# glaretechnologies/substrata

Measured on AMD Instinct MI355X. Metric: physics steps/sec at fixed dt, 100k bodies, higher is better.
Workload: dtype f32; 1 GPU; BASELINE config 3: 100000 mixed box/sphere/capsule bodies, 100x100x10 lattice spacing 1.5 m, seed 3, ground quad 2000 m, dt 1/60, Jolt default settings (10 velocity / 2 position iterations), sleeping enabled; bodies_per_gpu=100000, tiles=1, active_bodies_end=99193, contact_constraints_start=296641, contact_constraints_end=299690, contact_points_end=362045, colours_end=21, contact_constraints_after_settle=293058, dropped_pairs_or_manifolds=0

## Files before the change

### substrata_amd/csrc/sgp_dev_solve.h

```cpp
#pragma once

SGP_DEV sym33 body_world_inv_inertia(const DV& d, uint32_t body)
{
	return world_inv_inertia(quat_to_m33(Q4(d.pose[POSE_F4 * (size_t)body + 1])), V3(d.pose[POSE_F4 * (size_t)body + 2]));
}
SGP_DEV sym33 body_world_inv_inertia_rec(const DV& d, uint32_t body)
{
	const float4 a = d.vel[VEL_F4 * (size_t)body + 2], b = d.vel[VEL_F4 * (size_t)body + 3];
	sym33 s; s.xx = a.x; s.xy = a.y; s.xz = a.z; s.yy = a.w; s.yz = b.x; s.zz = b.y;
	return s;
}

SGP_DEV float lane_swap1(float x)
{
	return __int_as_float(__builtin_amdgcn_mov_dpp(__float_as_int(x), 0xB1, 0xF, 0xF, true));
}

struct ConHalf {
	uint32_t body;
	float4 nf; int np_col;
	v3     c[4][3];
	v3     iv[4][3];
	float  eff[4][3];
	float  bias[4];
// ... 67 lines not shown
			h.lam[i] = V3(l4);
		}
	}
}

template <int ROWS = -1> SGP_DEV void half_load_known(const DV& d, uint32_t slot, int side, int np_col, uint32_t body, ConHalf& h)
{
	h.body = body;
	h.nf = CUR(d).n_fric[slot];
	h.np_col = np_col;
	half_load_rows<ROWS>(d, slot, side, h);
}
template <int ROWS = -1> SGP_DEV void half_load(const DV& d, uint32_t slot, int side, ConHalf& h)
{
	const uint4 hd = con_hdr(CUR(d), slot);
	half_load_known<ROWS>(d, slot, side, (int)hd.z, side ? hd.y : hd.x, h);
}

SGP_DEV void half_store(const DV& d, uint32_t slot, int side, const ConHalf& h)
{
	if (side) return;
	const int np = h.np_col & 0xFF;
#pragma unroll
	for (int i = 0; i < 4; ++i) { if (i < np) CUR(d).lam[i][slot] = F4(h.lam[i], 0.0f); }
}

SGP_DEV float half_jv(v3 lv, v3 av, v3 axis, v3 c, int side)
{
	const float mine = v3_dot(axis, lv) + v3_dot(c, av);
	const float other = lane_swap1(mine);
	return side ? other - mine : mine - other;
}
SGP_DEV void half_apply(v3& lv, v3& av, float im, v3 axis, v3 iv, float lambda, int side)
{
	if (!(im > 0.0f)) return;
	if (side) { lv = v3_add(lv, v3_scale(axis, lambda * im)); av = v3_add(av, v3_scale(iv, lambda)); }
	else      { lv = v3_sub(lv, v3_scale(axis, lambda * im)); av = v3_sub(av, v3_scale(iv, lambda)); }
}

SGP_DEV bool half_solve_core(ConHalf& h, int side, float4& v4, float4& w4, uint32_t dbg)
{
	const int np = h.np_col & 0xFF;
	const float im = v4.w, friction = h.nf.w;
	v3 lv = V3(v4), av = V3(w4);
	const v3 n = V3(h.nf);
	const v3 t1 = (dbg & 2u) ? v3_normalized_perpendicular(n) : h.t1;
	const v3 t2 = v3_cross(n, t1);
	if (friction > 0.0f) {
#pragma unroll
		for (int i = 0; i < 4; ++i) {
			if (i < np && !(h.eff[i][1] <= 0.0f && h.eff[i][2] <= 0.0f)) {
				float l1 = h.lam[i].y + h.eff[i][1] * half_jv(lv, av, t1, h.c[i][1], side);
				float l2 = h.lam[i].z + h.eff[i][2] * half_jv(lv, av, t2, h.c[i][2], side);
				const float max_f = friction * h.lam[i].x;
				const float tot_sq = l1 * l1 + l2 * l2;
				if (tot_sq > max_f * max_f) { const float sc = max_f / sqrtf(tot_sq); l1 = l1 * sc; l2 = l2 * sc; }
				half_apply(lv, av, im, t1, h.iv[i][1], l1 - h.lam[i].y, side); h.lam[i].y = l1;
				half_apply(lv, av, im, t2, h.iv[i][2], l2 - h.lam[i].z, side); h.lam[i].z = l2;
			}
		}
	}
#pragma unroll
	for (int i = 0; i < 4; ++i) {
		if (i < np && h.eff[i][0] > 0.0f) {
			const float jv = half_jv(lv, av, n, h.c[i][0], side);
			const float lambda = h.eff[i][0] * (jv - h.bias[i]);
			const float nl = max0f(h.lam[i].x + lambda);
			half_apply(lv, av, im, n, h.iv[i][0], nl - h.lam[i].x, side);
			h.lam[i].x = nl;
		}
	}
	v4 = F4(lv, im); w4 = F4(av, 0.0f);
	return im > 0.0f;
}
template <int VS> SGP_DEV void half_solve(ConHalf& h, int side, float4* vel, uint32_t dbg = 0)
{
	if ((h.np_col & 0xFF) == 0) return;
	float4 v4 = vel[VS * (size_t)h.body], w4 = vel[VS * (size_t)h.body + 1];
	if (half_solve_core(h, side, v4, w4, dbg)) { vel[VS * (size_t)h.body] = v4; vel[VS * (size_t)h.body + 1] = w4; }
}

template <int VS, int ROWS = -1> SGP_DEV void solve_velocity_pair_t(const DV& d, uint32_t slot, int side, float4* vel)
{
	ConHalf h;
	half_load<ROWS>(d, slot, side, h);
	half_solve<VS>(h, side, vel, d.dbg_flags);
	half_store(d, slot, side, h);
}

template <int VS> SGP_DEV void solve_velocity_pair_norows(const DV& d, uint32_t slot, int side, float4* vel)
{
	const uint4 hd = con_hdr(CUR(d), slot);
	const int np = (int)hd.z & 0xFF;
	const uint32_t body = side ? hd.y : hd.x;
	const float4 nf = CUR(d).n_fric[slot];
	float4 r4[4]; float2 et[4]; v3 lam[4];
#pragma unroll
	for (int i = 0; i < 4; ++i) {
		if (i == 0 || i < np) { r4[i] = side ? CUR(d).r2e[i][slot] : CUR(d).r1b[i][slot]; et[i] = CUR(d).efft[i][slot]; lam[i] = V3(CUR(d).lam[i][slot]); }
		else { r4[i] = make_float4(0.0f, 0.0f, 0.0f, 0.0f); et[i] = make_float2(0.0f, 0.0f); lam[i] = V3(0.0f, 0.0f, 0.0f); }
	}
	if (np == 0) return;
	const sym33 I = body_world_inv_inertia_rec(d, body);
	float4 v4 = vel[VS * (size_t)body], w4 = vel[VS * (size_t)body + 1];
	const float im = v4.w, friction = nf.w;
	v3 lv = V3(v4), av = V3(w4);
	const v3 n = V3(nf);
	const v3 t1 = v3_normalized_perpendicular(n);
	const v3 t2 = v3_cross(n, t1);
	float eff0[4], bias[4];
#pragma unroll
	for (int i = 0; i < 4; ++i) { const float ow = lane_swap1(r4[i].w); eff0[i] = side ? r4[i].w : ow; bias[i] = side ? ow : r4[i].w; }
	if (friction > 0.0f) {
#pragma unroll
		for (int i = 0; i < 4; ++i) {
			if (i < np && !(et[i].x <= 0.0f && et[i].y <= 0.0f)) {
				const v3 r = V3(r4[i]);
				const v3 c1 = v3_cross(r, t1), c2 = v3_cross(r, t2);
				float l1 = lam[i].y + et[i].x * half_jv(lv, av, t1, c1, side);
				float l2 = lam[i].z + et[i].y * half_jv(lv, av, t2, c2, side);
				const float max_f = friction * lam[i].x;
				const float tot_sq = l1 * l1 + l2 * l2;
				if (tot_sq > max_f * max_f) { const float sc = max_f / sqrtf(tot_sq); l1 = l1 * sc; l2 = l2 * sc; }
				half_apply(lv, av, im, t1, sym33_mul(I, c1), l1 - lam[i].y, side); lam[i].y = l1;
				half_apply(lv, av, im, t2, sym33_mul(I, c2), l2 - lam[i].z, side); lam[i].z = l2;
			}
		}
	}
#pragma unroll
	for (int i = 0; i < 4; ++i) {
		if (i < np && eff0[i] > 0.0f) {
			const v3 c0 = v3_cross(V3(r4[i]), n);
			const float jv = half_jv(lv, av, n, c0, side);
			const float lambda = eff0[i] * (jv - bias[i]);
			const float nl = max0f(lam[i].x + lambda);
			half_apply(lv, av, im, n, sym33_mul(I, c0), nl - lam[i].x, side);
			lam[i].x = nl;
		}
	}
	if (im > 0.0f) { vel[VS * (size_t)body] = F4(lv, im); vel[VS * (size_t)body + 1] = F4(av, 0.0f); }
	if (!side) {
#pragma unroll
		for (int i = 0; i < 4; ++i) { if (i < np) CUR(d).lam[i][slot] = F4(lam[i], 0.0f); }
	}
}

struct PosHalf { float4 nf; int np; v3 loc[4]; };
SGP_DEV void pos_half_load(const DV& d, uint32_t slot, int side, int np_col, PosHalf& ph)
{
	ph.nf = CUR(d).n_fric[slot];
	ph.np = np_col & 0xFF;
#pragma unroll
	for (int i = 0; i < 4; ++i) if (i == 0 || i < ph.np) ph.loc[i] = V3(side ? CUR(d).loc2[i][slot] : CUR(d).loc1[i][slot]);
}
SGP_DEV void pos_half_solve(const DV& d, const PosHalf& ph, int side, float4* rec, v3 ii)
{
	const v3 nrm = V3(ph.nf);
	const int np = ph.np;
	const float4 p4 = rec[0];
	const float im = p4.w;
	quat q = Q4(rec[1]);
	v3 pos = V3(p4);
	bool moved = false;
	m33 R = quat_to_m33(q);
#pragma unroll
	for (int i = 0; i < 4; ++i) {
		if (i >= np) continue;
		const v3 mine = v3_add(pos, m33_mul(R, ph.loc[i]));
		const v3 other = V3(lane_swap1(mine.x), lane_swap1(mine.y), lane_swap1(mine.z));
		const v3 p1 = side ? other : mine, p2 = side ? mine : other;
		float sep = v3_dot(v3_sub(p2, p1), nrm) + d.st.penetration_slop;
		if (sep < 0.0f) {
			sep = fmaxf(sep, -d.st.max_penetration_distance);
			const v3 mid = v3_scale(v3_add(p1, p2), 0.5f);
			const v3 r = v3_sub(mid, pos);
			v3 Ic = V3(0.0f, 0.0f, 0.0f);
			float share = 0.0f;
			if (im > 0.0f) { const v3 c = v3_cross(r, nrm); Ic = sym33_mul(world_inv_inertia(R, ii), c); share = im + v3_dot(Ic, c); }
			const float oshare = lane_swap1(share);
			const float s1 = side ? oshare : share, s2 = side ? share : oshare;
			const float inv = s1 + s2;
			const float eff = inv > 0.0f ? 1.0f / inv : 0.0f;
			if (eff <= 0.0f) continue;
			const float lambda = -eff * d.st.baumgarte * sep;
			if (im > 0.0f) {
				if (side) { pos = v3_add(pos, v3_scale(nrm, lambda * im)); q = quat_add_rotation_step(q, v3_scale(Ic, lambda)); }
				else      { pos = v3_sub(pos, v3_scale(nrm, lambda * im)); q = quat_add_rotation_step(q, v3_scale(Ic, -lambda)); }
				R = quat_to_m33(q);
			}
			moved = true;
		}
	}
	if (moved && im > 0.0f) { rec[0] = F4(pos, im); rec[1] = make_float4(q.x, q.y, q.z, q.w); }
}
SGP_DEV void solve_position_pair(const DV& d, uint32_t slot, int side)
{
	const uint4 hd = con_hdr(CUR(d), slot);
	const uint32_t body = side ? hd.y : hd.x;
	PosHalf ph;
	pos_half_load(d, slot, side, (int)hd.z, ph);
	pos_half_solve(d, ph, side, d.pose + POSE_F4 * (size_t)body, V3(d.pose[POSE_F4 * (size_t)body + 2]));
}
SGP_DEV void solve_position_pair_at(const DV& d, uint32_t slot, int side, float4* rec, v3 ii)
{
	PosHalf ph;
	pos_half_load(d, slot, side, con_npc(CUR(d), slot), ph);
	pos_half_solve(d, ph, side, rec, ii);
}
#define SOLVE_VEL_TPB 256
#define SOLVE_XCD_CHUNKS 0x100

SGP_DEV uint32_t uf_prio(uint32_t x);
SGP_DEV uint32_t uf_find(const uint32_t* parent, uint32_t x);
```

### substrata_amd/csrc/sgp_k_solve.hip

```cpp
#include "sgp_dev_all.h"


struct BodyVel { v3 lv, av; };

SGP_DEV void apply_impulse(BodyVel& A, BodyVel& B, float im1, const sym33& I1, float im2, const sym33& I2, v3 r1, v3 r2, v3 axis, float lambda)
{
	if (im1 > 0.0f) {
		A.lv = v3_sub(A.lv, v3_scale(axis, lambda * im1));
		A.av = v3_sub(A.av, v3_scale(sym33_mul(I1, v3_cross(r1, axis)), lambda));
	}
	if (im2 > 0.0f) {
		B.lv = v3_add(B.lv, v3_scale(axis, lambda * im2));
		B.av = v3_add(B.av, v3_scale(sym33_mul(I2, v3_cross(r2, axis)), lambda));
	}
}

SGP_DEV float axis_jv(const BodyVel& A, const BodyVel& B, v3 r1, v3 r2, v3 axis)
{
	return (v3_dot(axis, A.lv) + v3_dot(v3_cross(r1, axis), A.av)) - (v3_dot(axis, B.lv) + v3_dot(v3_cross(r2, axis), B.av));
}

struct PairCtx { uint2 ab; float im1, im2; sym33 I1, I2; BodyVel A, B; v3 n, t1, t2; float friction; int np; };
template <int VS> SGP_DEV void load_pair(const DV& d, uint32_t slot, PairCtx& c, const float4* vel)
{
// ... 209 lines not shown
	}
}

#define TAIL_VEL_TPB 768
template <int ROWS> __global__ void __launch_bounds__(TAIL_VEL_TPB) k_solve_tail_vel(DV d, int first_colour)
{
	__shared__ uint32_t cs[SGP_MAX_COLOURS + 1];
	if (threadIdx.x <= SGP_MAX_COLOURS) cs[threadIdx.x] = d.cstarts[threadIdx.x];
	__syncthreads();
	if (cs[first_colour] == cs[SGP_MAX_COLOURS]) return;
	const int side = (int)(threadIdx.x & 1u);
	const uint32_t pair = threadIdx.x >> 1;
	const uint32_t tail_n = cs[SGP_OVERFLOW_COLOUR] - cs[first_colour];
	if (tail_n <= TAIL_VEL_TPB / 2 && !(d.dbg_flags & 1u)) {
		const uint32_t slot = cs[first_colour] + pair;
		const bool mine = pair < tail_n;
		ConHalf h; int my_col = -1;
		if (mine) { half_load<ROWS>(d, slot, side, h); my_col = (h.np_col >> 8) & 0xFF; }
		for (int c = first_colour; c < SGP_OVERFLOW_COLOUR; ++c) {
			if (cs[c] == cs[c + 1]) continue;
			if (my_col == c) half_solve<VEL_F4>(h, side, d.vel, d.dbg_flags);
			__syncthreads();
		}
		if (mine) half_store(d, slot, side, h);
	} else
	for (int c = first_colour; c < SGP_OVERFLOW_COLOUR; ++c) {
		const uint32_t b = cs[c], e = cs[c + 1];
		if (b == e) continue;
		for (uint32_t k = b + pair; k < e; k += TAIL_VEL_TPB / 2) solve_velocity_pair_t<VEL_F4, ROWS>(d, k, side, d.vel);
		__syncthreads();
	}
	const uint32_t first = cs[SGP_OVERFLOW_COLOUR], count = cs[SGP_OVERFLOW_COLOUR + 1] - first;
	if (count == 0 || threadIdx.x >= 2) return;
	uint64_t last = 0; bool have_last = false;
	for (uint32_t it = 0; it < count; ++it) {
		const uint32_t bslot = overflow_next(d, first, count, last, have_last);
		solve_velocity_pair_t<VEL_F4, ROWS>(d, bslot, side, d.vel);
	}
}
#define HC_CLASSES 9
#define HC_WG_PAIRS 256
#define HC_TPB (2 * HC_WG_PAIRS)
#define HC_BIG 0xFFFFFFFFu
#define HC_NONE 0xFFFFFFFFu
#define NPCOL_CATCH_ALL (1 << 17)
#define HC_BIG_LIST (4 * HC_WG_PAIRS)

SGP_DEV bool hc_can_move(const DV& d, uint32_t body) { return d.vel[VEL_F4 * (size_t)body].w > 0.0f; }

__global__ void __launch_bounds__(TPB) k_hc_hook(DV d, int first_colour)
{
	const uint32_t b = d.cstarts[first_colour], e = d.cstarts[SGP_OVERFLOW_COLOUR];
	const uint32_t tid = blockIdx.x * TPB + threadIdx.x, stride = gridDim.x * TPB;
	const uint32_t lim = min(2u * (e - b) + HC_CLASSES * HC_WG_PAIRS, d.cap_hc_list);
	for (uint32_t i = tid; i < lim; i += stride) d.hc_list[i] = HC_NONE;
	for (uint32_t k = b + tid; k < e; k += stride) {
		const uint2 ab = con_ab(CUR(d), k);
		if (!hc_can_move(d, ab.x) || !hc_can_move(d, ab.y)) continue;
		uint32_t ra = uf_find(d.hc_root, ab.x), rb = uf_find(d.hc_root, ab.y);
		while (ra != rb) {
			const bool a_hi = uf_prio(ra) > uf_prio(rb);
			const uint32_t hi = a_hi ? ra : rb, lo = a_hi ? rb : ra;
			const uint32_t old = atomicCAS(&d.hc_root[hi], hi, lo);
			if (old == hi) break;
			ra = uf_find(d.hc_root, old); rb = uf_find(d.hc_root, lo);
		}
	}
}
SGP_DEV uint32_t hc_root_of(const DV& d, uint2 ab)
{
	const uint32_t x = hc_can_move(d, ab.x) ? ab.x : (hc_can_move(d, ab.y) ? ab.y : HC_NONE);
	return x == HC_NONE ? HC_NONE : uf_find(d.hc_root, x);
}
__global__ void __launch_bounds__(TPB) k_hc_count(DV d, int first_colour)
{
	const uint32_t b = d.cstarts[first_colour], e = d.cstarts[SGP_OVERFLOW_COLOUR];
	for (uint32_t k = b + blockIdx.x * TPB + threadIdx.x; k < e; k += gridDim.x * TPB) {
		const uint32_t r = hc_root_of(d, con_ab(CUR(d), k));
		d.hc_rank[k] = r == HC_NONE ? 0u : atomicAdd(&d.hc_count[r], 1u);
	}
}
__global__ void __launch_bounds__(TPB) k_hc_alloc(DV d, int first_colour)
{
	const uint32_t b = d.cstarts[first_colour], e = d.cstarts[SGP_OVERFLOW_COLOUR];
	const int lane = (int)(threadIdx.x & 63u);
	for (uint32_t k0 = b + blockIdx.x * TPB; k0 < e; k0 += gridDim.x * TPB) {
		const uint32_t k = k0 + threadIdx.x;
		uint32_t r = HC_NONE, size = 0;
		if (k < e && d.hc_rank[k] == 0u) { r = hc_root_of(d, con_ab(CUR(d), k)); if (r != HC_NONE) size = d.hc_count[r]; }
		const bool lead = r != HC_NONE;
		int cls = -1;
		if (lead) {
			if (size > (uint32_t)HC_WG_PAIRS) d.hc_base[r] = HC_BIG;
			else cls = size <= 1u ? 0 : 32 - __clz((int)(size - 1u));
		}
		unsigned long long mine_m = 0ull;
#pragma unroll
		for (int c = 0; c < HC_CLASSES; ++c) { const unsigned long long m = __ballot(cls == c); if (cls == c) mine_m = m; }
		const int leader = mine_m ? __ffsll((long long)mine_m) - 1 : lane;
		uint32_t base = 0;
		if (cls >= 0 && lane == leader) base = atomicAdd(&d.ctr->hc_class[cls], (uint32_t)__popcll(mine_m));
		base = __shfl(base, leader, 64);
		if (cls >= 0) d.hc_base[r] = ((uint32_t)cls << 28) | (base + (uint32_t)__popcll(mine_m & ((1ull << lane) - 1ull)));
	}
}
SGP_DEV uint32_t hc_class_first(const DV& d, int cls)
{
	uint32_t first = 0;
	for (int c = 0; c < cls; ++c) first += ((d.ctr->hc_class[c] << c) + (HC_WG_PAIRS - 1)) & ~(uint32_t)(HC_WG_PAIRS - 1);
	return first;
}
__global__ void __launch_bounds__(TPB) k_hc_scatter(DV d, int first_colour)
{
	const uint32_t b = d.cstarts[first_colour], e = d.cstarts[SGP_OVERFLOW_COLOUR];
	if (blockIdx.x == 0 && threadIdx.x == 0) { d.ctr->hc_entries = hc_class_first(d, HC_CLASSES); d.ctr->hc_n = e - b; }
	for (uint32_t k = b + blockIdx.x * TPB + threadIdx.x; k < e; k += gridDim.x * TPB) {
		const uint32_t r = hc_root_of(d, con_ab(CUR(d), k));
		const uint32_t place = r == HC_NONE ? HC_BIG : d.hc_base[r];
		uint32_t at = HC_NONE;
		if (place != HC_BIG) {
			const int cls = (int)(place >> 28);
			at = hc_class_first(d, cls) + ((place & 0x0FFFFFFFu) << cls) + d.hc_rank[k];
		}
		if (at < d.cap_hc_list) d.hc_list[at] = k;
		else {
			con_npc(CUR(d), k) |= NPCOL_CATCH_ALL;
			const uint32_t bi = wave_alloc(&d.ctr->hc_n_big);
			if (bi < HC_BIG_LIST) d.hc_big_list[bi] = k;
		}
	}
}

__global__ void __launch_bounds__(TPB) k_hc_init(DV d, int first_colour)
{
	const uint32_t b = d.cstarts[first_colour], e = d.cstarts[SGP_OVERFLOW_COLOUR];
	for (uint32_t k = b + blockIdx.x * TPB + threadIdx.x; k < e; k += gridDim.x * TPB) {
		const uint2 ab = con_ab(CUR(d), k);
		if (hc_can_move(d, ab.x)) { d.hc_root[ab.x] = ab.x; d.hc_count[ab.x] = 0u; }
		if (hc_can_move(d, ab.y)) { d.hc_root[ab.y] = ab.y; d.hc_count[ab.y] = 0u; }
	}
}
__global__ void __launch_bounds__(TPB) k_hc_probe(DV d, int first_colour)
{
	const uint32_t b = d.cstarts[first_colour], e = d.cstarts[SGP_OVERFLOW_COLOUR];
	for (uint32_t k = b + blockIdx.x * TPB + threadIdx.x; k < e; k += gridDim.x * TPB) {
		if (d.hc_rank[k] != 0u) continue;
		const uint32_t r = hc_root_of(d, con_ab(CUR(d), k));
		if (r == HC_NONE) continue;
		const uint32_t size = d.hc_count[r];
		if (size > (uint32_t)HC_WG_PAIRS) atomicAdd(&d.ctr->hc_probe_big, size);
	}
}

__global__ void __launch_bounds__(HC_WG_PAIRS) k_hc_sort(DV d)
{
	__shared__ uint32_t s_cnt[SGP_MAX_COLOURS], s_first[SGP_MAX_COLOURS];
	__shared__ uint4 s_slot[HC_WG_PAIRS];
	const uint32_t entries = d.ctr->hc_entries;
	for (uint32_t e0 = blockIdx.x * HC_WG_PAIRS; e0 < entries; e0 += gridDim.x * HC_WG_PAIRS) {
		if (threadIdx.x < SGP_MAX_COLOURS) s_cnt[threadIdx.x] = 0u;
		__syncthreads();
		const uint32_t slot = d.hc_list[e0 + threadIdx.x];
		const uint4 hd = slot != HC_NONE ? con_hdr(CUR(d), slot) : make_uint4(0u, 0u, 0u, 0u);
		const int npc = (int)hd.z;
		const uint2 ab = make_uint2(hd.x, hd.y);
		const int col = slot != HC_NONE ? ((npc >> 8) & 0xFF) : SGP_MAX_COLOURS - 1;
		const uint32_t rank = atomicAdd(&s_cnt[col], 1u);
		__syncthreads();
		if (threadIdx.x < 64) {
			const uint32_t v = s_cnt[threadIdx.x];
			uint32_t x = v;
			for (int off = 1; off < 64; off <<= 1) { const uint32_t y = __shfl_up(x, off, 64); if ((int)threadIdx.x >= off) x += y; }
			s_first[threadIdx.x] = x - v;
		}
		__syncthreads();
		s_slot[s_first[col] + rank] = make_uint4(slot, (uint32_t)npc, ab.x, ab.y);
		__syncthreads();
		d.hc_entry[e0 + threadIdx.x] = s_slot[threadIdx.x];
		__syncthreads();
	}
}

#define HC_TABLE 1024
template <int MODE, int ROWS = -1> __global__ void __launch_bounds__(HC_TPB) k_solve_hc(const StepCounters* ctr_pre, const uint4* hc_entry_pre, DV d, int first_colour)
{
	constexpr int RS = MODE == 1 ? 2 : 3;
	__shared__ float4 s_rec[HC_TABLE * RS];
	__shared__ uint32_t s_key[HC_TABLE];
	__shared__ unsigned long long s_present;
	__shared__ uint32_t s_ticket;
	const int side = (int)(threadIdx.x & 1u);
	const uint32_t pair = threadIdx.x >> 1;
	const uint32_t entries = ctr_pre->hc_entries;
	const int n_colours = (int)ctr_pre->n_colours;
	for (uint32_t e0 = blockIdx.x * HC_WG_PAIRS; e0 < entries; e0 += gridDim.x * HC_WG_PAIRS) {
		__syncthreads();
		for (uint32_t i = threadIdx.x; i < HC_TABLE; i += HC_TPB) s_key[i] = HC_NONE;
		if (threadIdx.x == 0) s_present = 0ull;
		__syncthreads();
		const uint4 entry = hc_entry_pre[e0 + pair];
		const uint32_t slot = entry.x;
		const bool mine = slot != HC_NONE;
		ConHalf h; PosHalf ph; int my_col = -1;
		uint32_t body = HC_NONE, at = 0; bool owner = false;
		if (mine) {
			my_col = ((int)entry.y >> 8) & 0xFF;
			body = side ? entry.w : entry.z;
			if (MODE == 1) half_load_known<ROWS>(d, slot, side, (int)entry.y, body, h); else pos_half_load(d, slot, side, (int)entry.y, ph);
			if (side == 0) atomicOr(&s_present, 1ull << my_col);
			at = uf_prio(body) & (HC_TABLE - 1);
			for (;;) {
				const uint32_t old = atomicCAS(&s_key[at], HC_NONE, body);
				if (old == HC_NONE) { owner = true; break; }
				if (old == body) break;
				at = (at + 1) & (HC_TABLE - 1);
			}
			if (owner) {
				const float4* g = (MODE == 1 ? d.vel + VEL_F4 * (size_t)body : d.pose + POSE_F4 * (size_t)body);
				s_rec[RS * at] = g[0]; s_rec[RS * at + 1] = g[1];
				if (MODE != 1) s_rec[RS * at + 2] = d.pose[POSE_F4 * (size_t)body + 2];
			}
			if (MODE == 1) h.body = at;
		}
		__syncthreads();
		const unsigned long long present = s_present;
		for (int c = first_colour; c < n_colours; ++c) {
			if (!((present >> c) & 1ull)) continue;
			if (my_col == c) { if (MODE == 1) half_solve<2>(h, side, s_rec, d.dbg_flags); else pos_half_solve(d, ph, side, s_rec + RS * at, V3(s_rec[RS * at + 2])); }
			__syncthreads();
		}
		if (MODE == 1 && mine) half_store(d, slot, side, h);
		if (owner && s_rec[RS * at].w > 0.0f) {
			float4* g = (MODE == 1 ? d.vel + VEL_F4 * (size_t)body : d.pose + POSE_F4 * (size_t)body);
			g[0] = s_rec[RS * at]; g[1] = s_rec[RS * at + 1];
		}
	}
	const uint32_t n_big = d.ctr->hc_n_big;
	const uint32_t ofirst = d.cstarts[SGP_OVERFLOW_COLOUR], ocount = d.cstarts[SGP_OVERFLOW_COLOUR + 1] - ofirst;
	if (n_big == 0u && ocount == 0u) return;
	__syncthreads();
	if (threadIdx.x == 0) { __threadfence(); s_ticket = atomicAdd(&d.ctr->hc_done, 1u); }
	__syncthreads();
	if (s_ticket != gridDim.x - 1u) return;
	if (threadIdx.x == 0) d.ctr->hc_done = 0u;
	__threadfence();
	if (n_big != 0u && n_big <= (uint32_t)HC_BIG_LIST) {
		uint32_t mine[4]; int mcol[4]; int cnt = 0;
		for (uint32_t e = pair; e < n_big; e += HC_WG_PAIRS) { const uint32_t k = d.hc_big_list[e]; mine[cnt] = k; mcol[cnt] = (int)((con_npc(CUR(d), k) >> 8) & 0xFF); ++cnt; }
		for (int c = first_colour; c < n_colours; ++c) {
#pragma unroll
			for (int j = 0; j < 4; ++j) if (j < cnt && mcol[j] == c) { if (MODE == 1) solve_velocity_pair_t<VEL_F4, ROWS>(d, mine[j], side, d.vel); else solve_position_pair(d, mine[j], side); }
			__syncthreads();
		}
	} else
	for (int c = first_colour; c < n_colours && n_big != 0u; ++c) {
		const uint32_t cb = d.cstarts[c], ce = d.cstarts[c + 1];
		for (uint32_t k = cb + pair; k < ce; k += HC_WG_PAIRS) {
			if (!(con_npc(CUR(d), k) & NPCOL_CATCH_ALL)) continue;
			if (MODE == 1) solve_velocity_pair_t<VEL_F4, ROWS>(d, k, side, d.vel); else solve_position_pair(d, k, side);
		}
		__syncthreads();
	}
	if (ocount == 0u || threadIdx.x >= 2u) return;
	uint64_t last = 0; bool have_last = false;
	for (uint32_t it = 0; it < ocount; ++it) {
		const uint32_t bslot = overflow_next(d, ofirst, ocount, last, have_last);
		if (MODE == 1) solve_velocity_pair_t<VEL_F4, ROWS>(d, bslot, side, d.vel); else solve_position_pair(d, bslot, side);
	}
}

#define SMALL_LDS_BODIES 2048
#define SMALL_TPB 768
__global__ void __launch_bounds__(SMALL_TPB) k_solve_small(DV d, int warm_start, int iterations)
{
	__shared__ float4 sv[2 * SMALL_LDS_BODIES];
	__shared__ uint32_t cs[SGP_MAX_COLOURS + 1];
	const uint32_t n = min(d.sp->n_slots, (uint32_t)SMALL_LDS_BODIES);
	if (threadIdx.x <= SGP_MAX_COLOURS) cs[threadIdx.x] = d.cstarts[threadIdx.x];
	for (uint32_t i = threadIdx.x; i < 2 * n; i += SMALL_TPB) sv[i] = d.vel[VEL_F4 * (size_t)(i >> 1) + (i & 1u)];
	__syncthreads();
	const int side = (int)(threadIdx.x & 1u);
	const uint32_t pair = threadIdx.x >> 1;
	const uint32_t all_n = cs[SGP_OVERFLOW_COLOUR];
	if (all_n != 0 && all_n <= SMALL_TPB / 2 && cs[SGP_OVERFLOW_COLOUR] == cs[SGP_MAX_COLOURS]) {
		const uint32_t slot = pair;
		const bool mine = slot < all_n;
		if (warm_start) {
			for (int c = 0; c < SGP_OVERFLOW_COLOUR; ++c) {
				const uint32_t b = cs[c], e = cs[c + 1];
				if (b == e) continue;
				if (side == 0 && slot >= b && slot < e) warm_start_one_t<2>(d, slot, sv);
				__syncthreads();
			}
		}
		ConHalf h; int my_col = -1;
		if (mine) { half_load<0>(d, slot, side, h); my_col = (h.np_col >> 8) & 0xFF; }
		for (int pass = 0; pass < iterations; ++pass) {
			for (int c = 0; c < SGP_OVERFLOW_COLOUR; ++c) {
				if (cs[c] == cs[c + 1]) continue;
				if (my_col == c) half_solve<2>(h, side, sv, d.dbg_flags);
				__syncthreads();
			}
		}
		if (mine) half_store(d, slot, side, h);
	} else
	if (cs[0] != cs[SGP_MAX_COLOURS]) {
		for (int pass = warm_start ? -1 : 0; pass < iterations; ++pass) {
			for (int c = 0; c < SGP_OVERFLOW_COLOUR; ++c) {
				const uint32_t b = cs[c], e = cs[c + 1];
				if (b == e) continue;
				if (pass < 0) { for (uint32_t k = b + threadIdx.x; k < e; k += SMALL_TPB) warm_start_one_t<2>(d, k, sv); }
				else { for (uint32_t k = b + pair; k < e; k += SMALL_TPB / 2) solve_velocity_pair_t<2, 0>(d, k, side, sv); }
				__syncthreads();
			}
			const uint32_t first = cs[SGP_OVERFLOW_COLOUR], count = cs[SGP_OVERFLOW_COLOUR + 1] - first;
			if (count != 0) {
				if (threadIdx.x < 2) {
					uint64_t last = 0; bool have_last = false;
					for (uint32_t it = 0; it < count; ++it) {
						const uint32_t bslot = overflow_next(d, first, count, last, have_last);
						if (pass < 0) { if (side == 0) warm_start_one_t<2>(d, bslot, sv); } else solve_velocity_pair_t<2, 0>(d, bslot, side, sv);
					}
				}
				__syncthreads();
			}
		}
	}
	for (uint32_t i = threadIdx.x; i < 2 * n; i += SMALL_TPB) d.vel[VEL_F4 * (size_t)(i >> 1) + (i & 1u)] = sv[i];
}

struct ConReg { uint2 ab; float4 nf; int np_col; AxisRows rn[4], rt1[4], rt2[4]; float4 lam[4]; };

SGP_DEV void con_load(const DV& d, uint32_t slot, ConReg& r)
{
	const uint4 hd = con_hdr(CUR(d), slot);
	r.ab = make_uint2(hd.x, hd.y);
	r.nf = CUR(d).n_fric[slot];
	r.np_col = (int)hd.z;
	const int np = r.np_col & 0xFF;
#pragma unroll
	for (int i = 0; i < 4; ++i) {
		if (i < np) {
			r.rn[i] = load_axis_rows(d, slot, i, 0); r.rt1[i] = load_axis_rows(d, slot, i, 1); r.rt2[i] = load_axis_rows(d, slot, i, 2);
			r.lam[i] = CUR(d).lam[i][slot];
		}
	}
}

SGP_DEV void con_store(const DV& d, uint32_t slot, const ConReg& r)
{
	const int np = r.np_col & 0xFF;
#pragma unroll
	for (int i = 0; i < 4; ++i) { if (i < np) CUR(d).lam[i][slot] = r.lam[i]; }
}

template <int VS> SGP_DEV void con_solve_velocity(ConReg& r, float4* vel, uint32_t dbg = 0)
{
	const uint2 ab = r.ab;
	const int np = r.np_col & 0xFF;
	if (np == 0) return;
	const float4 va = vel[VS * (size_t)ab.x], wa = vel[VS * (size_t)ab.x + 1];
	const float4 vb = vel[VS * (size_t)ab.y], wb = vel[VS * (size_t)ab.y + 1];
	const float im1 = va.w, im2 = vb.w, friction = r.nf.w;
	BodyVel A, B;
	A.lv = V3(va); A.av = V3(wa); B.lv = V3(vb); B.av = V3(wb);
	const v3 n = V3(r.nf);
	const v3 t1 = (dbg & 2u) ? v3_normalized_perpendicular(n) : V3(r.rn[0].i1.w, r.rn[0].i2.w, r.rt1[0].i1.w);
	const v3 t2 = v3_cross(n, t1);
	if (friction > 0.0f) {
#pragma unroll
		for (int i = 0; i < 4; ++i) {
			if (i < np && !(r.rt1[i].c2.w <= 0.0f && r.rt2[i].c2.w <= 0.0f)) {
				float l1 = r.lam[i].y + r.rt1[i].c2.w * rows_jv(A, B, t1, r.rt1[i]);
				float l2 = r.lam[i].z + r.rt2[i].c2.w * rows_jv(A, B, t2, r.rt2[i]);
				const float max_f = friction * r.lam[i].x;
				const float tot_sq = l1 * l1 + l2 * l2;
				if (tot_sq > max_f * max_f) { const float sc = max_f / sqrtf(tot_sq); l1 = l1 * sc; l2 = l2 * sc; }
				rows_apply(A, B, im1, im2, t1, r.rt1[i], l1 - r.lam[i].y); r.lam[i].y = l1;
				rows_apply(A, B, im1, im2, t2, r.rt2[i], l2 - r.lam[i].z); r.lam[i].z = l2;
			}
		}
	}
#pragma unroll
	for (int i = 0; i < 4; ++i) {
		if (i < np && r.rn[i].c2.w > 0.0f) {
			const float jv = rows_jv(A, B, n, r.rn[i]);
			const float lambda = r.rn[i].c2.w * (jv - r.rn[i].c1.w);
			const float nl = max0f(r.lam[i].x + lambda);
			rows_apply(A, B, im1, im2, n, r.rn[i], nl - r.lam[i].x);
			r.lam[i].x = nl;
		}
	}
	if (im1 > 0.0f) { vel[VS * (size_t)ab.x] = F4(A.lv, im1); vel[VS * (size_t)ab.x + 1] = F4(A.av, 0.0f); }
	if (im2 > 0.0f) { vel[VS * (size_t)ab.y] = F4(B.lv, im2); vel[VS * (size_t)ab.y + 1] = F4(B.av, 0.0f); }
}

template <int VS> SGP_DEV void solve_velocity_one_t(const DV& d, uint32_t slot, float4* vel)
{
	ConReg r;
	con_load(d, slot, r);
	con_solve_velocity<VS>(r, vel, d.dbg_flags);
	con_store(d, slot, r);
}
__global__ void __launch_bounds__(512) k_solve_small_single(DV d, int warm_start, int iterations)
{
	__shared__ float4 sv[2 * SMALL_LDS_BODIES];
	__shared__ uint32_t cs[SGP_MAX_COLOURS + 1];
	const uint32_t n = min(d.sp->n_slots, (uint32_t)SMALL_LDS_BODIES);
	if (threadIdx.x <= SGP_MAX_COLOURS) cs[threadIdx.x] = d.cstarts[threadIdx.x];
	for (uint32_t i = threadIdx.x; i < 2 * n; i += 512) sv[i] = d.vel[VEL_F4 * (size_t)(i >> 1) + (i & 1u)];
	__syncthreads();
	const uint32_t all_n = cs[SGP_OVERFLOW_COLOUR];
	if (all_n != 0 && all_n <= 512u && cs[SGP_OVERFLOW_COLOUR] == cs[SGP_MAX_COLOURS]) {
		const uint32_t slot = threadIdx.x;
		const bool mine = slot < all_n;
		if (warm_start) {
			for (int c = 0; c < SGP_OVERFLOW_COLOUR; ++c) {
				const uint32_t b = cs[c], e = cs[c + 1];
				if (b == e) continue;
				if (slot >= b && slot < e) warm_start_one_t<2>(d, slot, sv);
				__syncthreads();
			}
		}
		ConReg r; int my_col = -1;
		if (mine) { con_load(d, slot, r); my_col = (r.np_col >> 8) & 0xFF; }
		for (int pass = 0; pass < iterations; ++pass) {
			for (int c = 0; c < SGP_OVERFLOW_COLOUR; ++c) {
				if (cs[c] == cs[c + 1]) continue;
				if (my_col == c) con_solve_velocity<2>(r, sv, d.dbg_flags);
				__syncthreads();
			}
		}
		if (mine) con_store(d, slot, r);
	} else
	if (cs[0] != cs[SGP_MAX_COLOURS]) {
		for (int pass = warm_start ? -1 : 0; pass < iterations; ++pass) {
			for (int c = 0; c < SGP_OVERFLOW_COLOUR; ++c) {
				const uint32_t b = cs[c], e = cs[c + 1];
				if (b == e) continue;
				for (uint32_t k = b + threadIdx.x; k < e; k += 512) {
					if (pass < 0) warm_start_one_t<2>(d, k, sv); else solve_velocity_one_t<2>(d, k, sv);
				}
				__syncthreads();
			}
			const uint32_t first = cs[SGP_OVERFLOW_COLOUR], count = cs[SGP_OVERFLOW_COLOUR + 1] - first;
			if (count != 0) {
				if (threadIdx.x == 0) {
					uint64_t last = 0; bool have_last = false;
					for (uint32_t it = 0; it < count; ++it) {
						uint64_t best = ~0ull; uint32_t bslot = first;
						for (uint32_t k = 0; k < count; ++k) {
							const uint2 okab = con_ab(CUR(d), first + k); const uint64_t pr = sgp_mix64(((uint64_t)okab.x << 32) | okab.y);
							if ((!have_last || pr > last) && pr <= best) { best = pr; bslot = first + k; }
						}
						last = best; have_last = true;
						if (pass < 0) warm_start_one_t<2>(d, bslot, sv); else solve_velocity_one_t<2>(d, bslot, sv);
					}
				}
				__syncthreads();
			}
		}
	}
	for (uint32_t i = threadIdx.x; i < 2 * n; i += 512) d.vel[VEL_F4 * (size_t)(i >> 1) + (i & 1u)] = sv[i];
}
#ifndef SGP_EXPERIMENTS
void launch_solve_probe(const DV&, int, int, uint32_t, hipStream_t) {}
void launch_ts_label(const DV&, uint32_t, hipStream_t) {}
void launch_colour_count_ts(const DV&, uint32_t, hipStream_t) {}
void launch_setup_ts(const DV&, uint32_t, hipStream_t) {}
void launch_ts_solve(const DV&, int, int, hipStream_t) {}
#endif
#define SOLVE_MANY_MIN 131072u
#ifndef SOLVE_MANY_OCC
#define SOLVE_MANY_OCC 3
#endif
void launch_solve_colour(const DV& d, int colour, uint32_t est, int mode, hipStream_t s, int compact_rows)
{
	uint32_t blocks = (est + est / 8 + 64 + SOLVE_TPB - 1) / SOLVE_TPB;
	if (mode != 0) blocks = (est + est / 8 + 64 + SOLVE_VEL_TPB / 2 - 1) / (SOLVE_VEL_TPB / 2);
	if (blocks > 8192) blocks = 8192;
	if (mode != 0) blocks = (blocks + 7u) & ~7u;
	if (mode != 0 && est >= 8192u && est <= 65536u) colour |= SOLVE_XCD_CHUNKS;
	if (mode == 0) hipLaunchKernelGGL(k_solve_colour<0>, dim3(blocks), dim3(SOLVE_TPB), 0, s, (const uint32_t*)d.cstarts, d.sp, d, colour);
	else if (mode == 1) {
		const bool many = est > SOLVE_MANY_MIN;
		if (compact_rows == 2) hipLaunchKernelGGL((k_solve_colour<1, 2>), dim3(blocks), dim3(SOLVE_VEL_TPB), 0, s, (const uint32_t*)d.cstarts, d.sp, d, colour);
		else if (compact_rows) { if (many) hipLaunchKernelGGL((k_solve_colour<1, 1, SOLVE_MANY_OCC>), dim3(blocks), dim3(SOLVE_VEL_TPB), 0, s, (const uint32_t*)d.cstarts, d.sp, d, colour); else hipLaunchKernelGGL((k_solve_colour<1, 1>), dim3(blocks), dim3(SOLVE_VEL_TPB), 0, s, (const uint32_t*)d.cstarts, d.sp, d, colour); }
		else hipLaunchKernelGGL((k_solve_colour<1, 0>), dim3(blocks), dim3(SOLVE_VEL_TPB), 0, s, (const uint32_t*)d.cstarts, d.sp, d, colour);
	}
	else if (est > SOLVE_MANY_MIN) hipLaunchKernelGGL((k_solve_colour<2, -1, SOLVE_MANY_OCC>), dim3(blocks), dim3(SOLVE_VEL_TPB), 0, s, (const uint32_t*)d.cstarts, d.sp, d, colour);
	else hipLaunchKernelGGL(k_solve_colour<2>, dim3(blocks), dim3(SOLVE_VEL_TPB), 0, s, (const uint32_t*)d.cstarts, d.sp, d, colour);
}
void launch_warm_bodies(const DV& d, uint32_t nb, hipStream_t s) { hipLaunchKernelGGL(k_warm_bodies, dim3(blocks_for(nb)), dim3(TPB), 0, s, d); }
void launch_solve_tail(const DV& d, int first_colour, int mode, hipStream_t s, int compact_rows)
{
	if (mode == 1) {
		if (compact_rows == 2) hipLaunchKernelGGL(k_solve_tail_vel<2>, dim3(1), dim3(TAIL_VEL_TPB), 0, s, d, first_colour);
		else if (compact_rows) hipLaunchKernelGGL(k_solve_tail_vel<1>, dim3(1), dim3(TAIL_VEL_TPB), 0, s, d, first_colour);
		else hipLaunchKernelGGL(k_solve_tail_vel<0>, dim3(1), dim3(TAIL_VEL_TPB), 0, s, d, first_colour);
	}
	else hipLaunchKernelGGL(k_solve_tail, dim3(1), dim3(512), 0, s, d, first_colour, mode);
}
void launch_hc_build(const DV& d, int first_colour, uint32_t est, hipStream_t s)
{
	const uint32_t blocks = std::max(1u, std::min(1024u, (est + est / 8 + TPB - 1) / TPB));
	hipLaunchKernelGGL(k_hc_hook, dim3(blocks), dim3(TPB), 0, s, d, first_colour);
	hipLaunchKernelGGL(k_hc_count, dim3(blocks), dim3(TPB), 0, s, d, first_colour);
	hipLaunchKernelGGL(k_hc_alloc, dim3(blocks), dim3(TPB), 0, s, d, first_colour);
	hipLaunchKernelGGL(k_hc_scatter, dim3(blocks), dim3(TPB), 0, s, d, first_colour);
	hipLaunchKernelGGL(k_hc_sort, dim3(std::max(1u, std::min(2048u, (2u * est + HC_CLASSES * HC_WG_PAIRS) / HC_WG_PAIRS))), dim3(HC_WG_PAIRS), 0, s, d);
}
void launch_hc_probe(const DV& d, int probe_colour, uint32_t probe_est, hipStream_t s)
{
	const uint32_t pb = std::max(1u, std::min(1024u, (probe_est + probe_est / 8 + TPB - 1) / TPB));
	hipLaunchKernelGGL(k_hc_hook, dim3(pb), dim3(TPB), 0, s, d, probe_colour);
	hipLaunchKernelGGL(k_hc_count, dim3(pb), dim3(TPB), 0, s, d, probe_colour);
	hipLaunchKernelGGL(k_hc_probe, dim3(pb), dim3(TPB), 0, s, d, probe_colour);
	hipLaunchKernelGGL(k_hc_init, dim3(pb), dim3(TPB), 0, s, d, probe_colour);
}
void launch_solve_hc(const DV& d, int first_colour, uint32_t est, int mode, hipStream_t s, int compact_rows)
{
	const uint32_t blocks = std::max(1u, std::min(2048u, (2u * est + HC_CLASSES * HC_WG_PAIRS) / HC_WG_PAIRS));
	if (mode == 1) {
		if (compact_rows == 2) hipLaunchKernelGGL((k_solve_hc<1, 2>), dim3(blocks), dim3(HC_TPB), 0, s, (const StepCounters*)d.ctr, (const uint4*)d.hc_entry, d, first_colour);
		else if (compact_rows) hipLaunchKernelGGL((k_solve_hc<1, 1>), dim3(blocks), dim3(HC_TPB), 0, s, (const StepCounters*)d.ctr, (const uint4*)d.hc_entry, d, first_colour);
		else hipLaunchKernelGGL((k_solve_hc<1, 0>), dim3(blocks), dim3(HC_TPB), 0, s, (const StepCounters*)d.ctr, (const uint4*)d.hc_entry, d, first_colour);
	}
	else hipLaunchKernelGGL((k_solve_hc<2, -1>), dim3(blocks), dim3(HC_TPB), 0, s, (const StepCounters*)d.ctr, (const uint4*)d.hc_entry, d, first_colour);
}
void launch_solve_small(const DV& d, int warm_start, int iterations, int lane_pairs, hipStream_t s)
{
	if (lane_pairs) hipLaunchKernelGGL(k_solve_small, dim3(1), dim3(SMALL_TPB), 0, s, d, warm_start, iterations);
	else hipLaunchKernelGGL(k_solve_small_single, dim3(1), dim3(512), 0, s, d, warm_start, iterations);
}
```

### substrata_amd/csrc/sgp_kernels.h

```cpp
#pragma once
#include <hip/hip_runtime.h>
#include <stdint.h>
#include "../../include/sgp.h"

#define BF_MOTION_MASK   0x3u
#define BF_LAYER_SHIFT   2
#define BF_LAYER_MASK    (0x3u << BF_LAYER_SHIFT)
#define BF_ALIVE         (1u << 4)
#define BF_ACTIVE        (1u << 5)
#define BF_SENSOR        (1u << 6)
#define BF_ALLOW_SLEEP   (1u << 7)
#define BF_ZERO_LIN_DRAG (1u << 8)
#define BF_LARGE         (1u << 9)
#define BF_UNDERWATER    (1u << 10)
#define BF_GHOST         (1u << 11)
#define BF_HAS_FORCE     (1u << 13)
#define BF_CACHE_INVALID (1u << 12)
#define BF_SHAPE_SHIFT   18
#define BF_SHAPE_MASK    (0x7u << BF_SHAPE_SHIFT)
#define BF_CHASSIS       (1u << 22)
#define BF_ALIAS         (1u << 21)
#define BF_WAKE          (1u << 14)
#define BF_CAN_SLEEP     (1u << 15)
#define BF_MOVABLE_PREV  (1u << 16)
// ... 83 lines not shown
	uint32_t colour_fill[SGP_MAX_COLOURS];
	uint32_t cnp_count[SGP_MAX_COLOURS * 4];
	uint32_t cnp_start[SGP_MAX_COLOURS * 4];
	uint32_t cnp_fill[SGP_MAX_COLOURS * 4];
};

struct EventCounters {
	uint32_t n_activated;
	uint32_t n_deactivated;
	uint32_t n_water;
	uint32_t n_contact_added;
	uint32_t n_contact_persisted;
	uint32_t pad[3];
};
#define SGP_EVENT_WINDOW 256u
struct EventWindow {
	EventCounters c;
	uint32_t ids[3][SGP_EVENT_WINDOW];
};

#define CMD_SET_POS      (1u << 0)
#define CMD_SET_ROT      (1u << 1)
#define CMD_SET_VEL      (1u << 2)
#define CMD_SET_SHAPE    (1u << 3)
#define CMD_ADD_FORCE    (1u << 4)
#define CMD_ADD_TORQUE   (1u << 5)
#define CMD_ADD_FORCE_AT (1u << 6)
#define CMD_ACTIVATE     (1u << 7)
#define CMD_SET_LAYER    (1u << 8)
#define CMD_REMOVE       (1u << 9)
#define CMD_MOVE_KINEMATIC (1u << 10)
#define CMD_CREATE       (1u << 11)
#define CMD_SET_CHASSIS  (1u << 12)

struct GhostRefresh { uint32_t id; float pos[3]; float rot[4]; float linv[3]; float angv[3]; };

struct BodyCmd {
	uint32_t id;
	uint32_t ops;
	float pos[3];
	float rot[4];
	float linv[3];
	float angv[3];
	float shape[4];
	float dt;
	float inv_mass, mass;
	float inv_inertia[3];
	float friction, restitution, gravity_factor, lin_damp, ang_damp;
	uint32_t flags;
	uint32_t pad_;
	uint64_t userdata;
};

struct StepParams {
	float    dt;
	uint32_t n_slots;
	uint32_t n_large;
	float    cell_size;
	float    bp_rmax;
	int      water_enabled; float water_z;
	int      contact_events;
	uint32_t parity;
	uint32_t compact_rows;
	uint32_t pad[6];
};

#define PREC_F4 4
struct ConstraintArrays {
	uint4*    hdr;
	float4*   n_fric;
	float4*   r1b[4];
	float4*   r2e[4];
	float4*   lam[4];
	float2*   efft[4];
	float4*   loc1[4];
	float4*   loc2[4];
	float4*   prec;
};

#define POSE_F4 4u
#define VEL_F4 4u
struct DV {
	StepParams* sp;
	uint32_t cap_bodies, cap_pairs, cap_manifolds;
	float4* pose;
	float4* vel;
	float4* dyn;
	float4* force;
	float4* torque;
	uint32_t* flags;
	float4* aabb_min;
	float4* aabb_max;
	float4* sleep_s[3];
	float*  sleep_timer;
	uint32_t* sleep_label;
	uint32_t* slot_gen;
	uint32_t* label_wake;
	uint2*  wake_pairs; uint32_t cap_wake_pairs;
	float*  submerged;
	uint64_t* userdata;
	uint64_t* colour_mask;
	float4* warm;
	uint64_t* claim[2];
	uint32_t* island;
	uint32_t* island_awake;
	uint32_t* export_counts;
	uint32_t* awake_mark;
	uint32_t ts_nt, ts_gx, ts_gy;
	uint8_t*  body_tile;
	uint64_t* body_tiles4;
	uint8_t*  man_tile;
	uint32_t* ts_count;
	uint32_t* ts_start;
	uint32_t* ts_fill;
	uint32_t* ts_adj;
	uint64_t* ts_wait;
	uint32_t* ts_epoch;
	uint32_t* ts_flags;
	uint16_t* ts_at;
	uint8_t*  ts_side;
	uint32_t table_size;
	uint32_t* cell_hash;
	uint32_t* cell_count;
	uint32_t* cell_start;
	uint32_t* cell_fill;
	uint32_t* scan_block_sums;
	float4*   sorted_min;
	float4*   sorted_max;
	struct BpGrid* grid;
	int*      bounds_acc;
	uint32_t* grid_cells_used;
	uint32_t* tile_slot;
	uint32_t* tile_of_slot;
	uint32_t  tile_table_size;
	const uint32_t* large_ids;
	uint2*    pairs;
	uint2*    man_ab;
	float4*   man_n;
	float4*   man_p1[4];
	float4*   man_p2[4];
	int32_t*  man_colour;
	uint32_t* ulist[2];
	uint64_t* man_prio;
	uint32_t* man_slot;
	uint32_t* man_prev;
	uint32_t* hc_root;
	uint32_t* hc_count;
	uint32_t* hc_base;
	uint32_t* hc_rank;
	uint32_t* hc_list;
	uint4*    hc_entry;
	uint32_t  cap_hc_list;
	uint32_t* hc_big_list;
	uint32_t dbg_flags;
	float4* rows;
	ConstraintArrays ca[2];
	uint4* ht; uint32_t ht_size;
	uint32_t* cache_total;
	uint32_t* ht_cur;
	uint32_t* cstarts;
	StepCounters* ctr;
	EventCounters* evc;
	uint32_t* ev_activated; uint32_t* ev_deactivated; uint32_t* ev_water;
	uint32_t ev_window;
	sgp_contact_event* ev_contacts_added; sgp_contact_event* ev_contacts_persisted; uint32_t cap_contact_events;
	const struct sgd_hull_s* hulls; uint32_t n_hulls;
	uint2* hull_pairs; uint32_t cap_hull_pairs;
	struct HullWork* hull_work;
	const struct MeshHeader* meshes; uint32_t n_meshes;
	const float4* mesh_verts; const uint4* mesh_tris; const uint32_t* mesh_tri_mat; const struct MeshNode* mesh_nodes; const uint32_t* mesh_field;
	const LargeGrid* lgrid; const uint32_t* lg_start; const uint32_t* lg_items;
	uint2* mesh_pairs; uint32_t cap_mesh_pairs; uint32_t* mesh_big;
	struct sgd_vehicle* vehicles; uint32_t n_vehicles; const sgp_vehicle_input* vehicle_inputs;
	float4* veh_rows; float4* veh_head; uint32_t veh_cap;
	uint64_t* veh_claim; uint32_t* veh_epoch; uint32_t* veh_defer_bits;
	sgp_settings st;
	float gx, gy, gz;
};

void launch_step_begin(const DV& d, const StepParams& sp, uint32_t nb, bool reset_step_scratch, bool ev_reset, hipStream_t s);
void launch_set_params(const DV& d, const StepParams& sp, hipStream_t s);
void launch_step_end(const DV& d, StepCounters* host_mapped, EventWindow* host_events, hipStream_t s);
void launch_fill_u64(uint64_t* p, uint64_t v, size_t n, hipStream_t s);
void launch_pre_solve(const DV& d, uint32_t nb, hipStream_t s);
void launch_bp_bounds(const DV& d, uint32_t nb, hipStream_t s);
void launch_bp_cell(const DV& d, uint32_t nb, hipStream_t s);
void launch_bp_scan(const DV& d, hipStream_t s);
void launch_bp_scatter(const DV& d, uint32_t nb, hipStream_t s);
void launch_bp_pairs(const DV& d, int small_lds, hipStream_t s);
void launch_bp_large(const DV& d, uint32_t nb, hipStream_t s);
void launch_bp_scatter_large(const DV& d, uint32_t nb, hipStream_t s);
void launch_narrowphase(const DV& d, uint32_t n_pairs_upper, hipStream_t s);
void launch_wake_round(const DV& d, uint32_t nb, int has_hulls, bool has_meshes, hipStream_t s);
void launch_narrowphase_hull(const DV& d, bool big_hulls, hipStream_t s);
void launch_narrowphase_mesh(const DV& d, bool has_hulls, hipStream_t s);
void launch_narrowphase_mesh_blocks(const DV& d, bool has_hulls, uint32_t blocks, hipStream_t s);
void launch_colour_inherit(const DV& d, uint32_t n_man, hipStream_t s);
void launch_colour_claim(const DV& d, uint32_t n_man, uint32_t round, hipStream_t s);
void launch_colour_commit(const DV& d, uint32_t n_man, uint32_t round, hipStream_t s);
void launch_colour_count(const DV& d, uint32_t n_man, hipStream_t s);
void launch_colour_finish(const DV& d, uint32_t first_round, int build_list, hipStream_t s);
void launch_setup(const DV& d, uint32_t n_man, hipStream_t s);
void launch_ts_label(const DV& d, uint32_t nb, hipStream_t s);
void launch_colour_count_ts(const DV& d, uint32_t n_man, hipStream_t s);
void launch_setup_ts(const DV& d, uint32_t n_man, hipStream_t s);
void launch_ts_solve(const DV& d, int passes, int colour_end, hipStream_t s);
void launch_solve_colour(const DV& d, int colour, uint32_t est, int mode, hipStream_t s, int compact_rows);
void launch_solve_probe(const DV& d, int variant, int colour, uint32_t est, hipStream_t s);
void launch_warm_bodies(const DV& d, uint32_t nb, hipStream_t s);
void launch_solve_tail(const DV& d, int first_colour, int mode, hipStream_t s, int compact_rows = 0);
#define SGP_SMALL_WORLD_BODIES 2048
void launch_hc_build(const DV& d, int first_colour, uint32_t est, hipStream_t s);
void launch_hc_probe(const DV& d, int probe_colour, uint32_t probe_est, hipStream_t s);
void launch_solve_hc(const DV& d, int first_colour, uint32_t est, int mode, hipStream_t s, int compact_rows);
void launch_solve_small(const DV& d, int warm_start, int iterations, int lane_pairs, hipStream_t s);
void launch_integrate_pose(const DV& d, uint32_t nb, hipStream_t s);
void launch_finalize(const DV& d, uint32_t nb, hipStream_t s);
void launch_island_mark(const DV& d, uint32_t n_con, int clear_cache, hipStream_t s);
void launch_island_hook(const DV& d, uint32_t n_con, hipStream_t s);
void launch_island_flag(const DV& d, uint32_t n_con, hipStream_t s);
void launch_sleep_apply(const DV& d, uint32_t nb, hipStream_t s);
void launch_buoyancy(const DV& d, uint32_t nb, hipStream_t s);
void launch_cache_build(const DV& d, uint32_t n_con, StepCounters* host_mapped, EventWindow* host_events, hipStream_t s);
void launch_contact_events(const DV& d, uint32_t n_man, hipStream_t s);
void launch_ghost_refresh(const DV& d, const GhostRefresh* recs, uint32_t n, hipStream_t s);
void launch_apply_cmds(const DV& d, const BodyCmd* cmds, const uint32_t* run_start, uint32_t n_runs, hipStream_t s);
void launch_gather_aabbs(const DV& d, const uint32_t* ids, uint32_t n, float4* out, hipStream_t s);
void launch_gather_states(const DV& d, const uint32_t* ids, uint32_t first, uint32_t n, sgp_body_state* out, hipStream_t s);
void launch_gather_active(const DV& d, uint32_t nb, sgp_body_state* out, uint32_t cap, hipStream_t s);
void launch_gather_active_poses(const DV& d, uint32_t nb, void* out, uint32_t cap, hipStream_t s);
void launch_dump_constraints(const DV& d, uint32_t which, uint32_t n_con, void* out, uint32_t cap, hipStream_t s);
void launch_vehicle_pre(const DV& d, bool cylinder_testers, hipStream_t s);
void launch_vehicle_solve(const DV& d, int mode, hipStream_t s);
void launch_solve_colour_veh(const DV& d, int colour, uint32_t est, int mode, hipStream_t s, int compact_rows);
struct RayMailbox {
	uint32_t req_seq, stop_gen; sgp_ray ray; uint32_t pad0[16 - 2 - sizeof(sgp_ray) / 4];
	uint32_t done_seq, exited_gen; sgp_hit hit; uint32_t pad1[16 - 2 - sizeof(sgp_hit) / 4 - 1]; uint32_t done_seq2;
};
static_assert(sizeof(RayMailbox) == 128 && sizeof(sgp_ray) == 36 && sizeof(sgp_hit) == 48, "RayMailbox: two 64-byte lines");
void launch_ray_server(const DV& d, RayMailbox* mb, uint32_t first_seq, uint32_t generation, uint64_t idle_ticks, uint64_t max_ticks, hipStream_t s);
void launch_raycast(const DV& d, const sgp_ray* rays, uint32_t n, sgp_hit* hits, hipStream_t s);
void launch_collide_capsules(const DV& d, const sgp_capsule_query* q, uint32_t n, sgp_query_contact* out, uint32_t cap, uint32_t* count, hipStream_t s);
void launch_spherecast(const DV& d, const sgp_ray* rays, const float* radii, uint32_t n, sgp_hit* hits, hipStream_t s);
enum { SQ_N_OUT = 0, SQ_N_PRIM = 1, SQ_N_HULL = 2, SQ_N_MESH = 3 };
struct SqBufs {
	const sgp_shape_query* qs; uint32_t n;
	sgp_query_contact* out; uint32_t cap;
	uint32_t* ctr;
	uint2* prim; uint2* hull; uint2* mesh; uint32_t pcap;
};
void launch_shape_queries_wave(const DV& d, const SqBufs& b, hipStream_t s);
void launch_shape_queries_pairs(const DV& d, const SqBufs& b, hipStream_t s);
enum { SC_N_OUT = 0, SC_N_PRIM = 1, SC_N_HULL = 2, SC_N_MESH = 3, SC_N_CAPPED = 4, SC_N_DROPPED = 5, SC_N_CTR = 8 };
struct ScBufs {
	const sgp_shape_cast* cs; uint32_t n;
	sgp_cast_hit* out;
	uint32_t* ctr;
	uint2* prim; uint2* hull; uint2* mesh; uint32_t pcap;
};
void launch_shape_casts(const DV& d, const ScBufs& b, hipStream_t s);
#define SGP_CHAR_MAX_PUSHES 32
#define SGP_CHAR_MAX_ADDED 32
#define SGP_CHAR_MAX_SEEN 128
#define SGP_CHAR_MESH_LIST 32
struct CharRec {
	uint32_t alive, reset_serial, pose_serial, pad_;
	float pose[3];
	float radius, half_height, offset[3], up[3], sv_n[3], sv_c, cos_max_slope, mass, max_strength, predictive, padding, recovery, tolerance;
	uint32_t max_coll_it, max_cons_it; float min_time;
	float stick[3], stairs_up[3], min_step_fwd, step_fwd_test, cos_fwd, down_extra[3];
};
struct CharIn { float vel[3]; uint32_t ignore, flags, serial; };
struct CharContact { uint32_t body, idx; float p[3], n[3], v[3], dist; uint32_t bits; float inv_mass; };
struct CharState {
	float pos[3], vel[3]; uint32_t ground_state; float gn[3], gv[3], gp[3]; uint32_t ground_body, overflow;
	uint32_t n_active, n_seen, reset_serial, pose_serial, in_serial, pad_[3];
};
struct CharPush { uint32_t body; float f[3], p[3]; uint32_t pad_; };
struct CharAdded { uint32_t body, pad_; float p[3], n[3]; };
struct CharBufs {
	const CharRec* rec; const CharIn* in; CharState* st;
	CharContact* active;
	uint32_t* seen;
	CharPush* push; uint32_t* n_push;
	uint32_t* push_any;
	CharAdded* added; uint32_t* n_added;
	uint32_t n;
};
void launch_characters_update(const DV* d_dev, const CharBufs& b, float dt, hipStream_t s);
void launch_characters_push(const DV& d, const CharBufs& b, hipStream_t s);
void launch_characters_sync(const CharBufs& b, hipStream_t s);
void launch_export_boundary(const DV& d, uint32_t nb, float3 lo, float3 hi, float margin, sgp_ghost_record* out, uint32_t cap, uint32_t* count, hipStream_t s);

#define SGP_MAX_TILES 64
struct TileRoute { float boxes[6 * SGP_MAX_TILES]; uint32_t n_tiles, my_rank; float margin, pad; };
struct RouteHeader { uint32_t seg_count[SGP_MAX_TILES]; uint32_t seg_start[SGP_MAX_TILES]; uint32_t n_emigrants; uint32_t total; uint32_t pad[2]; };
#define SGP_TILE_HIST_BINS 1024
struct TilePlanes { uint32_t gx, gy, gz, by_contacts; float glo[3], ghi[3]; float xp[4]; float yp[16]; };
void launch_tiles_hist(const DV& d, uint32_t nb, const TilePlanes& tp, int level, uint32_t* out, hipStream_t s);
#define ROUTE_OK 0u
#define ROUTE_REDO 1u
#define ROUTE_FAILED 2u
void launch_route_export(const DV& d, uint32_t nb, const TileRoute& t, uint32_t* block_counts, uint32_t* block_offsets, RouteHeader* header,
                         sgp_ghost_record* out, uint32_t cap, uint32_t* emigrant_ids, uint32_t emigrant_cap, uint32_t* gather_row, uint32_t cap_recv, uint32_t host_status, hipStream_t s);
void launch_pack_ghost_keys(const sgp_ghost_record* recs, uint32_t n, void* out_uint4, void* aux_uint4, const float* region_lo, const float* region_hi, hipStream_t s);
void launch_create_from_records(const DV& d, const sgp_ghost_record* recs, const void* list_uint4, uint32_t n, float gravity_factor, float lin_damp, float ang_damp, hipStream_t s);
#define GKEY_VALID      (1u << 0)
#define GKEY_SHAPE_SHIFT 1
#define GKEY_FLAGS_SHIFT 4
#define GKEY_IN_REGION  (1u << 10)
void launch_ghost_refresh_records(const DV& d, const sgp_ghost_record* recs, const uint32_t* ids, uint32_t n, hipStream_t s);

#define SGP_CKPT_MAX_SEGS 160
struct CkptTable { uint32_t n; uint32_t start[SGP_CKPT_MAX_SEGS + 1]; const void* src[SGP_CKPT_MAX_SEGS]; void* dst[SGP_CKPT_MAX_SEGS]; };
void launch_ckpt_copy(const CkptTable& t, uint32_t n_cus, hipStream_t s);
void launch_ckpt_grid_reset(const DV& d, hipStream_t s);
```

### substrata_amd/csrc/sgp_world.hip

```cpp
#include "sgp_world_internal.h"

thread_local std::string g_last_error;
int g_device_count = -1;

static std::mutex g_worlds_mutex;
static std::set<uint64_t> g_worlds;
static uint64_t g_next_serial = 0;
uint64_t world_register() { std::lock_guard<std::mutex> l(g_worlds_mutex); const uint64_t s = ++g_next_serial; g_worlds.insert(s); return s; }
void world_unregister(uint64_t serial) { std::lock_guard<std::mutex> l(g_worlds_mutex); g_worlds.erase(serial); }
bool world_alive(uint64_t serial) { std::lock_guard<std::mutex> l(g_worlds_mutex); return g_worlds.count(serial) != 0; }


SGP_API void sgp_default_settings(sgp_settings* s)
{
	s->num_velocity_steps = 10;
	s->num_position_steps = 2;
	s->baumgarte = 0.2f;
	s->penetration_slop = 0.02f;
	s->speculative_contact_distance = 0.02f;
	s->min_velocity_for_restitution = 1.0f;
	s->max_penetration_distance = 0.2f;
	s->time_before_sleep = 0.5f;
	s->point_velocity_sleep_threshold = 0.03f;
	s->contact_point_preserve_lambda_max_dist_sq = 0.01f * 0.01f;
// ... 8 lines not shown

SGP_API void sgp_default_world_desc(sgp_world_desc* d)
{
	memset(d, 0, sizeof(*d));
	d->max_bodies = 65536;
	d->gravity[0] = 0.0f; d->gravity[1] = 0.0f; d->gravity[2] = -9.81f;
	d->large_body_radius = 4.0f;
	sgp_default_settings(&d->settings);
}

SGP_API void sgp_default_body_desc(sgp_body_desc* d)
{
	memset(d, 0, sizeof(*d));
	d->rot[3] = 1.0f;
	d->shape_type = SGP_SHAPE_BOX;
	d->shape[0] = d->shape[1] = d->shape[2] = 0.5f;
	d->motion_type = SGP_MOTION_STATIC;
	d->layer = SGP_LAYER_NON_MOVING;
	d->mass = 100.0f; d->friction = 0.5f; d->restitution = 0.3f;
	d->gravity_factor = 1.0f;
	d->linear_damping = 0.05f; d->angular_damping = 0.05f;
	d->allow_sleeping = 1;
}

SGP_API int sgp_abi_version(void) { return SGP_ABI_VERSION; }
SGP_API const char* sgp_last_error(void) { return g_last_error.c_str(); }
SGP_API const char* sgp_kernel_class_name(int k) { return (k >= 0 && k < KC_COUNT) ? k_class_names[k] : nullptr; }
SGP_API int sgp_abi_sizeof(int which)
{
	switch (which) {
	case 0: return (int)sizeof(sgp_settings); case 1: return (int)sizeof(sgp_world_desc); case 2: return (int)sizeof(sgp_body_desc);
	case 3: return (int)sizeof(sgp_body_state); case 4: return (int)sizeof(sgp_body_event); case 5: return (int)sizeof(sgp_contact_event);
	case 6: return (int)sizeof(sgp_ray); case 7: return (int)sizeof(sgp_hit); case 8: return (int)sizeof(sgp_step_stats);
	case 9: return (int)sizeof(sgp_step_profile); case 10: return (int)sizeof(sgp_ghost_record);
	case 11: return (int)sizeof(sgp_vehicle_desc); case 12: return (int)sizeof(sgp_vehicle_input); case 13: return (int)sizeof(sgp_vehicle_state);
	case 14: return (int)sizeof(sgp_hull_info); case 15: return (int)sizeof(sgp_capsule_query); case 16: return (int)sizeof(sgp_query_contact); case 17: return (int)sizeof(sgp_mesh_info);
	case 18: return (int)sizeof(sgp_heightfield_desc); case 19: return (int)sizeof(sgp_checkpoint_info); case 20: return (int)sizeof(sgp_shape_query);
	case 22: return (int)sizeof(sgp_shape_cast); case 23: return (int)sizeof(sgp_cast_hit);
	case 25: return (int)sizeof(sgp_character_desc); case 26: return (int)sizeof(sgp_character_input); case 27: return (int)sizeof(sgp_character_state);
	case 28: return (int)sizeof(sgp_character_contact);
	default: return -1;
	}
}

SGP_API int sgp_init(void)
{
	int n = 0;
	const hipError_t e = hipGetDeviceCount(&n);
	if (e != hipSuccess || n <= 0) { g_device_count = 0; return fail(SGP_ERR_NO_DEVICE, "no HIP device available (there is no CPU fallback)", e); }
	g_device_count = n;
	return n;
}


static int alloc_constraints(sgp_world* w, ConstraintArrays& c, uint32_t cap)
{
	DEV_ALLOC(c.hdr, cap); DEV_ALLOC(c.n_fric, cap);
	DEV_ALLOC(c.prec, (size_t)cap * PREC_F4);
	for (int k = 0; k < 4; ++k) {
		DEV_ALLOC(c.r1b[k], cap); DEV_ALLOC(c.r2e[k], cap); DEV_ALLOC(c.lam[k], cap); DEV_ALLOC(c.efft[k], cap);
		DEV_ALLOC(c.loc1[k], cap); DEV_ALLOC(c.loc2[k], cap);
	}
	return SGP_OK;
}

SGP_API int sgp_world_destroy(sgp_world* w);
SGP_API int sgp_vehicle_destroy(sgp_world* w, uint32_t id);

SGP_API int sgp_world_create(const sgp_world_desc* desc, sgp_world** out)
{
	if (!desc || !out || desc->max_bodies == 0) return fail(SGP_ERR_INVALID, "sgp_world_create: bad arguments");
	if (g_device_count < 0) sgp_init();
	if (g_device_count <= 0) return fail(SGP_ERR_NO_DEVICE, "sgp_world_create: no HIP device available (there is no CPU fallback)");
	if (desc->device < 0 || desc->device >= g_device_count) return fail(SGP_ERR_INVALID, "sgp_world_create: bad device ordinal");
	if (desc->max_bodies >= (1u << 25)) return fail(SGP_ERR_CAPACITY, "sgp_world_create: max_bodies must be below 2^25 (the cell arrays hold 64 cells per body slot in 32-bit indices)");
	sgp_world* w = new sgp_world();
	w->desc = *desc;
	w->device = desc->device;
	if (w->desc.large_body_radius <= 0.0f) w->desc.large_body_radius = 4.0f;
	if (w->desc.max_body_pairs == 0) w->desc.max_body_pairs = 16u * desc->max_bodies + 1024u;
	if (w->desc.max_manifolds == 0) w->desc.max_manifolds = std::min(8u * desc->max_bodies + 1024u, MAN_PREV_NONE - 1u);
	if (w->desc.max_manifolds >= MAN_PREV_NONE) { delete w; return fail(SGP_ERR_CAPACITY, "sgp_world_create: max_manifolds must be below 2^28 (a manifold's reference to its previous constraint keeps 28 bits for the slot)"); }
	memset(&w->dv, 0, sizeof(w->dv));
	memset(&w->stats, 0, sizeof(w->stats));
	hipError_t e = hipSetDevice(w->device);
	if (e != hipSuccess) { delete w; return fail(SGP_ERR_HIP, "hipSetDevice", e); }
	e = hipStreamCreateWithFlags(&w->stream, hipStreamNonBlocking);
	if (e != hipSuccess) { delete w; return fail(SGP_ERR_HIP, "hipStreamCreate", e); }
	e = hipStreamCreateWithFlags(&w->capture_stream, hipStreamNonBlocking);
	if (e != hipSuccess) { delete w; return fail(SGP_ERR_HIP, "hipStreamCreate", e); }
	*out = w;
	DV& d = w->dv;
	const uint32_t N = desc->max_bodies, P = w->desc.max_body_pairs, M = w->desc.max_manifolds;
	d.cap_bodies = N; d.cap_pairs = P; d.cap_manifolds = M;
	DEV_ALLOC(d.pose, POSE_F4 * (size_t)N); DEV_ALLOC(d.vel, VEL_F4 * (size_t)N); DEV_ALLOC(d.dyn, N);
	DEV_ALLOC(d.force, N); DEV_ALLOC(d.torque, N);
	DEV_ALLOC(d.flags, N); DEV_ALLOC(d.aabb_min, N); DEV_ALLOC(d.aabb_max, N);
	for (int k = 0; k < 3; ++k) DEV_ALLOC(d.sleep_s[k], N);
	DEV_ALLOC(d.sleep_timer, N); DEV_ALLOC(d.submerged, N); DEV_ALLOC(d.userdata, N);
	DEV_ALLOC(d.colour_mask, N); DEV_ALLOC(d.warm, (size_t)N * SGP_MAX_COLOURS * 2); DEV_ALLOC(d.claim[0], N); DEV_ALLOC(d.claim[1], N);
	DEV_ALLOC(d.veh_claim, N); DEV_ALLOC(d.veh_epoch, 1);
	DEV_ALLOC(d.island, N); DEV_ALLOC(d.island_awake, N); DEV_ALLOC(d.awake_mark, N); DEV_ALLOC(d.export_counts, N / 256 + 2);
	d.table_size = std::max(4096u, next_pow2(64u * N));
	DEV_ALLOC(d.cell_hash, N);
	DEV_ALLOC(d.cell_count, d.table_size + 4); DEV_ALLOC(d.cell_start, d.table_size + 4); DEV_ALLOC(d.cell_fill, d.table_size + 4);
	{
		uint32_t dflt = 1u << 16; while (dflt < (1u << 23) && (uint64_t)dflt < 1024ull * (uint64_t)N) dflt <<= 1;
		const char* e = getenv("SGP_GRID_TILE_TABLE"); d.tile_table_size = e && atoi(e) > 0 ? (uint32_t)atoi(e) : dflt;
	}
	DEV_ALLOC(d.tile_slot, d.tile_table_size); DEV_ALLOC(d.tile_of_slot, d.table_size / 64u + 4u);
	if (hipMemsetAsync(d.tile_slot, 0xFF, sizeof(uint32_t) * (size_t)d.tile_table_size, w->stream) != hipSuccess) return fail(SGP_ERR_HIP, "tile table init");
	DEV_ALLOC(w->d_large, N); w->cap_large = N; d.large_ids = w->d_large;
	DEV_ALLOC(w->d_lgrid, 1); DEV_ALLOC(w->d_lg_start, SGP_LG_MAX_CELLS + 1); w->cap_lg_items = 4096; DEV_ALLOC(w->d_lg_items, w->cap_lg_items);
	HIP_TRY(hipMemset(w->d_lgrid, 0, sizeof(LargeGrid)));
	d.lgrid = w->d_lgrid; d.lg_start = w->d_lg_start; d.lg_items = w->d_lg_items;
	{ void* q = nullptr; w->cap_mesh_table = 256; HIP_TRY(hipMalloc(&q, sizeof(MeshHeader) * w->cap_mesh_table)); HIP_TRY(hipMemsetAsync(q, 0, sizeof(MeshHeader) * w->cap_mesh_table, w->stream)); w->d_meshes = (MeshHeader*)q; w->device_bytes += sizeof(MeshHeader) * w->cap_mesh_table; }
	d.meshes = w->d_meshes; d.n_meshes = 1; w->meshes.push_back(MeshHeader{}); w->mesh_refs.push_back(0);
	d.cap_mesh_pairs = P / 4 + 1024; DEV_ALLOC(d.mesh_pairs, 4 * (size_t)d.cap_mesh_pairs); DEV_ALLOC(d.mesh_big, d.cap_mesh_pairs);
	{ void* q = nullptr; w->cap_hull_table = 64; HIP_TRY(hipMalloc(&q, sizeof(sgd_hull) * w->cap_hull_table)); HIP_TRY(hipMemsetAsync(q, 0, sizeof(sgd_hull) * w->cap_hull_table, w->stream)); w->d_hulls = (sgd_hull*)q; w->device_bytes += sizeof(sgd_hull) * w->cap_hull_table; }
	d.hulls = w->d_hulls;
	d.cap_hull_pairs = P / 4 + 1024; DEV_ALLOC(d.hull_pairs, d.cap_hull_pairs);
	{ void* hw = nullptr; const size_t bytes = (size_t)d.cap_hull_pairs * 64; HIP_TRY(hipMalloc(&hw, bytes)); w->allocs.push_back(hw); w->alloc_bytes[hw] = bytes; w->device_bytes += bytes; d.hull_work = (HullWork*)hw; }
	{
		sgd_hull cube; sgd_hull_cube_template(&cube);
		w->hulls.push_back(cube); w->hull_refs.push_back(1);
		HIP_TRY(hipMemcpyAsync(&w->d_hulls[0], &w->hulls[0], sizeof(sgd_hull), hipMemcpyHostToDevice, w->stream));
		d.n_hulls = 1;
	}
	DEV_ALLOC(d.sorted_min, N); DEV_ALLOC(d.sorted_max, N); DEV_ALLOC(d.grid, 1); DEV_ALLOC(d.grid_cells_used, 1);
	DEV_ALLOC(d.bounds_acc, 8); { const int init[8] = { 0x7FFFFFFF, 0x7FFFFFFF, 0x7FFFFFFF, (int)0x80000000, (int)0x80000000, (int)0x80000000, 0, 0 }; if (hipMemcpyAsync(d.bounds_acc, init, sizeof(init), hipMemcpyHostToDevice, w->stream) != hipSuccess || hipStreamSynchronize(w->stream) != hipSuccess) return fail(SGP_ERR_HIP, "bounds_acc init"); } DEV_ALLOC(d.scan_block_sums, (d.table_size + 1) / 1024 + 2);
	DEV_ALLOC(d.pairs, P);
	d.cap_wake_pairs = P / 4 + 1024; DEV_ALLOC(d.wake_pairs, d.cap_wake_pairs);
	DEV_ALLOC(d.sleep_label, N); DEV_ALLOC(d.label_wake, N); DEV_ALLOC(d.slot_gen, N);
	HIP_TRY(hipMemsetAsync(d.label_wake, 0, sizeof(uint32_t) * N, w->stream));
	HIP_TRY(hipMemsetAsync(d.slot_gen, 0, sizeof(uint32_t) * N, w->stream));
	DEV_ALLOC(d.man_ab, M); DEV_ALLOC(d.man_n, M); DEV_ALLOC(d.man_colour, M); DEV_ALLOC(d.man_prio, M); DEV_ALLOC(d.man_prev, M); DEV_ALLOC(d.man_slot, M);
	DEV_ALLOC(d.hc_root, N); DEV_ALLOC(d.hc_count, N); DEV_ALLOC(d.hc_base, N); DEV_ALLOC(d.hc_rank, M);
	{
		int dev = 0, cus = 0;
		if (hipGetDevice(&dev) == hipSuccess) hipDeviceGetAttribute(&cus, hipDeviceAttributeMultiprocessorCount, dev);
		d.ts_nt = 0; d.ts_gx = d.ts_gy = 0;
#ifdef SGP_EXPERIMENTS
		if (cus >= 256) { d.ts_nt = 256; d.ts_gx = 16; d.ts_gy = 16; } else if (cus >= 128) { d.ts_nt = 128; d.ts_gx = 16; d.ts_gy = 8; } else if (cus >= 64) { d.ts_nt = 64; d.ts_gx = 8; d.ts_gy = 8; }
#endif
		if (d.ts_nt) {
			const size_t E = (size_t)SGP_MAX_COLOURS * d.ts_nt;
			DEV_ALLOC(d.body_tile, N); DEV_ALLOC(d.body_tiles4, N); DEV_ALLOC(d.man_tile, M);
			DEV_ALLOC(d.ts_count, E + 1); DEV_ALLOC(d.ts_start, E + 1); DEV_ALLOC(d.ts_fill, E + 1);
			DEV_ALLOC(d.ts_adj, (size_t)d.ts_nt * 8); DEV_ALLOC(d.ts_wait, d.ts_nt); DEV_ALLOC(d.ts_epoch, (size_t)d.ts_nt * 32); DEV_ALLOC(d.ts_flags, 4);
			DEV_ALLOC(d.ts_at, 2 * (size_t)M); DEV_ALLOC(d.ts_side, 2 * (size_t)M);
		}
	}
	d.cap_hc_list = 2u * M + 4096u; DEV_ALLOC(d.hc_list, d.cap_hc_list); DEV_ALLOC(d.hc_entry, d.cap_hc_list); DEV_ALLOC(d.hc_big_list, 1024);
	DEV_ALLOC(d.ulist[0], M); DEV_ALLOC(d.ulist[1], M);
	for (int k = 0; k < 4; ++k) { DEV_ALLOC(d.man_p1[k], M); DEV_ALLOC(d.man_p2[k], M); }
	DEV_ALLOC(d.rows, (size_t)48 * M);
	{ int r = alloc_constraints(w, d.ca[0], M); if (r != SGP_OK) return r; }
	{ int r = alloc_constraints(w, d.ca[1], M); if (r != SGP_OK) return r; }
	w->ht_alloc = next_pow2(2u * M);
	DEV_ALLOC(d.ht, w->ht_alloc);
	HIP_TRY(hipMemsetAsync(d.ht, 0xFF, sizeof(uint4) * w->ht_alloc, w->stream));
	d.ht_size = w->ht_alloc;
	DEV_ALLOC(d.ht_cur, 1);
	DEV_ALLOC(d.cache_total, 2); HIP_TRY(hipMemsetAsync(d.cache_total, 0, sizeof(uint32_t) * 2, w->stream));
	{ static const uint32_t first = 1024u; HIP_TRY(hipMemcpyAsync(d.ht_cur, &first, sizeof(first), hipMemcpyHostToDevice, w->stream)); }
	DEV_ALLOC(d.cstarts, SGP_MAX_COLOURS + 2);
	DEV_ALLOC(d.ctr, 1); DEV_ALLOC(d.evc, 1);
	DEV_ALLOC(d.ev_activated, N); DEV_ALLOC(d.ev_deactivated, N); DEV_ALLOC(d.ev_water, N);
	HIP_TRY(hipHostMalloc((void**)&w->h_ctr, sizeof(StepCounters), hipHostMallocMapped));
	HIP_TRY(hipHostGetDevicePointer((void**)&w->h_ctr_dev, w->h_ctr, 0));
	HIP_TRY(hipHostMalloc((void**)&w->h_evw, sizeof(EventWindow), hipHostMallocMapped));
	HIP_TRY(hipHostGetDevicePointer((void**)&w->h_evw_dev, w->h_evw, 0));
	memset(w->h_evw, 0, sizeof(EventWindow)); w->h_evc = &w->h_evw->c;
	d.ev_window = SGP_EVENT_WINDOW;
	{ const char* e = getenv("SGP_EVENT_WINDOW"); if (e && atoi(e) >= 0) d.ev_window = std::min((uint32_t)atoi(e), SGP_EVENT_WINDOW); }
	HIP_TRY(hipHostMalloc((void**)&w->h_sp, sizeof(StepParams), hipHostMallocDefault));
	memset(w->h_sp, 0, sizeof(StepParams));
	DEV_ALLOC(w->d_sp, 1);
	d.sp = w->d_sp;
	{ StepParams init = *w->h_sp; init.parity = w->h_sp->parity ^ 1u; HIP_TRY(hipMemcpyAsync(w->d_sp, &init, sizeof(init), hipMemcpyHostToDevice, w->stream)); HIP_TRY(hipStreamSynchronize(w->stream)); }
	{ const char* e = getenv("SGP_NO_GRAPH"); if (e && e[0] == '1') w->use_graphs = false; }
	{ const char* e = getenv("SGP_NO_SMALL_WORLD"); if (e && e[0] == '1') w->use_small_world = false; }
	{ const char* e = getenv("SGP_NO_RAY_SERVER"); if (e && e[0] == '1') w->ray_server_enabled = false; }
	{ const char* e = getenv("SGP_QUERY_PATH"); if (e && !strcmp(e, "wave")) w->query_path = 1; else if (e && !strcmp(e, "pairs")) w->query_path = 2; }
	{ const char* e = getenv("SGP_NO_WAKE_ROUND"); if (e && e[0] == '1') w->use_wake_round = false; }
	{ const char* e = getenv("SGP_CHECKPOINT_FULL"); if (e && e[0] == '1') w->checkpoint_full = true; }
	w->serial = world_register();
	{ const char* e = getenv("SGP_DEBUG_FLAGS"); w->dv.dbg_flags = e ? (uint32_t)atoi(e) : 0u; }
#ifdef SGP_EXPERIMENTS
	{ const char* e = getenv("SGP_TILE_SOLVER"); if (e) w->use_tile_solver = atoi(e); }
#endif
	{ const char* e = getenv("SGP_VEHICLE_FUSED"); if (e) w->fuse_vehicle_solve = atoi(e) != 0; }
	{ const char* e = getenv("SGP_COMPACT_ROWS_MIN"); if (e && atoll(e) >= 0) w->compact_rows_min = (uint32_t)atoll(e); }
	{ const char* e = getenv("SGP_ROWS_MODE"); if (e && (atoi(e) == 1 || atoi(e) == 2)) w->rows_mode_large = (uint32_t)atoi(e); }
	{ const char* e = getenv("SGP_ROWS_IN_SMALL_WORLDS"); if (e && e[0] == '1' && !w->use_small_world) w->rows_in_small_worlds = true; }
	{ const char* e = getenv("SGP_ROWS_MODE2_MIN"); if (e && atoll(e) >= 0) w->rows_mode2_min = (uint32_t)atoll(e); }
	{ const char* e = getenv("SGP_ROWS_MODE_DEFAULT"); if (e && atoi(e) >= 0 && atoi(e) <= 2) w->rows_mode_default = (uint32_t)atoi(e); }
	{ const char* e = getenv("SGP_TS_MIN_CONSTRAINTS"); if (e && atoi(e) >= 0) w->ts_min_constraints = (uint32_t)atoi(e); }
	{ const char* e = getenv("SGP_HC_BUDGET"); if (e) { const int v = atoi(e); if (v <= 0) w->use_components = false; else w->hc_budget = (uint32_t)v; } }
	{ int dev = 0, cus = 0; if (hipGetDevice(&dev) == hipSuccess && hipDeviceGetAttribute(&cus, hipDeviceAttributeMultiprocessorCount, dev) == hipSuccess && cus > 0) w->n_cus = (uint32_t)cus; }
	{ const char* e = getenv("SGP_HC_MIN_COLOURS"); if (e && atoi(e) >= 0) w->hc_min_colours = (uint32_t)atoi(e); }
	{ const char* e = getenv("SGP_TAIL_THRESHOLD"); if (e && atoi(e) > 0) w->tail_threshold = (uint32_t)atoi(e); }
	d.st = desc->settings;
	d.gx = desc->gravity[0]; d.gy = desc->gravity[1]; d.gz = desc->gravity[2];
	w->hb.resize(N);
	HIP_TRY(hipStreamSynchronize(w->stream));
	return SGP_OK;
}

SGP_API int sgp_world_destroy(sgp_world* w)
{
	if (!w) return fail(SGP_ERR_INVALID, "sgp_world_destroy: NULL");
	if (w->serial) world_unregister(w->serial);
	hipSetDevice(w->device);
	ray_server_stop(w);
	if (w->stream) hipStreamSynchronize(w->stream);
	if (w->ray_mb) hipHostFree(w->ray_mb);
	for (void* p : w->allocs) hipFree(p);
	if (w->stage_dev) hipFree(w->stage_dev);
	if (w->d_meshes) hipFree(w->d_meshes);
	if (w->d_hulls) hipFree(w->d_hulls);
	if (w->d_mesh_verts) hipFree(w->d_mesh_verts);
	if (w->d_mesh_tris) hipFree(w->d_mesh_tris);
	if (w->d_mesh_tri_mat) hipFree(w->d_mesh_tri_mat);
	if (w->d_mesh_nodes) hipFree(w->d_mesh_nodes);
	if (w->d_mesh_field) hipFree(w->d_mesh_field);
	if (w->d_vehicles) hipFree(w->d_vehicles);
	if (w->d_veh_inputs) hipFree(w->d_veh_inputs);
	hipFree(w->d_veh_rows); hipFree(w->d_veh_head);
	if (w->stage_host) hipHostFree(w->stage_host);
	if (w->view_host) hipHostFree(w->view_host);
	if (w->h_ctr) hipHostFree(w->h_ctr);
	if (w->h_evw) hipHostFree(w->h_evw);
	if (w->h_sp) hipHostFree(w->h_sp);
	for (auto& kv : w->graphs) hipGraphExecDestroy(kv.second);
	for (hipEvent_t ev : w->event_pool) hipEventDestroy(ev);
	if (w->stage_ev_ok) for (int i = 0; i <= SGP_NUM_STAGES; ++i) hipEventDestroy(w->stage_ev[i]);
	if (w->capture_stream) hipStreamDestroy(w->capture_stream);
	if (w->stream) hipStreamDestroy(w->stream);
	delete w;
	return SGP_OK;
}


static int upload_sp(sgp_world* w)
{
	StepParams& sp = *w->h_sp;
	sp.n_slots = w->high;
	sp.n_large = (uint32_t)w->large_linear.size();
	sp.bp_rmax = std::max(0.25f, w->max_small_radius);
	sp.cell_size = sp.bp_rmax + w->dv.st.speculative_contact_distance;
	if (w->sp_uploaded_valid) {
		StepParams cmp = sp; cmp.dt = w->sp_uploaded.dt; cmp.parity = w->sp_uploaded.parity;
		if (memcmp(&w->sp_uploaded, &cmp, sizeof(cmp)) == 0) return SGP_OK;
	}
	{ StepParams up = sp; up.parity = sp.parity ^ 1u; launch_set_params(w->dv, up, w->stream); }
	w->sp_uploaded = sp; w->sp_uploaded_valid = true;
	return SGP_OK;
}

static int rebuild_large_grid(sgp_world* w)
{
	if (!w->large_dirty) {
		if (!w->large_list_dirty) return SGP_OK;
		w->large_list_dirty = false;
		if (w->large_linear.size() > w->cap_large) return fail(SGP_ERR_CAPACITY, "large-body list full");
		if (!w->large_linear.empty()) HIP_TRY(hipMemcpyAsync(w->d_large, w->large_linear.data(), sizeof(uint32_t) * w->large_linear.size(), hipMemcpyHostToDevice, w->stream));
		HIP_TRY(hipStreamSynchronize(w->stream));
		w->grid_valid = false;
		return upload_sp(w);
	}
	w->large_dirty = false; w->large_list_dirty = false;
	DV& d = w->dv;
	std::vector<uint32_t> stat;
	w->large_linear.clear();
	{
		std::vector<uint32_t> keep; keep.reserve(w->large_ids.size());
		for (uint32_t id : w->large_ids) { HostBody& b = w->hb[id]; if (b.in_large_ids == 1 && (b.flags & BF_ALIVE) && (b.flags & BF_LARGE)) { keep.push_back(id); b.in_large_ids = 2; } }
		for (uint32_t id : keep) w->hb[id].in_large_ids = 1;
		w->large_ids.swap(keep);
	}
	if (w->lg_tombs) for (HostBody& b : w->hb) b.lg_tomb = 0;
	w->lg_tombs = 0; w->lg_pending = 0;
	for (uint32_t id : w->large_ids) { w->hb[id].lg_state = 0; if ((w->hb[id].flags & BF_MOTION_MASK) == SGP_MOTION_STATIC) stat.push_back(id); else w->large_linear.push_back(id); }
	LargeGrid g; memset(&g, 0, sizeof(g)); g.cell = 1.0f; g.inv_cell = 1.0f; g.nx = g.ny = g.nz = 1;
	std::vector<uint32_t> start, items;
	if (stat.size() < 32) { w->large_linear.insert(w->large_linear.end(), stat.begin(), stat.end()); stat.clear(); }
	if (!stat.empty()) {
		const uint32_t n = (uint32_t)stat.size();
		const size_t id_bytes = (sizeof(uint32_t) * n + 15) & ~size_t(15);
		{ int r = ensure_stage(w, id_bytes + sizeof(float4) * 2 * (size_t)n); if (r != SGP_OK) return r; }
		memcpy(w->stage_host, stat.data(), sizeof(uint32_t) * n);
		HIP_TRY(hipMemcpyAsync(w->stage_dev, w->stage_host, sizeof(uint32_t) * n, hipMemcpyHostToDevice, w->stream));
		launch_gather_aabbs(d, (const uint32_t*)w->stage_dev, n, (float4*)((char*)w->stage_dev + id_bytes), w->stream);
		HIP_TRY(hipMemcpyAsync((char*)w->stage_host + id_bytes, (char*)w->stage_dev + id_bytes, sizeof(float4) * 2 * (size_t)n, hipMemcpyDeviceToHost, w->stream));
		HIP_TRY(hipStreamSynchronize(w->stream));
		const float4* bb = (const float4*)((char*)w->stage_host + id_bytes);
		std::vector<float> ext(n);
		for (uint32_t k = 0; k < n; ++k) ext[k] = std::max(std::max(bb[2 * k + 1].x - bb[2 * k].x, bb[2 * k + 1].y - bb[2 * k].y), bb[2 * k + 1].z - bb[2 * k].z);
		std::vector<float> sorted_ext(ext);
		std::nth_element(sorted_ext.begin(), sorted_ext.begin() + n / 2, sorted_ext.end());
		float cell = std::max(2.0f * sorted_ext[n / 2], 0.5f);
		if (!(cell < 1.0e30f)) cell = 1.0e30f;
		auto cell_of = [](float x, float o, float inv, int nn) { return std::min(std::max((int)floorf((x - o) * inv), 0), nn - 1); };
		bool placed = false;
		for (int attempt = 0; attempt < 64 && !placed; ++attempt) {
// ... 65 lines not shown
	hipSetDevice(w->device);
	DV& d = w->dv;
	{ int r = upload_sp(w); if (r != SGP_OK) return r; }
	if (!w->ghost_refresh.empty() || !w->cmds.empty()) { int r = flush_event_reset(w); if (r != SGP_OK) return r; }
	if (!w->ghost_refresh.empty()) {
		const size_t bytes = w->ghost_refresh.size() * sizeof(GhostRefresh);
		{ int r = ensure_stage(w, bytes); if (r != SGP_OK) return r; }
		memcpy(w->stage_host, w->ghost_refresh.data(), bytes);
		HIP_TRY(hipMemcpyAsync(w->stage_dev, w->stage_host, bytes, hipMemcpyHostToDevice, w->stream));
		launch_ghost_refresh(d, (const GhostRefresh*)w->stage_dev, (uint32_t)w->ghost_refresh.size(), w->stream);
		HIP_TRY(hipStreamSynchronize(w->stream));
		w->ghost_refresh.clear();
		w->grid_valid = false;
		w->dirty_since_step = true;
	}
	if (w->cmds.empty()) return rebuild_large_grid(w);
	w->grid_valid = false;
	w->dirty_since_step = true;
	w->events_on_device = true;
	const size_t n = w->cmds.size();
	std::vector<uint32_t> order(n);
	for (size_t i = 0; i < n; ++i) order[i] = (uint32_t)i;
	bool ordered = true;
	for (size_t i = 1; i < n && ordered; ++i) ordered = w->cmds[i - 1].id <= w->cmds[i].id;
	if (!ordered) {
		std::vector<uint64_t> keys(n);
		for (size_t i = 0; i < n; ++i) keys[i] = ((uint64_t)w->cmds[i].id << 32) | (uint64_t)i;
		std::sort(keys.begin(), keys.end());
		for (size_t i = 0; i < n; ++i) order[i] = (uint32_t)(keys[i] & 0xFFFFFFFFull);
	}
	const size_t cmd_bytes = n * sizeof(BodyCmd);
	const size_t run_off = (cmd_bytes + 15) & ~size_t(15);
	const size_t total = run_off + (n + 1) * sizeof(uint32_t);
	{ int r = ensure_stage(w, total); if (r != SGP_OK) return r; }
	BodyCmd* hc = (BodyCmd*)w->stage_host;
	uint32_t* hr = (uint32_t*)((char*)w->stage_host + run_off);
	uint32_t n_runs = 0;
	for (size_t i = 0; i < n; ++i) {
		hc[i] = w->cmds[order[i]];
		if (i == 0 || hc[i].id != hc[i - 1].id) hr[n_runs++] = (uint32_t)i;
		if ((hc[i].ops & (CMD_SET_POS | CMD_SET_ROT | CMD_SET_SHAPE)) && hc[i].id < w->hb.size() && (w->hb[hc[i].id].flags & BF_LARGE) && (w->hb[hc[i].id].flags & BF_MOTION_MASK) == SGP_MOTION_STATIC) w->large_dirty = true;
	}
	hr[n_runs] = (uint32_t)n;
	HIP_TRY(hipMemcpyAsync(w->stage_dev, w->stage_host, total, hipMemcpyHostToDevice, w->stream));
	launch_apply_cmds(d, (const BodyCmd*)w->stage_dev, (const uint32_t*)((char*)w->stage_dev + run_off), n_runs, w->stream);
	HIP_TRY(hipStreamSynchronize(w->stream));
	w->cmds.clear();
	return rebuild_large_grid(w);
}

int flush_event_reset(sgp_world* w)
{
	if (!w->ev_reset_pending) return SGP_OK;
	HIP_TRY(hipMemsetAsync(w->dv.evc, 0, sizeof(EventCounters), w->stream));
	w->ev_reset_pending = false;
	return SGP_OK;
}

int collect_events(sgp_world* w, bool counters_fresh)
{
	DV& d = w->dv;
	if (!counters_fresh) {
		if (!w->events_on_device) return SGP_OK;
		if (w->ev_reset_pending) { w->events_on_device = false; return SGP_OK; }
		HIP_TRY(hipMemcpyAsync(w->h_evc, d.evc, sizeof(EventCounters), hipMemcpyDeviceToHost, w->stream));
		HIP_TRY(hipStreamSynchronize(w->stream));
	}
	w->events_on_device = false;
	const EventCounters ec = *w->h_evc;
	if (!(ec.n_activated | ec.n_deactivated | ec.n_water | ec.n_contact_added | ec.n_contact_persisted)) return SGP_OK;
	struct L { uint32_t n_raised, n; uint32_t* dev; const uint32_t* win; std::vector<sgp_body_event>* out; };
	L lists[3] = { { ec.n_activated, std::min(ec.n_activated, d.cap_bodies), d.ev_activated, w->h_evw->ids[0], &w->ev_act },
	               { ec.n_deactivated, std::min(ec.n_deactivated, d.cap_bodies), d.ev_deactivated, w->h_evw->ids[1], &w->ev_deact },
	               { ec.n_water, std::min(ec.n_water, d.cap_bodies), d.ev_water, w->h_evw->ids[2], &w->ev_water } };
	const uint32_t win = std::min(std::min(d.ev_window, SGP_EVENT_WINDOW), d.cap_bodies);
	for (L& l : lists) {
		if (!l.n) continue;
		const uint32_t* ids = l.win;
		if (!counters_fresh || l.n_raised > win) {
			{ int r = ensure_stage(w, sizeof(uint32_t) * l.n); if (r != SGP_OK) return r; }
			HIP_TRY(hipMemcpyAsync(w->stage_host, l.dev, sizeof(uint32_t) * l.n, hipMemcpyDeviceToHost, w->stream));
			HIP_TRY(hipStreamSynchronize(w->stream));
			ids = (const uint32_t*)w->stage_host;
		}
		for (uint32_t k = 0; k < l.n; ++k) { sgp_body_event e; e.id = ids[k]; e._pad = 0; e.userdata = w->hb[ids[k]].userdata; l.out->push_back(e); }
	}
	struct CL { uint32_t n; sgp_contact_event* dev; std::vector<sgp_contact_event>* out; };
	CL cl[2] = { { std::min(ec.n_contact_added, d.cap_contact_events), d.ev_contacts_added, &w->ev_added },
	             { std::min(ec.n_contact_persisted, d.cap_contact_events), d.ev_contacts_persisted, &w->ev_pers } };
	for (CL& l : cl) {
		if (!l.n) continue;
		{ int r = ensure_stage(w, sizeof(sgp_contact_event) * l.n); if (r != SGP_OK) return r; }
		HIP_TRY(hipMemcpyAsync(w->stage_host, l.dev, sizeof(sgp_contact_event) * l.n, hipMemcpyDeviceToHost, w->stream));
		HIP_TRY(hipStreamSynchronize(w->stream));
		const sgp_contact_event* src = (const sgp_contact_event*)w->stage_host;
		for (uint32_t k = 0; k < l.n; ++k) { sgp_contact_event e = src[k];
			while (e.id1 > 0 && (w->hb[e.id1].flags & BF_ALIAS)) --e.id1;
			while (e.id2 > 0 && (w->hb[e.id2].flags & BF_ALIAS)) --e.id2;
			e.id1 = compound_id_of(w, e.id1, nullptr); e.id2 = compound_id_of(w, e.id2, nullptr);
			e.userdata1 = w->hb[e.id1].userdata; e.userdata2 = w->hb[e.id2].userdata; l.out->push_back(e); }
	}
	w->ev_reset_pending = true;
	return SGP_OK;
}


static hipEvent_t pool_event(sgp_world* w)
{
	if (w->event_next == w->event_pool.size()) { hipEvent_t e; hipEventCreate(&e); w->event_pool.push_back(e); }
	return w->event_pool[w->event_next++];
}
struct KScope {
	sgp_world* w; int kc; hipEvent_t a, b; bool on;
	KScope(sgp_world* w_, int kc_) : w(w_), kc(kc_), on(w_->profiling) { if (on) { a = pool_event(w); b = pool_event(w); hipEventRecord(a, w->stream); } }
	~KScope() { if (on) { hipEventRecord(b, w->stream); w->prof.push_back({ kc, a, b }); } }
};
#define STAGE_MARK(i) do { if (w->profiling) hipEventRecord(w->stage_ev[i], w->stream); } while (0)

int read_counters(sgp_world* w)
{
	HIP_TRY(hipMemcpyAsync(w->h_ctr, w->dv.ctr, sizeof(StepCounters), hipMemcpyDeviceToHost, w->stream));
	HIP_TRY(hipStreamSynchronize(w->stream));
	return SGP_OK;
}


static uint32_t bucket_up(uint32_t x)
{
	if (x <= 1024) return 1024;
	uint32_t p = 1; while ((p << 1) <= x) p <<= 1;
	const uint32_t q = p / 4;
	return ((x + q - 1) / q) * q;
}

struct StepPlan {
	uint32_t nb;
	uint32_t rounds;
	uint32_t est_pairs, est_man;
	int      tail_first;
	uint32_t colour_est[SGP_MAX_COLOURS];
	int      water, contact_events, warm_start, vel_iters, pos_iters;
	uint32_t n_vehicles;
	int      veh_cylinder;
	int      has_meshes;
	int      has_hulls;
	int      wake_round;
	int      small_colouring;
	int      small_world;
	int      bp_small;
	int      hc_first;
	uint32_t hc_est;
	int      hc_probe;
	uint32_t hc_probe_est;
	int      tile_solver;
	int      small_pairs;
	int      ev_reset;
	StepParams sp;
};

static void make_plan(const sgp_world* w, StepPlan& p)
{
	memset(&p, 0, sizeof(p));
	p.nb = bucket_up(w->high);
	{
		uint32_t r = 1;
		while (r < 16u && r < w->plan_rounds && w->plan_round_n[r] > SGP_COLOUR_WIDE_MIN) ++r;
		static const uint32_t steps[] = { 1, 2, 3, 4, 6, 8, 12, 16 };
		p.rounds = 16; for (uint32_t k : steps) if (k >= r) { p.rounds = k; break; }
	}
	p.est_pairs = bucket_up(std::max(w->last_pairs + w->last_pairs / 8, 4u * w->high));
	p.est_man = bucket_up(std::max(w->last_manifolds + w->last_manifolds / 8, 2u * w->high));
	int tf = 0;
	while (tf < SGP_OVERFLOW_COLOUR && w->plan_colour_count[tf] > w->tail_threshold) { p.colour_est[tf] = bucket_up(w->plan_colour_count[tf] + w->plan_colour_count[tf] / 8); ++tf; }
	if (tf == 0 && !w->plan_seen && w->high > SGP_SMALL_WORLD_BODIES) {
		for (; tf < 12; ++tf) p.colour_est[tf] = bucket_up(w->high / 2u);
	}
	p.tail_first = tf;
	p.water = w->h_sp->water_enabled; p.contact_events = w->h_sp->contact_events;
	p.warm_start = w->dv.st.warm_start; p.vel_iters = w->dv.st.num_velocity_steps; p.pos_iters = w->dv.st.num_position_steps;
	p.n_vehicles = w->n_vehicles;
	p.veh_cylinder = w->veh_cylinder_seen ? 1 : 0;
	p.has_hulls = w->hulls.size() > 1 ? (w->n_big_hulls ? 2 : 1) : 0;
	p.has_meshes = w->meshes.size() > 1 ? 1 : 0;
	p.wake_round = w->use_wake_round ? 1 : 0;
	p.small_colouring = (w->last_manifolds <= SGP_SMALL_COLOURING_MANIFOLDS && w->high <= SGP_SMALL_WORLD_BODIES) ? 1 : 0;
	p.small_world = (tf == 0 && w->high <= SGP_SMALL_WORLD_BODIES && w->n_vehicles == 0 && w->use_small_world) ? 1 : 0;
	p.small_pairs = (w->n_con <= 384u || w->n_con > 512u) ? 1 : 0;
	p.bp_small = w->bp_dense_last ? 0 : 1;
	p.hc_first = -1;
	if (!p.small_world && w->use_components && w->n_con != 0) {
		uint64_t total = 0, sum = 0;
		for (int c = 0; c < SGP_OVERFLOW_COLOUR; ++c) total += w->plan_colour_count[c];
		for (int c = tf; c < SGP_OVERFLOW_COLOUR; ++c) sum += w->plan_colour_count[c];
		int k = tf;
		const uint64_t budget = w->hc_k < 0 ? w->hc_budget : 1000u;
		const uint64_t fits = (uint64_t)w->n_cus * 256u * 18u / 25u;
		while (k > 0 && (sum + w->plan_colour_count[k - 1]) * 1000u <= total * budget && sum + w->plan_colour_count[k - 1] <= fits) sum += w->plan_colour_count[--k];
		if (w->hc_k >= 0) k = std::min(tf, std::max(k, w->hc_k));
		sum = 0; for (int c = k; c < SGP_OVERFLOW_COLOUR; ++c) sum += w->plan_colour_count[c];
		p.hc_first = k;
		p.hc_est = bucket_up((uint32_t)sum + (uint32_t)(sum / 8));
		p.hc_probe = -1;
		if (w->hc_k >= 0 && w->hc_probe_in == 0 && k > 0 && (sum + w->plan_colour_count[k - 1]) * 1000u <= total * budget && sum + w->plan_colour_count[k - 1] <= fits) {
			p.hc_probe = k - 1;
			const uint64_t ps = sum + w->plan_colour_count[k - 1];
			p.hc_probe_est = bucket_up((uint32_t)ps + (uint32_t)(ps / 8));
		}
		p.tail_first = k;
		int used = 0;
		for (int c = k; c < SGP_OVERFLOW_COLOUR; ++c) used += w->plan_colour_count[c] != 0u;
		if (used < (int)w->hc_min_colours) { p.hc_first = -1; p.hc_probe = -1; p.hc_est = 0; p.hc_probe_est = 0; p.tail_first = tf; }
	}
	p.tile_solver = (w->use_tile_solver && w->dv.ts_nt && !p.small_world && w->n_vehicles == 0 && p.vel_iters > 0 && w->n_con >= w->ts_min_constraints &&
	                 w->high >= SGP_MAX_COLOURS * w->dv.ts_nt && w->last_active <= w->dv.ts_nt * 1536u && !w->h_sp->compact_rows) ? w->use_tile_solver : 0;
	p.ev_reset = w->ev_reset_pending ? 1 : 0;
	p.sp = *w->h_sp;
	p.sp.parity = 0u;
}

static int enqueue_step(sgp_world* w, const StepPlan& p)
{
	const DV& d = w->dv;
	hipStream_t s = w->stream;
	const uint32_t nb = p.nb;
	STAGE_MARK(0);
	{ KScope k(w, KC_MISC); launch_step_begin(d, p.sp, nb, true, p.ev_reset != 0, s); }
	STAGE_MARK(1);
	{ KScope k(w, KC_BP_CELL); launch_bp_bounds(d, nb, s); launch_bp_cell(d, nb, s); }
	{ KScope k(w, KC_BP_SCAN); launch_bp_scan(d, s); }
	{ KScope k(w, KC_BP_SCATTER); launch_bp_scatter_large(d, nb, s); }
	if (p.n_vehicles) { KScope k(w, KC_VEHICLE); launch_vehicle_pre(d, p.veh_cylinder != 0, s); }
	{ KScope k(w, KC_BP_PAIRS); launch_bp_pairs(d, p.bp_small, s); }
	STAGE_MARK(2);
	{ KScope k(w, KC_NARROWPHASE); launch_narrowphase(d, p.est_pairs, s); if (p.has_hulls) launch_narrowphase_hull(d, p.has_hulls == 2, s); if (p.has_meshes) launch_narrowphase_mesh(d, p.has_hulls != 0, s); }
	if (p.wake_round) { KScope k(w, KC_NARROWPHASE); launch_wake_round(d, nb, p.has_hulls, p.has_meshes, s); }
	{ KScope k(w, KC_APPLY_FORCES); launch_pre_solve(d, nb, s); }
	STAGE_MARK(3);
	{ KScope k(w, KC_COLOUR_CLAIM); launch_colour_inherit(d, p.est_man, s); }
	if (p.contact_events) { KScope k(w, KC_MISC); launch_contact_events(d, p.est_man, s); }
	if (p.small_colouring) {
		KScope k(w, KC_COLOUR_COMMIT); launch_colour_finish(d, 0, 1, s);
	} else {
		uint32_t est_unc = p.est_man;
		for (uint32_t round = 0; round < p.rounds; ++round) {
			{ KScope k(w, KC_COLOUR_CLAIM); launch_colour_claim(d, est_unc, round, s); }
			{ KScope k(w, KC_COLOUR_COMMIT); launch_colour_commit(d, est_unc, round, s); }
			if (round >= 1) est_unc = std::max(est_unc - est_unc / 4, 8192u);
		}
		{ KScope k(w, KC_COLOUR_COMMIT); launch_colour_finish(d, p.rounds, 0, s); }
	}
	if (p.tile_solver) {
		{ KScope k(w, KC_COLOUR_COUNT); launch_ts_label(d, nb, s); launch_colour_count_ts(d, p.est_man, s); }
		{ KScope k(w, KC_SETUP); launch_setup_ts(d, p.est_man, s); }
	} else {
		{ KScope k(w, KC_COLOUR_COUNT); launch_colour_count(d, p.est_man, s); }
		{ KScope k(w, KC_SETUP); launch_setup(d, p.est_man, s); }
	}
	if (p.hc_first >= 0 && p.hc_probe >= 0) { KScope k(w, KC_SETUP); launch_hc_probe(d, p.hc_probe, p.hc_probe_est, s); }
	if (p.hc_first >= 0) { KScope k(w, KC_SETUP); launch_hc_build(d, p.hc_first, p.hc_est, s); }
	STAGE_MARK(4);
	auto solve_pass = [&](int mode, int kc) {
		const bool veh_fused = p.n_vehicles && p.tail_first > 0 && mode != 0 && w->fuse_vehicle_solve;
		if (p.n_vehicles && !veh_fused) { KScope k(w, KC_VEHICLE); launch_vehicle_solve(d, mode, s); }
		for (int c = 0; c < p.tail_first; ++c) { KScope k(w, kc); if (c == 0 && veh_fused) launch_solve_colour_veh(d, c, p.colour_est[c], mode, s, (int)p.sp.compact_rows); else launch_solve_colour(d, c, p.colour_est[c], mode, s, (int)p.sp.compact_rows); }
		if (p.hc_first >= 0) { KScope k(w, kc); launch_solve_hc(d, p.hc_first, p.hc_est, mode, s, (int)p.sp.compact_rows); }
		else { KScope k(w, kc); launch_solve_tail(d, p.tail_first, mode, s, (int)p.sp.compact_rows); }
	};
	if (p.small_world) { KScope k(w, KC_SOLVE_VELOCITY); launch_solve_small(d, p.warm_start, p.vel_iters, p.small_pairs, s); }
	else {
		if (p.warm_start) {
			if (p.n_vehicles) { KScope k(w, KC_VEHICLE); launch_vehicle_solve(d, 0, s); }
			{ KScope k(w, KC_WARM_START); launch_warm_bodies(d, nb, s); }
		}
		if (p.tile_solver == 1) { KScope k(w, KC_SOLVE_VELOCITY); launch_ts_solve(d, p.vel_iters, SGP_MAX_COLOURS, s); }
		else if (p.tile_solver == 3 && p.hc_first >= 0) {
			for (int it = 0; it < p.vel_iters; ++it) {
				{ KScope k(w, KC_SOLVE_VELOCITY); launch_ts_solve(d, 1, p.tail_first, s); }
				{ KScope k(w, KC_SOLVE_VELOCITY); launch_solve_hc(d, p.hc_first, p.hc_est, 1, s, (int)p.sp.compact_rows); }
			}
		}
		else for (int it = 0; it < p.vel_iters; ++it) solve_pass(1, KC_SOLVE_VELOCITY);
	}
	STAGE_MARK(5);
	{ KScope k(w, KC_INTEGRATE_POSE); launch_integrate_pose(d, nb, s); }
	STAGE_MARK(6);
	for (int it = 0; it < p.pos_iters; ++it) solve_pass(2, KC_SOLVE_POSITION);
	STAGE_MARK(7);
	{ KScope k(w, KC_FINALIZE); launch_finalize(d, nb, s); }
	for (int r = 0; r < SGP_ISLAND_MARK_ROUNDS; ++r) { KScope k(w, KC_ISLAND_HOOK); launch_island_mark(d, p.est_man, r == 0 ? 1 : 0, s); }
	{ KScope k(w, KC_ISLAND_HOOK); launch_island_hook(d, p.est_man, s); }
	{ KScope k(w, KC_ISLAND_FLAG); launch_island_flag(d, p.est_man, s); }
	{ KScope k(w, KC_SLEEP_APPLY); launch_sleep_apply(d, nb, s); }
	if (p.water) { KScope k(w, KC_BUOYANCY); launch_buoyancy(d, nb, s); }
	{
		KScope k(w, KC_CACHE_BUILD);
		launch_cache_build(d, p.est_man, w->h_ctr_dev, w->h_evw_dev, s);
	}
	STAGE_MARK(8);
	return SGP_OK;
}

static int step_impl(sgp_world* w, float dt, bool final_readback)
{
	if (!(dt > 0.0f)) return fail(SGP_ERR_INVALID, "sgp_world_step: dt must be > 0");
	static const bool timing = getenv("SGP_TIMING") != nullptr;
	static double t_acc[8] = { 0, 0, 0, 0, 0, 0, 0, 0 }; static int t_n = 0; static double t_exit = 0.0;
	auto now = []() { return std::chrono::duration<double, std::micro>(std::chrono::steady_clock::now().time_since_epoch()).count(); };
	const double ts0 = timing ? now() : 0.0;
	{ int r = flush_cmds(w); if (r != SGP_OK) return r; }
	DV& d = w->dv;
	if (w->high == 0) { memset(&w->stats, 0, sizeof(w->stats)); return SGP_OK; }
	if (w->last_active == 0 && !w->dirty_since_step && !w->profiling) {
		sgp_step_stats& st = w->stats;
		const uint32_t nb_ = st.num_bodies;
		uint32_t lc[SGP_NUM_LAYERS]; memcpy(lc, st.layer_counts, sizeof(lc));
		memset(&st, 0, sizeof(st));
		st.num_bodies = nb_; memcpy(st.layer_counts, lc, sizeof(lc)); st.device_bytes = w->device_bytes;
		w->idle_steps++; w->last_step_idle = true; w->steps_taken++;
		return SGP_OK;
	}
	w->last_step_idle = false;
	w->steps_taken++;
	if (w->veh_inputs_dirty && w->n_vehicles) {
		HIP_TRY(hipMemcpyAsync(w->d_veh_inputs, w->veh_inputs.data(), sizeof(sgp_vehicle_input) * w->n_vehicles, hipMemcpyHostToDevice, w->stream));
		w->veh_inputs_dirty = false;
	}
	const double tt0 = timing ? now() : 0.0;
	w->h_sp->dt = dt;
	w->h_sp->compact_rows = ((w->high <= SGP_SMALL_WORLD_BODIES && !w->rows_in_small_worlds) || w->n_con == 0u) ? 0u : (w->n_con >= w->compact_rows_min ? w->rows_mode_large : (w->rows_mode_default == 2u && w->n_con < w->rows_mode2_min ? 1u : w->rows_mode_default));
	StepPlan plan;
	make_plan(w, plan);
	const std::string key((const char*)&plan, sizeof(plan));
	bool launched = false;
	const double ts2 = timing ? now() : 0.0;
	if (w->use_graphs && !w->profiling) {
		auto it = w->graphs.find(key);
		if (it == w->graphs.end()) {
			const uint32_t par = 0u;
			w->plan_repeats[par] = (key == w->last_plan_key[par]) ? w->plan_repeats[par] + 1 : 0;
			if (w->plan_repeats[par] >= (plan.nb <= 2048u ? 1u : 3u)) {
				{ const int r0 = enqueue_step(w, plan); if (r0 != SGP_OK) return r0; w->eager_steps++; launched = true; }
				if (w->graphs.size() >= 16) { for (auto& kv : w->graphs) hipGraphExecDestroy(kv.second); w->graphs.clear(); }
				hipGraph_t g = nullptr; hipGraphExec_t ge = nullptr;
				HIP_TRY(hipStreamBeginCapture(w->capture_stream, hipStreamCaptureModeThreadLocal));
				hipStream_t run_stream = w->stream; w->stream = w->capture_stream;
				const int r = enqueue_step(w, plan);
				w->stream = run_stream;
				const hipError_t e = hipStreamEndCapture(w->capture_stream, &g);
				if (r != SGP_OK) { if (g) hipGraphDestroy(g); return r; }
				if (e != hipSuccess) return fail(SGP_ERR_HIP, "hipStreamEndCapture", e);
				const hipError_t e2 = hipGraphInstantiate(&ge, g, nullptr, nullptr, 0);
				hipGraphDestroy(g);
				if (e2 != hipSuccess) return fail(SGP_ERR_HIP, "hipGraphInstantiate", e2);
				w->graphs.emplace(key, ge);
			}
		}
		else { HIP_TRY(hipGraphLaunch(it->second, w->stream)); launched = true; w->graph_launches++; }
	}
	w->last_plan_key[0] = key;
	if (!launched) { const int r = enqueue_step(w, plan); if (r != SGP_OK) return r; w->eager_steps++; }
	w->sp_uploaded = plan.sp; w->sp_uploaded_valid = true;
	w->events_on_device = true;
	w->ev_reset_pending = false;
	const double tt1 = timing ? now() : 0.0;
	HIP_TRY(hipStreamSynchronize(w->stream));
	const double tt2 = timing ? now() : 0.0;
	if (w->h_ctr->any_awake) w->h_sp->parity ^= 1u;
	w->grid_valid = false;
	w->dirty_since_step = false;
	w->last_active = w->h_ctr->n_active;
	const StepCounters c1 = *w->h_ctr;
	const uint32_t n_con = c1.n_constraints;
	if (plan.tile_solver && c1.ts_error) return fail(SGP_ERR_HIP, "sgp_world_step: the tile solver timed out waiting for a neighbouring tile (a workgroup of the resident launch was not running); set SGP_TILE_SOLVER=0");
	w->n_con = n_con;
	w->last_pairs = c1.n_pairs; w->last_manifolds = c1.n_manifolds;
	w->plan_rounds = c1.rounds_used;
	memcpy(w->plan_round_n, c1.round_n, sizeof(w->plan_round_n));
	for (int c = 0; c < SGP_MAX_COLOURS; ++c) w->plan_colour_count[c] = c1.colour_count[c];
	w->plan_seen = true;
	w->bp_dense_last = c1.bp_dense != 0u;
	if (plan.hc_first >= 0) {
		int k = plan.hc_first;
		if (c1.hc_n_big > 0u) {
			w->hc_bump = (w->hc_since_bump < 32u) ? std::min(2u * w->hc_bump, 8u) : 1u;
			w->hc_since_bump = 0;
			if (c1.hc_n_big > 4096u) w->hc_bump = 8u;
			k = std::min(k + (int)w->hc_bump, (int)SGP_OVERFLOW_COLOUR - 1); w->hc_probe_gap = 64; w->hc_probe_in = 64;
		}
		else if (plan.hc_probe >= 0) {
			if (c1.hc_probe_big == 0u) { k = plan.hc_probe; w->hc_probe_gap = 16; w->hc_probe_in = 16; }
			else { w->hc_probe_gap = std::min(2u * w->hc_probe_gap, 1024u); w->hc_probe_in = w->hc_probe_gap; }
		} else if (w->hc_probe_in) w->hc_probe_in--;
		w->hc_k = k;
		if (w->hc_since_bump < 0xFFFFu) w->hc_since_bump++;
	}
	sgp_step_stats& st = w->stats;
	memset(&st, 0, sizeof(st));
	st.num_bodies = w->n_alive;
	st.num_wake_pairs = std::min(c1.n_wake_pairs, d.cap_wake_pairs);
	st.num_pairs = std::min(c1.n_pairs, d.cap_pairs) + st.num_wake_pairs;
	st.num_manifolds = n_con;
	st.num_contact_points = c1.n_points;
	st.num_colours = c1.n_colours;
	st.num_colour_rounds = c1.rounds_used;
	st.num_overflow_constraints = c1.colour_count[SGP_OVERFLOW_COLOUR];
	st.num_cached_manifolds = c1.n_cached;
	st.num_component_constraints = c1.hc_n; st.num_catch_all_constraints = c1.hc_n_big;
	st.num_deferred_vehicles = c1.veh_deferred;
	st.tile_solver = plan.tile_solver ? (c1.ts_all_adjacent ? 2u : 1u) : 0u;
	st.pairs_dropped = c1.pairs_dropped; st.manifolds_dropped = c1.manifolds_dropped;
	st.device_bytes = w->device_bytes;
	st.num_active = c1.n_active;
	const double ts5 = timing ? now() : 0.0;
	double ts6 = ts5;
	if (final_readback) {
		const size_t a0 = w->ev_act.size(), d0 = w->ev_deact.size();
		{ int r = collect_events(w, true); if (r != SGP_OK) return r; }
		st.num_activated = (uint32_t)(w->ev_act.size() - a0);
		st.num_deactivated = (uint32_t)(w->ev_deact.size() - d0);
		if (timing) ts6 = now();
		memcpy(st.layer_counts, w->layer_counts, sizeof(st.layer_counts));
	}
	if (timing) {
		const double tt3 = now();
		t_acc[0] += tt1 - tt0; t_acc[1] += tt2 - tt1; t_acc[2] += tt3 - tt2; t_n++;
		t_acc[3] += tt0 - ts0; t_acc[4] += ts2 - tt0; t_acc[5] += ts5 - tt2; t_acc[6] += ts6 - ts5; if (t_exit != 0.0) t_acc[7] += ts0 - t_exit;
		if (t_n == 500 || t_n == 100) {
			fprintf(stderr, "[sgp timing] enqueue %.1f us  sync wait %.1f us  post %.1f us; colouring: %u rounds used, %u planned wide, uncoloured at round start:", t_acc[0] / t_n, t_acc[1] / t_n, t_acc[2] / t_n, c1.rounds_used, plan.rounds);
			for (uint32_t r = 1; r < std::min(c1.rounds_used + 1u, 32u); ++r) fprintf(stderr, " %u", c1.round_n[r]);
			fprintf(stderr, "\n");
			fprintf(stderr, "[sgp timing] host parts (us): flush %.1f  plan %.1f  launch %.1f  wait %.1f  stats %.1f  events %.1f  layer counts %.1f  caller %.1f\n",
			        t_acc[3] / t_n, t_acc[4] / t_n, (t_acc[0] - t_acc[4]) / t_n, t_acc[1] / t_n, t_acc[5] / t_n, t_acc[6] / t_n, (t_acc[2] - t_acc[5] - t_acc[6]) / t_n, t_acc[7] / t_n);
			if (t_n == 500) { for (double& a : t_acc) a = 0; t_n = 0; }
		}
		t_exit = now();
	}
	return SGP_OK;
}

// ... 118 lines not shown
```

### substrata_amd/csrc/sgp_world_checkpoint.hip

```cpp
#include "sgp_world_internal.h"

#define CKPT_MAGIC "SGPCKPT"
#define CKPT_FORMAT_VERSION 1u
#define CKPT_MAX_VEHICLES (1u << 20)

struct CkptScalars {
	uint32_t high, n_alive, lg_pending, lg_tombs, lg_static, last_active, last_pairs, last_manifolds, n_con, plan_rounds, n_vehicles, steps_taken;
	uint32_t plan_round_n[32], plan_colour_count[SGP_MAX_COLOURS];
	uint32_t hc_bump, hc_since_bump, hc_probe_in, hc_probe_gap; int32_t hc_k;
	uint32_t large_dirty, large_list_dirty, dirty_since_step, sp_uploaded_valid, plan_seen, bp_dense_last, last_step_idle, veh_cylinder_seen;
	float max_small_radius; uint32_t pad_;
	StepParams h_sp, sp_uploaded; StepCounters h_ctr; EventCounters h_evc; sgp_step_stats stats;
};
struct CkptCompound { uint32_t id; std::vector<uint32_t> ids; std::vector<sgp_compound_child> children; float pos[3]; float rot[4]; };
struct CkptHost {
	CkptScalars s;
	std::vector<HostBody> hb;
	std::vector<uint32_t> free_list, large_ids, large_linear, free_triples, mesh_refs, hull_refs, veh_body;
	std::vector<uint8_t> veh_alive; std::vector<sgp_vehicle_input> veh_inputs;
	std::vector<CkptCompound> compounds;
	std::vector<sgp_body_event> ev_act, ev_deact, ev_water; std::vector<sgp_contact_event> ev_added, ev_pers;
	size_t bytes() const
	{
		size_t b = sizeof(s) + hb.size() * sizeof(HostBody) + 4 * (free_list.size() + large_ids.size() + large_linear.size() + free_triples.size() + mesh_refs.size() + hull_refs.size() + veh_body.size());
		b += veh_alive.size() + veh_inputs.size() * sizeof(sgp_vehicle_input) + (ev_act.size() + ev_deact.size() + ev_water.size()) * sizeof(sgp_body_event) + (ev_added.size() + ev_pers.size()) * sizeof(sgp_contact_event);
		for (const CkptCompound& c : compounds) b += sizeof(CkptCompound) + c.ids.size() * 4 + c.children.size() * sizeof(sgp_compound_child);
		return b;
	}
};
struct CkptShapes {
	uint64_t epoch = 0; uint32_t n_big_hulls = 0;
	std::vector<MeshHeader> meshes; std::vector<float4> mesh_verts; std::vector<uint4> mesh_tris; std::vector<uint32_t> mesh_tri_mat; std::vector<MeshNode> mesh_nodes; std::vector<uint32_t> mesh_field;
	std::vector<sgd_hull> hulls; std::vector<uint32_t> free_mesh_ids, free_hull_ids;
	std::vector<std::pair<uint32_t, uint32_t>> free_vert_ranges, free_tri_ranges, free_node_ranges, free_field_ranges;
	size_t bytes() const
	{
		return meshes.size() * sizeof(MeshHeader) + mesh_verts.size() * 16 + mesh_tris.size() * 16 + mesh_tri_mat.size() * 4 + mesh_nodes.size() * sizeof(MeshNode) + mesh_field.size() * 4 + hulls.size() * sizeof(sgd_hull) +
		       4 * (free_mesh_ids.size() + free_hull_ids.size()) + 8 * (free_vert_ranges.size() + free_tri_ranges.size() + free_node_ranges.size() + free_field_ranges.size());
	}
};

struct CkptCounts { uint32_t high, cache_n, ht_n, n_vehicles, cache_buf; };
struct CkptArray { uint32_t id; void* ptr; size_t alloc, lean; };
struct CkptSeg { uint32_t id; uint32_t pad_; uint64_t bytes, lean, offset; };

struct sgp_checkpoint {
	sgp_world* owner = nullptr; uint64_t owner_serial = 0; int device = 0; hipStream_t stream = nullptr;
	sgp_world_desc desc{};
	bool full = false;
	void* dev = nullptr; size_t dev_cap = 0, dev_used = 0;
	std::vector<CkptSeg> segs; std::vector<void*> seg_ptr;
	CkptHost host;
	std::shared_ptr<const CkptShapes> shapes;
	CkptCounts counts{};
	mutable uint64_t shape_bytes_copied = 0;
	uint64_t world_device_bytes = 0;
};

static inline size_t up16(size_t b) { return (b + 15) & ~size_t(15); }
static inline size_t up256(size_t b) { return (b + 255) & ~size_t(255); }

#define CKPT_UNNAMED_BASE 0x40000000u
struct CkptIds { uint32_t lg_items = 0, vehicles = 0; };
static void for_each_array(sgp_world* w, const CkptCounts& c, std::vector<CkptArray>& out, CkptIds* ids = nullptr)
{
	out.clear();
	const DV& d = w->dv;
	uint32_t id = 0;
	std::unordered_map<void*, int> seen;
	auto add = [&](const void* cp, char kind, size_t stride, size_t alloc_override = 0) {
		++id;
		void* p = const_cast<void*>(cp);
		if (!p) return;
		size_t alloc = alloc_override;
		if (!alloc) { auto it = w->alloc_bytes.find(p); if (it == w->alloc_bytes.end()) return; alloc = it->second; }
		seen[p] = 1;
		size_t lean = 0;
		switch (kind) {
		case 'B': lean = (size_t)c.high * stride; break;
		case 'C': lean = (size_t)c.cache_n * stride; break;
		case 'T': lean = (size_t)c.ht_n * stride; break;
		case 'V': lean = (size_t)c.n_vehicles * stride; break;
		case 'W': lean = alloc; break;
		default: lean = 0; break;
		}
		lean = std::min(up16(lean), alloc & ~size_t(15));
		if (kind == 'W' && (alloc & 15)) lean = alloc;
		out.push_back(CkptArray{ id, p, alloc, lean });
	};
	add(d.pose, 'B', 16 * POSE_F4); add(d.vel, 'B', 16 * VEL_F4); add(d.dyn, 'B', 16); add(d.force, 'B', 16); add(d.torque, 'B', 16);
	add(d.flags, 'B', 4); add(d.aabb_min, 'B', 16); add(d.aabb_max, 'B', 16);
	for (int k = 0; k < 3; ++k) add(d.sleep_s[k], 'B', 16);
	add(d.sleep_timer, 'B', 4); add(d.submerged, 'B', 4); add(d.userdata, 'B', 8);
	add(d.colour_mask, 'B', 8);
	add(d.warm, 'S', 0);
	add(d.claim[0], 'B', 8); add(d.claim[1], 'B', 8);
	add(d.veh_claim, 'B', 8); add(d.veh_epoch, 'W', 0);
	add(d.island, 'B', 4); add(d.island_awake, 'B', 4); add(d.awake_mark, 'B', 4); add(d.export_counts, 'W', 0);
	add(d.cell_hash, 'B', 4);
	add(d.cell_count, 'S', 0); add(d.cell_start, 'S', 0); add(d.cell_fill, 'S', 0); add(d.tile_slot, 'S', 0); add(d.tile_of_slot, 'S', 0);
	add(w->d_large, 'B', 4); add(w->d_lgrid, 'W', 0); add(w->d_lg_start, 'W', 0); add(w->d_lg_items, 'W', 0); if (ids) ids->lg_items = id;
	add(d.mesh_pairs, 'S', 0); add(d.mesh_big, 'S', 0); add(d.hull_pairs, 'S', 0); add(d.hull_work, 'S', 0);
	add(d.sorted_min, 'S', 0); add(d.sorted_max, 'S', 0);
	add(d.grid, 'W', 0); add(d.grid_cells_used, 'S', 0); add(d.bounds_acc, 'S', 0); add(d.scan_block_sums, 'S', 0);
	add(d.pairs, 'S', 0); add(d.wake_pairs, 'S', 0);
	add(d.sleep_label, 'B', 4); add(d.label_wake, 'B', 4); add(d.slot_gen, 'B', 4);
	add(d.man_ab, 'S', 0); add(d.man_n, 'S', 0); add(d.man_colour, 'S', 0); add(d.man_prio, 'S', 0); add(d.man_prev, 'S', 0); add(d.man_slot, 'S', 0);
	add(d.hc_root, 'B', 4); add(d.hc_count, 'B', 4); add(d.hc_base, 'B', 4); add(d.hc_rank, 'S', 0);
	add(d.hc_list, 'S', 0); add(d.hc_entry, 'S', 0); add(d.hc_big_list, 'W', 0);
	add(d.ulist[0], 'S', 0); add(d.ulist[1], 'S', 0);
	for (int k = 0; k < 4; ++k) { add(d.man_p1[k], 'S', 0); add(d.man_p2[k], 'S', 0); }
	add(d.rows, 'S', 0);
	for (uint32_t b = 0; b < 2; ++b) {
		const ConstraintArrays& a = d.ca[b];
		const char k = b == c.cache_buf ? 'C' : 'S';
		add(a.hdr, k, 16); add(a.n_fric, k, 16); add(a.prec, k, 16 * PREC_F4);
		for (int j = 0; j < 4; ++j) { add(a.r1b[j], k, 16); add(a.r2e[j], k, 16); add(a.lam[j], k, 16); add(a.efft[j], k, 8); add(a.loc1[j], k, 16); add(a.loc2[j], k, 16); }
	}
	add(d.ht, 'T', 16); add(d.ht_cur, 'W', 0); add(d.cache_total, 'W', 0); add(d.cstarts, 'W', 0);
	add(d.ctr, 'W', 0); add(d.evc, 'W', 0);
	add(d.ev_activated, 'S', 0); add(d.ev_deactivated, 'S', 0); add(d.ev_water, 'S', 0);
	add(d.ev_contacts_added, 'S', 0); add(d.ev_contacts_persisted, 'S', 0);
	add(w->d_sp, 'W', 0);
	add(w->d_vehicles, 'V', sizeof(sgd_vehicle), w->cap_vehicles ? sizeof(sgd_vehicle) * (size_t)w->cap_vehicles : 0); if (ids) ids->vehicles = id;
	if (w->cap_vehicles) {
		const size_t nc = w->cap_vehicles;
		add(w->d_veh_inputs, 'S', 0, sizeof(sgp_vehicle_input) * nc);
		add(w->d_veh_rows, 'S', 0, sizeof(float4) * 16u * 4u * nc);
		add(w->d_veh_head, 'S', 0, sizeof(float4) * 5u * nc + sizeof(uint32_t) * (nc / 32u + 4u));
	} else id += 3;
	add(w->d_meshes, 'S', 0, sizeof(MeshHeader) * w->cap_mesh_table); add(w->d_hulls, 'S', 0, sizeof(sgd_hull) * w->cap_hull_table);
	add(w->d_mesh_verts, 'S', 0, sizeof(float4) * w->cap_mesh_verts); add(w->d_mesh_tris, 'S', 0, sizeof(uint4) * w->cap_mesh_tris);
	add(w->d_mesh_tri_mat, 'S', 0, sizeof(uint32_t) * w->cap_mesh_tri_mat); add(w->d_mesh_nodes, 'S', 0, sizeof(MeshNode) * w->cap_mesh_nodes);
	add(w->d_mesh_field, 'S', 0, sizeof(uint32_t) * w->cap_mesh_field);
	uint32_t k = 0;
	for (void* p : w->allocs) { if (!seen.count(p)) { auto it = w->alloc_bytes.find(p); if (it != w->alloc_bytes.end()) out.push_back(CkptArray{ CKPT_UNNAMED_BASE + k, p, it->second, it->second }); } ++k; }
}

static void copy_pieces_kernel(sgp_world* w, const std::vector<CkptSeg>& segs, const std::vector<void*>& world_ptr, const std::vector<uint64_t>& bytes, char* buf, bool to_checkpoint)
{
	CkptTable t; t.n = 0; t.start[0] = 0;
	auto flush = [&]() { if (t.n) launch_ckpt_copy(t, w->n_cus, w->stream); t.n = 0; t.start[0] = 0; };
	for (size_t i = 0; i < segs.size(); ++i) {
		if (!world_ptr[i] || !bytes[i]) continue;
		uint64_t done = 0;
		while (done < bytes[i]) {
			const uint64_t room = (uint64_t)0xFFFFFF00u - t.start[t.n];
			const uint64_t units = std::min((bytes[i] - done) / 16, room);
			if (t.n == SGP_CKPT_MAX_SEGS || units == 0) { flush(); continue; }
			char* a = (char*)world_ptr[i] + done; char* b = buf + segs[i].offset + done;
			t.src[t.n] = to_checkpoint ? a : b; t.dst[t.n] = to_checkpoint ? b : a;
			t.start[t.n + 1] = t.start[t.n] + (uint32_t)units; t.n++;
			done += units * 16;
		}
	}
	flush();
}

static int read_device_counts(sgp_world* w, CkptCounts& c)
{
	const DV& d = w->dv;
	{ int r = ensure_stage(w, 64); if (r != SGP_OK) return r; }
	uint32_t* h = (uint32_t*)w->stage_host;
	HIP_TRY(hipMemcpyAsync(h, d.cache_total, 8, hipMemcpyDeviceToHost, w->stream));
	HIP_TRY(hipMemcpyAsync(h + 2, d.ht_cur, 4, hipMemcpyDeviceToHost, w->stream));
	HIP_TRY(hipStreamSynchronize(w->stream));
	c.high = w->high;
	c.cache_buf = (w->h_sp->parity & 1u) ^ 1u;
	c.cache_n = std::min(h[c.cache_buf], d.cap_manifolds);
	c.ht_n = std::min(h[2], d.ht_size);
	c.n_vehicles = w->n_vehicles;
	return SGP_OK;
}

static void grab_host(const sgp_world* w, CkptHost& h)
{
	CkptScalars& s = h.s; memset(&s, 0, sizeof(s));
	s.high = w->high; s.n_alive = w->n_alive; s.lg_pending = w->lg_pending; s.lg_tombs = w->lg_tombs; s.lg_static = w->lg_static; s.last_active = w->last_active;
	s.last_pairs = w->last_pairs; s.last_manifolds = w->last_manifolds; s.n_con = w->n_con; s.plan_rounds = w->plan_rounds; s.n_vehicles = w->n_vehicles; s.steps_taken = w->steps_taken;
	memcpy(s.plan_round_n, w->plan_round_n, sizeof(s.plan_round_n)); memcpy(s.plan_colour_count, w->plan_colour_count, sizeof(s.plan_colour_count));
	s.hc_bump = w->hc_bump; s.hc_since_bump = w->hc_since_bump; s.hc_probe_in = w->hc_probe_in; s.hc_probe_gap = w->hc_probe_gap; s.hc_k = w->hc_k;
	s.large_dirty = w->large_dirty; s.large_list_dirty = w->large_list_dirty; s.dirty_since_step = w->dirty_since_step; s.sp_uploaded_valid = w->sp_uploaded_valid;
	s.plan_seen = w->plan_seen; s.bp_dense_last = w->bp_dense_last; s.last_step_idle = w->last_step_idle; s.veh_cylinder_seen = w->veh_cylinder_seen;
	s.max_small_radius = w->max_small_radius;
	s.h_sp = *w->h_sp; s.sp_uploaded = w->sp_uploaded; s.h_ctr = *w->h_ctr; s.h_evc = *w->h_evc; s.stats = w->stats;
	h.hb.assign(w->hb.begin(), w->hb.begin() + w->high);
	h.free_list = w->free_list; h.large_ids = w->large_ids; h.large_linear = w->large_linear; h.free_triples = w->free_triples; h.mesh_refs = w->mesh_refs; h.hull_refs = w->hull_refs;
	h.veh_body = w->veh_body; h.veh_alive = w->veh_alive; h.veh_inputs = w->veh_inputs;
	h.compounds.clear();
	for (const auto& kv : w->compounds) { CkptCompound c; c.id = kv.first; c.ids = kv.second.ids; c.children = kv.second.children; memcpy(c.pos, kv.second.pos, sizeof(c.pos)); memcpy(c.rot, kv.second.rot, sizeof(c.rot)); h.compounds.push_back(std::move(c)); }
	std::sort(h.compounds.begin(), h.compounds.end(), [](const CkptCompound& a, const CkptCompound& b) { return a.id < b.id; });
	h.ev_act = w->ev_act; h.ev_deact = w->ev_deact; h.ev_water = w->ev_water; h.ev_added = w->ev_added; h.ev_pers = w->ev_pers;
}

static void apply_host(sgp_world* w, const CkptHost& h)
{
	const CkptScalars& s = h.s;
	for (uint32_t i = s.high; i < w->high; ++i) w->hb[i] = HostBody{};
	std::copy(h.hb.begin(), h.hb.end(), w->hb.begin());
	w->high = s.high; w->n_alive = s.n_alive; w->lg_pending = s.lg_pending; w->lg_tombs = s.lg_tombs; w->lg_static = s.lg_static; w->last_active = s.last_active;
	w->last_pairs = s.last_pairs; w->last_manifolds = s.last_manifolds; w->n_con = s.n_con; w->plan_rounds = s.plan_rounds; w->n_vehicles = s.n_vehicles; w->steps_taken = s.steps_taken;
	memcpy(w->plan_round_n, s.plan_round_n, sizeof(s.plan_round_n)); memcpy(w->plan_colour_count, s.plan_colour_count, sizeof(s.plan_colour_count));
	w->hc_bump = s.hc_bump; w->hc_since_bump = s.hc_since_bump; w->hc_probe_in = s.hc_probe_in; w->hc_probe_gap = s.hc_probe_gap; w->hc_k = s.hc_k;
	w->large_dirty = s.large_dirty != 0; w->large_list_dirty = s.large_list_dirty != 0; w->dirty_since_step = s.dirty_since_step != 0; w->sp_uploaded_valid = s.sp_uploaded_valid != 0;
	w->plan_seen = s.plan_seen != 0; w->bp_dense_last = s.bp_dense_last != 0; w->last_step_idle = s.last_step_idle != 0; w->veh_cylinder_seen = s.veh_cylinder_seen != 0;
	w->max_small_radius = s.max_small_radius;
	*w->h_sp = s.h_sp; w->sp_uploaded = s.sp_uploaded; *w->h_ctr = s.h_ctr; *w->h_evc = s.h_evc; w->stats = s.stats;
	w->free_list = h.free_list; w->large_ids = h.large_ids; w->large_linear = h.large_linear; w->free_triples = h.free_triples; w->mesh_refs = h.mesh_refs; w->hull_refs = h.hull_refs;
	w->veh_body = h.veh_body; w->veh_alive = h.veh_alive; w->veh_inputs = h.veh_inputs; w->veh_inputs_dirty = true;
	w->compounds.clear();
	for (const CkptCompound& c : h.compounds) { CompoundRec r; r.ids = c.ids; r.children = c.children; memcpy(r.pos, c.pos, sizeof(r.pos)); memcpy(r.rot, c.rot, sizeof(r.rot)); w->compounds.emplace(c.id, std::move(r)); }
	w->ev_act = h.ev_act; w->ev_deact = h.ev_deact; w->ev_water = h.ev_water; w->ev_added = h.ev_added; w->ev_pers = h.ev_pers;
	w->cmds.clear(); w->ghost_refresh.clear();
	w->events_on_device = false; w->ev_reset_pending = false;
	recount_layers(w);
	w->grid_valid = false;
}

static std::shared_ptr<const CkptShapes> grab_shapes(const sgp_world* w)
{
	auto p = std::make_shared<CkptShapes>();
	p->epoch = w->shape_epoch; p->n_big_hulls = w->n_big_hulls;
	p->meshes = w->meshes; p->mesh_verts = w->mesh_verts; p->mesh_tris = w->mesh_tris; p->mesh_tri_mat = w->mesh_tri_mat; p->mesh_nodes = w->mesh_nodes; p->mesh_field = w->mesh_field;
	p->hulls = w->hulls; p->free_mesh_ids = w->free_mesh_ids; p->free_hull_ids = w->free_hull_ids;
	p->free_vert_ranges = w->free_vert_ranges; p->free_tri_ranges = w->free_tri_ranges; p->free_node_ranges = w->free_node_ranges; p->free_field_ranges = w->free_field_ranges;
	return p;
}
static int apply_shapes(sgp_world* w, const CkptShapes& p)
{
	w->n_big_hulls = p.n_big_hulls;
	w->meshes = p.meshes; w->mesh_verts = p.mesh_verts; w->mesh_tris = p.mesh_tris; w->mesh_tri_mat = p.mesh_tri_mat; w->mesh_nodes = p.mesh_nodes; w->mesh_field = p.mesh_field;
	w->hulls = p.hulls; w->free_mesh_ids = p.free_mesh_ids; w->free_hull_ids = p.free_hull_ids;
	w->free_vert_ranges = p.free_vert_ranges; w->free_tri_ranges = p.free_tri_ranges; w->free_node_ranges = p.free_node_ranges; w->free_field_ranges = p.free_field_ranges;
	return shapes_upload_all(w);
}

static bool holds_ghosts(const sgp_world* w)
{
	if (!w->ghost_map.empty() || !w->ghost_seq.empty() || !w->ghost_refresh.empty() || !w->rec_creates.empty()) return true;
	for (uint32_t i = 0; i < w->high; ++i) if (w->hb[i].ghost) return true;
	return false;
}

static void fill_info(const sgp_checkpoint* cp, sgp_checkpoint_info* o);
static uint64_t blob_size(const sgp_checkpoint* cp);

SGP_API int sgp_world_checkpoint(sgp_world* w, sgp_checkpoint** io)
{
	if (!w || !io) return fail(SGP_ERR_INVALID, "sgp_world_checkpoint: NULL");
	if (*io && ((*io)->owner != w || (*io)->owner_serial != w->serial)) return fail(SGP_ERR_INVALID, "sgp_world_checkpoint: the checkpoint belongs to another world");
	if (holds_ghosts(w)) return fail(SGP_ERR_INVALID, "sgp_world_checkpoint: the world holds ghost bodies (a tiled world keeps state in sgp_tiles and on other ranks: not supported)");
	hipSetDevice(w->device);
	{ int r = flush_cmds(w); if (r != SGP_OK) return r; }
	{ int r = collect_events(w); if (r != SGP_OK) return r; }
	{ int r = flush_event_reset(w); if (r != SGP_OK) return r; }
	CkptCounts c;
	{ int r = read_device_counts(w, c); if (r != SGP_OK) return r; }
	std::vector<CkptArray> arrays;
	for_each_array(w, c, arrays);
	const bool full = w->checkpoint_full;
	std::vector<CkptSeg> segs; std::vector<void*> ptrs; std::vector<uint64_t> bytes;
	size_t total = 0;
	for (const CkptArray& a : arrays) {
		const size_t b = full ? a.alloc : a.lean;
		if (!b) continue;
		segs.push_back(CkptSeg{ a.id, 0u, (uint64_t)b, (uint64_t)a.lean, (uint64_t)total }); ptrs.push_back(a.ptr); bytes.push_back(b);
		total += up256(b);
	}
	sgp_checkpoint* cp = *io;
	const bool created = cp == nullptr;
	if (!cp) { cp = new sgp_checkpoint(); cp->owner = w; cp->owner_serial = w->serial; cp->device = w->device; cp->stream = w->stream; cp->desc = w->desc; }
	if (total > cp->dev_cap) {
		if (cp->dev) { hipFree(cp->dev); cp->dev = nullptr; cp->dev_cap = 0; }
		const size_t nc = up256(total + total / 4 + 4096);
		void* q = nullptr;
		const hipError_t e = hipMalloc(&q, nc);
		if (e != hipSuccess) { if (created) delete cp; else cp->segs.clear(); return fail(SGP_ERR_HIP, "sgp_world_checkpoint: hipMalloc", e); }
		cp->dev = q; cp->dev_cap = nc;
	}
	*io = cp;
	cp->full = full; cp->dev_used = total; cp->segs = segs; cp->seg_ptr = ptrs; cp->counts = c; cp->world_device_bytes = w->device_bytes;
	if (full) {
		for (size_t i = 0; i < segs.size(); ++i) HIP_TRY(hipMemcpyAsync((char*)cp->dev + segs[i].offset, ptrs[i], bytes[i], hipMemcpyDeviceToDevice, w->stream));
	} else {
		std::vector<void*> kp(ptrs);
		for (size_t i = 0; i < segs.size(); ++i) if (bytes[i] & 15) { HIP_TRY(hipMemcpyAsync((char*)cp->dev + segs[i].offset, ptrs[i], bytes[i], hipMemcpyDeviceToDevice, w->stream)); kp[i] = nullptr; }
		copy_pieces_kernel(w, segs, kp, bytes, (char*)cp->dev, true);
// ... 347 lines not shown
```

### substrata_amd/csrc/sgp_world_internal.h

```cpp
#pragma once
#include <hip/hip_runtime.h>
#include <algorithm>
#include <cmath>
#include <cstdio>
#include <cstdlib>
#include <cstring>
#include <string>
#include <vector>
#include <unordered_map>
#include <map>
#include <chrono>
#include <memory>
#include <mutex>
#include <set>
#include "sgp_kernels.h"
#include "sgp_device_vehicle.h"
#include "sgp_hull_build.h"

#define SGP_API extern "C" __attribute__((visibility("default")))

extern thread_local std::string g_last_error;
extern int g_device_count;

inline int fail(int code, const char* what, hipError_t e = hipSuccess)
{
	char buf[512];
	if (e != hipSuccess) snprintf(buf, sizeof(buf), "%s: %s", what, hipGetErrorString(e));
	else snprintf(buf, sizeof(buf), "%s", what);
	g_last_error = buf;
	return code;
}
#define HIP_TRY(expr) do { hipError_t e_ = (expr); if (e_ != hipSuccess) return fail(SGP_ERR_HIP, #expr, e_); } while (0)

inline const char* const k_class_names[KC_COUNT] = {
	"apply_forces", "bp_cell", "bp_scan", "bp_scatter", "bp_pairs", "bp_large", "narrowphase", "wake",
	"colour_claim", "colour_commit", "colour_count", "setup", "warm_start", "solve_velocity",
	"integrate_pose", "solve_position", "finalize", "island_hook", "island_flag", "sleep_apply", "buoyancy",
	"cache_build", "misc", "edit", "gather", "prep_bodies", "vehicle" };


struct HostBody {
	uint32_t flags = 0;
	uint64_t userdata = 0;
	float bound_radius = 0.0f;
	float volume = 0.0f;
	bool ghost = false;
	uint32_t shape_ref = 0;
	uint32_t comp_root = SGP_INVALID_ID;
	uint32_t comp_child = 0;
	uint8_t in_large_ids = 0;
	uint8_t lg_state = 0;
	uint8_t lg_tomb = 0;
};

struct CompoundRec { std::vector<uint32_t> ids; std::vector<sgp_compound_child> children; float pos[3]; float rot[4]; };

struct ProfEvent { int kc; hipEvent_t a, b; };

struct sgp_world {
	sgp_world_desc desc;
	int device = 0;
	hipStream_t stream = nullptr;
	hipStream_t capture_stream = nullptr;
	DV dv;
	std::vector<void*> allocs;
	std::unordered_map<void*, size_t> alloc_bytes;
	bool checkpoint_full = false;
	uint64_t serial = 0;
	uint64_t shape_epoch = 0, shape_epoch_counter = 0;
	std::shared_ptr<const struct CkptShapes> shape_snapshot;
	uint32_t steps_taken = 0;
	uint64_t device_bytes = 0;
	std::vector<HostBody> hb;
	std::vector<uint32_t> free_list;
	uint32_t high = 0, n_alive = 0;
	std::vector<uint32_t> large_ids; bool large_dirty = false;
	uint32_t lg_pending = 0, lg_tombs = 0; bool large_list_dirty = false;
	std::vector<uint32_t> large_linear;
	LargeGrid* d_lgrid = nullptr; uint32_t* d_lg_start = nullptr; uint32_t* d_lg_items = nullptr; uint32_t cap_lg_items = 0; uint32_t lg_static = 0;
	uint32_t* d_large = nullptr; uint32_t cap_large = 0;
	float max_small_radius = 0.0f;
	uint32_t last_export = 0;
	std::unordered_map<uint64_t, uint64_t> ghost_map;
	std::vector<uint4> rec_creates;
	uint32_t ghost_gen = 0; bool ghost_map_stale = false; uint64_t ghost_seq_version = 1;
	std::vector<GhostRefresh> ghost_refresh;
	std::vector<std::pair<uint64_t, uint32_t>> ghost_seq;
	std::unordered_map<uint32_t, CompoundRec> compounds;
	std::vector<BodyCmd> cmds;
	void* stage_dev = nullptr; size_t stage_dev_bytes = 0;
	void* stage_host = nullptr; size_t stage_host_bytes = 0;
	void* view_host = nullptr; size_t view_host_bytes = 0;
	StepCounters* h_ctr = nullptr; StepCounters* h_ctr_dev = nullptr;
	EventWindow* h_evw = nullptr; EventWindow* h_evw_dev = nullptr; EventCounters* h_evc = nullptr;
	bool ev_reset_pending = false;
	uint32_t layer_counts[SGP_NUM_LAYERS] = { 0 };
	bool dirty_since_step = true;
	bool events_on_device = true;
	StepParams sp_uploaded; bool sp_uploaded_valid = false;
	uint32_t last_active = 0xFFFFFFFFu;
	StepParams* h_sp = nullptr; StepParams* d_sp = nullptr;
	std::map<std::string, hipGraphExec_t> graphs;
	std::string last_plan_key[2]; uint32_t plan_repeats[2] = { 0, 0 };
	bool use_graphs = true; bool use_small_world = true; bool use_wake_round = true; uint32_t tail_threshold = 256;
	uint32_t rows_mode_default = 2;
	bool rows_in_small_worlds = false;
	uint32_t rows_mode2_min = 65536;
	uint32_t rows_mode_large = 2;
	uint32_t compact_rows_min = 1000000;
	int use_tile_solver = 0;
	uint32_t ts_min_constraints = 16384;
	bool use_components = true; uint32_t hc_budget = 160; uint32_t n_cus = 256; uint32_t hc_min_colours = 4; int hc_k = -1; uint32_t hc_bump = 1, hc_since_bump = 0xFFFFu; uint32_t hc_probe_in = 8, hc_probe_gap = 16;
	bool bp_dense_last = false;
	bool plan_seen = false;
	uint32_t graph_launches = 0, eager_steps = 0, idle_steps = 0;
	RayMailbox* ray_mb = nullptr; bool ray_server_on = false; bool ray_server_enabled = true; uint32_t ray_seq = 0, ray_gen = 0;
	uint32_t ray_server_launches = 0, ray_server_rays = 0;
	int query_path = 0; uint32_t sq_wave_max_n = 32; float sq_pairs_per_query = 2.0f, sq_out_per_query = 4.0f; uint32_t sq_reruns = 0, sq_last_n = 0, sq_last_out = 0, sq_last_pairs = 0;
	float sc_pairs_per_cast = 2.0f; uint32_t sc_reruns = 0, sc_capped = 0;
	bool last_step_idle = false;
	bool grid_valid = false;
	std::vector<MeshHeader> meshes; std::vector<float4> mesh_verts; std::vector<uint4> mesh_tris; std::vector<uint32_t> mesh_tri_mat; std::vector<MeshNode> mesh_nodes;
	MeshHeader* d_meshes = nullptr; float4* d_mesh_verts = nullptr; uint4* d_mesh_tris = nullptr; uint32_t* d_mesh_tri_mat = nullptr; MeshNode* d_mesh_nodes = nullptr;
	size_t cap_mesh_verts = 0, cap_mesh_tris = 0, cap_mesh_tri_mat = 0, cap_mesh_nodes = 0;
	std::vector<uint32_t> mesh_field; uint32_t* d_mesh_field = nullptr; size_t cap_mesh_field = 0;
	std::vector<uint32_t> mesh_refs, hull_refs, free_mesh_ids, free_hull_ids;
	uint32_t n_big_hulls = 0;
	std::vector<std::pair<uint32_t, uint32_t>> free_vert_ranges, free_tri_ranges, free_node_ranges, free_field_ranges;
	size_t cap_mesh_table = 0, cap_hull_table = 0;
	std::vector<uint32_t> free_triples;
	std::vector<sgd_hull> hulls; sgd_hull* d_hulls = nullptr;
	sgd_vehicle* d_vehicles = nullptr; sgp_vehicle_input* d_veh_inputs = nullptr; uint32_t cap_vehicles = 0, n_vehicles = 0;
	float4* d_veh_rows = nullptr; float4* d_veh_head = nullptr;
	bool fuse_vehicle_solve = true;
	std::vector<uint8_t> veh_alive; std::vector<uint32_t> veh_body; std::vector<sgp_vehicle_input> veh_inputs; bool veh_inputs_dirty = false;
	bool veh_cylinder_seen = false;
	std::vector<sgp_body_event> ev_act, ev_deact, ev_water;
	std::vector<sgp_contact_event> ev_added, ev_pers;
	sgp_step_stats stats;
	uint32_t last_pairs = 0, last_manifolds = 0, n_con = 0;
	uint32_t plan_rounds = 12;
	uint32_t plan_round_n[32] = { 0, ~0u, ~0u, ~0u, ~0u, ~0u, ~0u, ~0u };
	uint32_t plan_colour_count[SGP_MAX_COLOURS] = { 0 };
	uint32_t table_alloc = 0, ht_alloc = 0;
	bool profiling = false;
	std::vector<ProfEvent> prof;
	std::vector<hipEvent_t> event_pool; size_t event_next = 0;
	hipEvent_t stage_ev[SGP_NUM_STAGES + 1];
	bool stage_ev_ok = false;
};

template <typename T> inline int dev_alloc(sgp_world* w, T*& p, size_t n)
{
	void* q = nullptr;
	const size_t bytes = (std::max<size_t>(n, 1) * sizeof(T) + 15) & ~size_t(15);
	hipError_t e = hipMalloc(&q, bytes);
	if (e != hipSuccess) return fail(SGP_ERR_HIP, "hipMalloc", e);
	e = hipMemsetAsync(q, 0, bytes, w->stream);
	if (e != hipSuccess) return fail(SGP_ERR_HIP, "hipMemsetAsync", e);
	w->allocs.push_back(q);
	w->alloc_bytes[q] = bytes;
	w->device_bytes += bytes;
	p = (T*)q;
	return SGP_OK;
}
#define DEV_ALLOC(ptr, n) do { int r_ = dev_alloc(w, ptr, n); if (r_ != SGP_OK) return r_; } while (0)

inline int ensure_stage(sgp_world* w, size_t bytes)
{
	if (bytes > w->stage_dev_bytes) {
		if (w->stage_dev) { hipStreamSynchronize(w->stream); hipFree(w->stage_dev); w->device_bytes -= w->stage_dev_bytes; }
		size_t nb = std::max<size_t>(bytes, 1 << 16); nb = nb + nb / 2;
		HIP_TRY(hipMalloc(&w->stage_dev, nb));
		w->stage_dev_bytes = nb; w->device_bytes += nb;
	}
	if (bytes > w->stage_host_bytes) {
		if (w->stage_host) { hipStreamSynchronize(w->stream); hipHostFree(w->stage_host); }
		size_t nb = std::max<size_t>(bytes, 1 << 16); nb = nb + nb / 2;
		HIP_TRY(hipHostMalloc(&w->stage_host, nb, hipHostMallocDefault));
		w->stage_host_bytes = nb;
	}
	return SGP_OK;
}

inline uint32_t next_pow2(uint32_t v) { uint32_t p = 1; while (p < v) p <<= 1; return p; }


static inline bool finite3(const float* v) { return std::isfinite(v[0]) && std::isfinite(v[1]) && std::isfinite(v[2]); }
static inline bool finite4(const float* v) { return finite3(v) && std::isfinite(v[3]); }
#define REQUIRE_FINITE(cond, what) do { if (!(cond)) return fail(SGP_ERR_INVALID, what ": non-finite argument"); } while (0)
static inline bool counts_in_layer(uint32_t f) { return (f & (BF_ALIVE | BF_ALIAS)) == BF_ALIVE; }
static inline void set_body_flags(sgp_world* w, HostBody& b, uint32_t f)
{
	if (counts_in_layer(b.flags)) w->layer_counts[(b.flags & BF_LAYER_MASK) >> BF_LAYER_SHIFT]--;
	if (counts_in_layer(f)) w->layer_counts[(f & BF_LAYER_MASK) >> BF_LAYER_SHIFT]++;
	b.flags = f;
}
static inline void recount_layers(sgp_world* w)
{
	memset(w->layer_counts, 0, sizeof(w->layer_counts));
	for (uint32_t i = 0; i < w->high; ++i) if (counts_in_layer(w->hb[i].flags)) w->layer_counts[(w->hb[i].flags & BF_LAYER_MASK) >> BF_LAYER_SHIFT]++;
}
static inline bool live(const sgp_world* w, uint32_t id) { return w && id < w->high && (w->hb[id].flags & BF_ALIVE); }

static BodyCmd blank_cmd(uint32_t id, uint32_t ops) { BodyCmd c; memset(&c, 0, sizeof(c)); c.id = id; c.ops = ops; return c; }
static inline uint32_t compound_id_of(const sgp_world* w, uint32_t id, uint32_t* sub_out)
{
	const HostBody& b = w->hb[id];
	if (b.comp_root == SGP_INVALID_ID) { if (sub_out) *sub_out = 0; return id; }
	if (sub_out) *sub_out = b.comp_child;
	return b.comp_root;
}

void ray_server_stop(sgp_world* w);
void invalidate_graphs(sgp_world* w);
int flush_cmds(sgp_world* w);
int collect_events(sgp_world* w, bool counters_fresh = false);
int flush_event_reset(sgp_world* w);
int read_counters(sgp_world* w);
uint64_t world_register(); void world_unregister(uint64_t serial); bool world_alive(uint64_t serial);
int ensure_vehicle_capacity(sgp_world* w, uint32_t need);
int shapes_upload_all(sgp_world* w);
int ensure_query_grid(sgp_world* w);
int add_one(sgp_world* w, const sgp_body_desc* d, uint32_t* id_out, bool ghost);
int book_record_body(sgp_world* w, uint32_t* flags_io, uint64_t userdata, float radius, float volume, bool ghost, uint32_t* id_out);
```

### substrata_amd/csrc/sgp_world_tiles.hip

```cpp
#include "sgp_world_internal.h"


SGP_API int sgp_world_export_boundary(sgp_world* w, const float lo[3], const float hi[3], float margin, sgp_ghost_record* out, uint32_t cap, uint32_t* n_out)
{
	if (!w || !n_out) return fail(SGP_ERR_INVALID, "sgp_world_export_boundary: NULL");
	hipSetDevice(w->device);
	static const bool timing = getenv("SGP_TIMING") != nullptr;
	const auto t0 = std::chrono::steady_clock::now();
	{ int r = flush_cmds(w); if (r != SGP_OK) return r; }
	const uint32_t lim = std::min(cap, w->dv.cap_bodies);
	{ int r = ensure_stage(w, sizeof(sgp_ghost_record) * std::max(lim, 1u)); if (r != SGP_OK) return r; }
	launch_export_boundary(w->dv, w->high, make_float3(lo[0], lo[1], lo[2]), make_float3(hi[0], hi[1], hi[2]), margin,
	                       (sgp_ghost_record*)w->stage_dev, lim, &w->dv.ctr->n_export, w->stream);
	uint32_t guess = out ? std::min(lim, w->last_export + w->last_export / 4 + 64u) : 0u;
	if (guess) HIP_TRY(hipMemcpyAsync(w->stage_host, w->stage_dev, sizeof(sgp_ghost_record) * guess, hipMemcpyDeviceToHost, w->stream));
	{ int r = read_counters(w); if (r != SGP_OK) return r; }
	const uint32_t n = w->h_ctr->n_export, m = std::min(n, lim);
	w->last_export = n;
	const auto t1 = std::chrono::steady_clock::now();
	if (m && out) {
		if (m > guess) {
			HIP_TRY(hipMemcpyAsync((char*)w->stage_host + sizeof(sgp_ghost_record) * guess, (char*)w->stage_dev + sizeof(sgp_ghost_record) * guess,
			                       sizeof(sgp_ghost_record) * (m - guess), hipMemcpyDeviceToHost, w->stream));
			HIP_TRY(hipStreamSynchronize(w->stream));
// ... 93 lines not shown
				w->grid_valid = false; w->dirty_since_step = true;
				return SGP_OK;
			}
			w->ghost_refresh.resize(n);
			for (uint32_t k = 0; k < n; ++k) {
				GhostRefresh& c = w->ghost_refresh[k];
				c.id = w->ghost_seq[k].second;
				memcpy(c.pos, in[k].pos, 12); memcpy(c.rot, in[k].rot, 16); memcpy(c.linv, in[k].lin_vel, 12); memcpy(c.angv, in[k].ang_vel, 12);
			}
			return SGP_OK;
		}
	}
	w->ghost_refresh.clear();
	w->cmds.reserve(w->cmds.size() + n);
	std::vector<std::pair<uint64_t, uint32_t>> seq(n, std::pair<uint64_t, uint32_t>(0, SGP_INVALID_ID));
	std::vector<uint32_t> gone;
	auto refresh_cmd = [&](uint32_t id, uint32_t rec_k) {
		if (dev) return;
		const sgp_ghost_record& r = in[rec_k];
		BodyCmd c = blank_cmd(id, CMD_SET_POS | CMD_SET_ROT | CMD_SET_VEL | CMD_ACTIVATE);
		memcpy(c.pos, r.pos, 12); memcpy(c.rot, r.rot, 16); memcpy(c.linv, r.lin_vel, 12); memcpy(c.angv, r.ang_vel, 12);
		w->cmds.push_back(c);
	};
	bool ascending = true;
	for (uint32_t k = 1; k < n && ascending; ++k) ascending = in.gid(k - 1) < in.gid(k);
	for (size_t k = 1; k < w->ghost_seq.size() && ascending; ++k) ascending = w->ghost_seq[k - 1].first < w->ghost_seq[k].first;
	if (ascending) {
		const std::vector<std::pair<uint64_t, uint32_t>>& old = w->ghost_seq;
		size_t i = 0, j = 0;
		while (i < n || j < old.size()) {
			if (j == old.size() || (i < n && in.gid(i) < old[j].first)) {
				uint32_t id; const int r = make_ghost_at(w, in, (uint32_t)i, &id);
				if (r != SGP_OK && r != SGP_ERR_REJECTED) return r;
				seq[i] = std::make_pair(in.gid(i), r == SGP_OK ? id : SGP_INVALID_ID); ++i;
			} else if (i == n || old[j].first < in.gid(i)) {
				if (old[j].second != SGP_INVALID_ID && live(w, old[j].second)) gone.push_back(old[j].second);
				++j;
			} else {
				uint32_t id = old[j].second;
				if (id != SGP_INVALID_ID && live(w, id)) refresh_cmd(id, (uint32_t)i);
				else { const int r = make_ghost_at(w, in, (uint32_t)i, &id); if (r != SGP_OK && r != SGP_ERR_REJECTED) return r; if (r != SGP_OK) id = SGP_INVALID_ID; }
				seq[i] = std::make_pair(in.gid(i), id); ++i; ++j;
			}
		}
		w->ghost_map_stale = true;
	} else {
		if (w->ghost_map_stale) {
			w->ghost_map.clear();
			for (const auto& e : w->ghost_seq) if (e.second != SGP_INVALID_ID) w->ghost_map[e.first] = ((uint64_t)w->ghost_gen << 32) | e.second;
			w->ghost_map_stale = false;
		}
		const uint32_t gen = ++w->ghost_gen;
		for (uint32_t k = 0; k < n; ++k) {
			seq[k].first = in.gid(k);
			auto it = w->ghost_map.find(in.gid(k));
			if (it != w->ghost_map.end() && live(w, (uint32_t)it->second)) {
				const uint32_t id = (uint32_t)it->second;
				refresh_cmd(id, k);
				it->second = ((uint64_t)gen << 32) | id;
				seq[k].second = id;
				continue;
			}
			uint32_t id; const int r = make_ghost_at(w, in, k, &id);
			if (r == SGP_OK) { w->ghost_map[in.gid(k)] = ((uint64_t)gen << 32) | id; seq[k].second = id; }
			else if (r != SGP_ERR_REJECTED) return r;
		}
		for (auto it = w->ghost_map.begin(); it != w->ghost_map.end();) {
			if ((uint32_t)(it->second >> 32) != gen) { if (live(w, (uint32_t)it->second)) gone.push_back((uint32_t)it->second); it = w->ghost_map.erase(it); }
			else ++it;
		}
	}
	std::sort(gone.begin(), gone.end());
	for (uint32_t id : gone) sgp_body_remove(w, id);
	w->ghost_seq.swap(seq);
	w->ghost_seq_version++;
	if (dev && n) {
		{ int r = flush_cmds(w); if (r != SGP_OK) return r; }
		{ int r = upload_ghost_ids(w, dev, skip, n_all); if (r != SGP_OK) return r; }
		{ int r = flush_event_reset(w); if (r != SGP_OK) return r; }
		launch_ghost_refresh_records(w->dv, dev->d_recs, *dev->d_ids, n_all, w->stream);
		w->grid_valid = false; w->dirty_since_step = true;
	}
	return SGP_OK;
}

SGP_API int sgp_world_import_ghosts(sgp_world* w, const sgp_ghost_record* in, uint32_t n)
{
	if (!w || (!in && n)) return fail(SGP_ERR_INVALID, "sgp_world_import_ghosts: NULL");
	hipSetDevice(w->device);
	return import_ghosts_impl(w, in, n, nullptr);
}


static inline bool in_box(const float* p, const float* lo, const float* hi, float pad)
{
	return p[0] >= lo[0] - pad && p[0] < hi[0] + pad && p[1] >= lo[1] - pad && p[1] < hi[1] + pad && p[2] >= lo[2] - pad && p[2] < hi[2] + pad;
}

SGP_API int sgp_tiles_route(const sgp_ghost_record* recs, uint32_t n, uint32_t my_rank, const float* boxes, uint32_t n_tiles, float pad,
                            sgp_ghost_record* send_out, uint32_t cap, uint32_t* send_counts,
                            uint32_t* emigrant_ids, uint32_t emigrant_cap, uint32_t* n_emigrants)
{
	if ((!recs && n) || !boxes || !send_counts || !n_emigrants || my_rank >= n_tiles) return fail(SGP_ERR_INVALID, "sgp_tiles_route: bad arguments");
	const float* mylo = boxes + 6 * (size_t)my_rank; const float* myhi = mylo + 3;
	std::vector<uint8_t> emig(n, 0);
	uint32_t ne = 0;
	for (uint32_t k = 0; k < n; ++k) {
		bool taker = false;
		for (uint32_t r = 0; r < n_tiles && !taker; ++r) if (r != my_rank) taker = in_box(recs[k].pos, boxes + 6 * (size_t)r, boxes + 6 * (size_t)r + 3, 0.0f);
		if (n_tiles > 1 && taker && (recs[k].motion_type & 0xFFu) == SGP_MOTION_DYNAMIC && !(recs[k].flags & SGP_GHOST_FLAG_CHASSIS) && !in_box(recs[k].pos, mylo, myhi, 0.0f)) {
			emig[k] = 1;
			if (ne < emigrant_cap && emigrant_ids) emigrant_ids[ne] = (uint32_t)(recs[k].global_id & 0xFFFFFFFFull);
			++ne;
		}
	}
	*n_emigrants = ne;
	if (ne > emigrant_cap) return fail(SGP_ERR_CAPACITY, "sgp_tiles_route: emigrant list too small");
	uint32_t w = 0;
	for (uint32_t r = 0; r < n_tiles; ++r) {
		send_counts[r] = 0;
		if (r == my_rank) continue;
		const float* lo = boxes + 6 * (size_t)r; const float* hi = lo + 3;
		for (uint32_t k = 0; k < n; ++k) {
			if (!in_box(recs[k].pos, lo, hi, pad)) continue;
			if (w >= cap || !send_out) return fail(SGP_ERR_CAPACITY, "sgp_tiles_route: send buffer too small");
			sgp_ghost_record o = recs[k];
			o.global_id |= (uint64_t)my_rank << 40;
			if (emig[k]) o.motion_type = SGP_MOTION_DYNAMIC | SGP_GHOST_TAKE_OWNERSHIP;
			send_out[w++] = o;
			++send_counts[r];
		}
	}
	return SGP_OK;
}

SGP_API int sgp_tiles_split(const sgp_ghost_record* in, uint32_t n, const float lo[3], const float hi[3],
                            sgp_ghost_record* ghosts_out, uint32_t* n_ghosts, sgp_ghost_record* immigrants_out, uint32_t* n_immigrants)
{
	if ((!in && n) || !lo || !hi || !n_ghosts || !n_immigrants || (n && (!ghosts_out || !immigrants_out))) return fail(SGP_ERR_INVALID, "sgp_tiles_split: bad arguments");
	uint32_t g = 0, m = 0;
	for (uint32_t k = 0; k < n; ++k) {
		if (in[k].motion_type & SGP_GHOST_TAKE_OWNERSHIP) { if (in_box(in[k].pos, lo, hi, 0.0f)) immigrants_out[m++] = in[k]; }
		else ghosts_out[g++] = in[k];
	}
	*n_ghosts = g; *n_immigrants = m;
	return SGP_OK;
}


SGP_API int sgp_world_device_array(sgp_world* w, int which, void** dev_ptr_out, uint32_t* count_out)
{
	if (!w || !dev_ptr_out) return fail(SGP_ERR_INVALID, "sgp_world_device_array: NULL");
	void* p = nullptr;
	switch (which) { case 0: p = w->dv.pose; break; case 1: p = w->dv.vel; break;
	default: return fail(SGP_ERR_INVALID, "sgp_world_device_array: bad index"); }
	*dev_ptr_out = p;
	if (count_out) *count_out = w->high;
	return SGP_OK;
}

SGP_API int sgp_world_stream(sgp_world* w, void** stream_out)
{
	if (!w || !stream_out) return fail(SGP_ERR_INVALID, "sgp_world_stream: NULL");
	ray_server_stop(w);
	*stream_out = (void*)w->stream;
	return SGP_OK;
}

#include <dlfcn.h>

namespace {
typedef struct { char internal[128]; } sgp_nccl_unique_id;
typedef void* sgp_nccl_comm;
enum { SGP_NCCL_UINT8 = 1, SGP_NCCL_UINT32 = 3 };
struct RcclApi {
	void* lib = nullptr; bool tried = false;
	int (*GetUniqueId)(sgp_nccl_unique_id*) = nullptr;
	int (*CommInitRank)(sgp_nccl_comm*, int, sgp_nccl_unique_id, int) = nullptr;
	int (*CommDestroy)(sgp_nccl_comm) = nullptr;
	int (*AllGather)(const void*, void*, size_t, int, sgp_nccl_comm, hipStream_t) = nullptr;
	int (*Send)(const void*, size_t, int, int, sgp_nccl_comm, hipStream_t) = nullptr;
	int (*Recv)(void*, size_t, int, int, sgp_nccl_comm, hipStream_t) = nullptr;
	int (*GroupStart)() = nullptr;
	int (*GroupEnd)() = nullptr;
	const char* (*GetErrorString)(int) = nullptr;
	int (*CommCount)(sgp_nccl_comm, int*) = nullptr;
};
RcclApi g_rccl;

#if __has_include(<rccl/rccl.h>)
}
#include <rccl/rccl.h>
#include <type_traits>
namespace {
template <class A, class B> constexpr bool sgp_abi_same_arg()
{
	return sizeof(A) == sizeof(B) && std::is_pointer<A>::value == std::is_pointer<B>::value && std::is_class<A>::value == std::is_class<B>::value &&
	       (std::is_integral<A>::value || std::is_enum<A>::value) == (std::is_integral<B>::value || std::is_enum<B>::value);
}
template <class F, class G> struct sgp_abi_same : std::false_type {};
template <class R, class... A, class S, class... B> struct sgp_abi_same<R (*)(A...), S (*)(B...)>
{
	template <bool same_arity, class Dummy = void> struct args { static constexpr bool value = false; };
	template <class Dummy> struct args<true, Dummy> { static constexpr bool value = (sgp_abi_same_arg<A, B>() && ... && true); };
	static constexpr bool value = sgp_abi_same_arg<R, S>() && args<sizeof...(A) == sizeof...(B)>::value;
};
#define SGP_CHECK_RCCL(member, fn) static_assert(sgp_abi_same<decltype(RcclApi::member), decltype(&fn)>::value, "hand-declared prototype of " #fn " does not match <rccl/rccl.h>")
SGP_CHECK_RCCL(GetUniqueId, ncclGetUniqueId);
SGP_CHECK_RCCL(CommInitRank, ncclCommInitRank);
SGP_CHECK_RCCL(CommDestroy, ncclCommDestroy);
SGP_CHECK_RCCL(AllGather, ncclAllGather);
SGP_CHECK_RCCL(Send, ncclSend);
SGP_CHECK_RCCL(Recv, ncclRecv);
SGP_CHECK_RCCL(GroupStart, ncclGroupStart);
SGP_CHECK_RCCL(GroupEnd, ncclGroupEnd);
SGP_CHECK_RCCL(GetErrorString, ncclGetErrorString);
SGP_CHECK_RCCL(CommCount, ncclCommCount);
static_assert(sizeof(ncclUniqueId) == sizeof(sgp_nccl_unique_id) && NCCL_UNIQUE_ID_BYTES == SGP_TILES_UNIQUE_ID_BYTES, "ncclUniqueId is 128 bytes");
static_assert((int)ncclUint8 == SGP_NCCL_UINT8 && (int)ncclUint32 == SGP_NCCL_UINT32 && (int)ncclSuccess == 0, "ncclDataType_t / ncclResult_t values");
#endif

bool rccl_load()
{
	if (g_rccl.tried) return g_rccl.lib != nullptr;
	g_rccl.tried = true;
	if (const char* explicit_lib = getenv("SGP_RCCL_LIBRARY")) { if (*explicit_lib) g_rccl.lib = dlopen(explicit_lib, RTLD_NOW | RTLD_GLOBAL); if (*explicit_lib && !g_rccl.lib) return false; }
	const char* names[] = { "librccl.so.1", "librccl.so", "/opt/rocm/lib/librccl.so.1", "/opt/rocm/lib/librccl.so" };
	if (!g_rccl.lib) for (const char* n : names) { g_rccl.lib = dlopen(n, RTLD_NOW | RTLD_NOLOAD | RTLD_GLOBAL); if (g_rccl.lib) break; }
	if (!g_rccl.lib) for (const char* n : names) { g_rccl.lib = dlopen(n, RTLD_NOW | RTLD_GLOBAL); if (g_rccl.lib) break; }
	if (!g_rccl.lib) return false;
	bool ok = true;
	auto sym = [&](const char* name) { void* p = dlsym(g_rccl.lib, name); if (!p) ok = false; return p; };
	g_rccl.GetUniqueId = (int (*)(sgp_nccl_unique_id*))sym("ncclGetUniqueId");
	g_rccl.CommInitRank = (int (*)(sgp_nccl_comm*, int, sgp_nccl_unique_id, int))sym("ncclCommInitRank");
	g_rccl.CommDestroy = (int (*)(sgp_nccl_comm))sym("ncclCommDestroy");
	g_rccl.AllGather = (int (*)(const void*, void*, size_t, int, sgp_nccl_comm, hipStream_t))sym("ncclAllGather");
	g_rccl.Send = (int (*)(const void*, size_t, int, int, sgp_nccl_comm, hipStream_t))sym("ncclSend");
	g_rccl.Recv = (int (*)(void*, size_t, int, int, sgp_nccl_comm, hipStream_t))sym("ncclRecv");
	g_rccl.GroupStart = (int (*)())sym("ncclGroupStart");
	g_rccl.GroupEnd = (int (*)())sym("ncclGroupEnd");
	g_rccl.GetErrorString = (const char* (*)(int))sym("ncclGetErrorString");
	if (!ok) { g_rccl.lib = nullptr; return false; }
	g_rccl.CommCount = (int (*)(sgp_nccl_comm, int*))dlsym(g_rccl.lib, "ncclCommCount");
	return true;
}
int rccl_fail(const char* what, int rc)
{
	g_last_error = std::string(what) + ": " + (g_rccl.GetErrorString ? g_rccl.GetErrorString(rc) : "RCCL error");
	return SGP_ERR_HIP;
}
#define RCCL_TRY(call, what) do { const int rc_ = (call); if (rc_ != 0) return rccl_fail(what, rc_); } while (0)
}

#define SGP_TILES_EMIG_INLINE 512

struct sgp_tiles {
	sgp_world* w = nullptr;
	uint32_t rank = 0, n_tiles = 1;
	TileRoute route;
	sgp_nccl_comm comm = nullptr;
	uint32_t* d_block_counts = nullptr; uint32_t* d_block_offsets = nullptr; uint32_t cap_blocks = 0;
	char* d_ctl = nullptr;
	uint32_t host_status = ROUTE_OK;
	int test_fail_growth = 0;
	sgp_ghost_record* d_send = nullptr; uint32_t cap_send = 0;
	sgp_ghost_record* d_recv = nullptr; uint32_t cap_recv = 0;
	uint32_t* d_emig = nullptr; uint32_t cap_emig = 0;
	uint32_t* d_seq_ids = nullptr; uint32_t cap_seq = 0; uint64_t ids_version = 0;
	char* h_ctl = nullptr; sgp_ghost_record* h_recv = nullptr; uint32_t cap_h_recv = 0;
	uint4* d_keys = nullptr; uint32_t cap_keys = 0; void* h_keys = nullptr; uint32_t cap_h_keys = 0;
	uint4* d_aux = nullptr; uint32_t cap_aux = 0; void* h_aux = nullptr;
	uint4* d_create = nullptr; uint32_t cap_create = 0; uint4* h_create = nullptr; uint32_t cap_h_create = 0;
	bool host_records_only = false;
	std::vector<uint32_t> recv_counts, recv_offsets;
	std::vector<uint64_t> seq_gids;
	bool seq_valid = false;
	sgp_tiles_stats stats;
	std::vector<sgp_migration> migrations;
	uint32_t* d_hist = nullptr; uint32_t* d_hist_all = nullptr; uint32_t* h_hist = nullptr;
};
static size_t tiles_row_words(uint32_t n_tiles) { return (size_t)n_tiles + 2; }
static size_t tiles_matrix_off() { return sizeof(RouteHeader); }
static size_t tiles_row_off(uint32_t n_tiles) { return tiles_matrix_off() + sizeof(uint32_t) * (size_t)n_tiles * tiles_row_words(n_tiles); }
static size_t tiles_emig_off(uint32_t n_tiles) { return tiles_row_off(n_tiles) + sizeof(uint32_t) * tiles_row_words(n_tiles); }
static size_t tiles_ctl_bytes(uint32_t n_tiles) { return tiles_emig_off(n_tiles) + sizeof(uint32_t) * SGP_TILES_EMIG_INLINE; }

SGP_API int sgp_tiles_unique_id(uint8_t out[SGP_TILES_UNIQUE_ID_BYTES])
{
	if (!out) return fail(SGP_ERR_INVALID, "sgp_tiles_unique_id: NULL");
	if (!rccl_load()) return fail(SGP_ERR_HIP, "sgp_tiles_unique_id: RCCL (librccl.so) not found");
	sgp_nccl_unique_id id;
	RCCL_TRY(g_rccl.GetUniqueId(&id), "ncclGetUniqueId");
	static_assert(sizeof(id) == SGP_TILES_UNIQUE_ID_BYTES, "ncclUniqueId is 128 bytes");
	memcpy(out, &id, sizeof(id));
	return SGP_OK;
}

template <typename T> static int tiles_grow(sgp_world* w, T*& p, uint32_t& cap, uint32_t need, bool keep = false)
{
	if (need <= cap) return SGP_OK;
	const uint32_t nc = std::max(need + need / 2, 4096u);
	T* q = nullptr;
	HIP_TRY(hipMalloc((void**)&q, sizeof(T) * (size_t)nc));
	if (p) { HIP_TRY(hipStreamSynchronize(w->stream)); if (keep && cap) HIP_TRY(hipMemcpy(q, p, sizeof(T) * (size_t)cap, hipMemcpyDeviceToDevice)); hipFree(p); }
	p = q; cap = nc;
	return SGP_OK;
}

SGP_API int sgp_tiles_destroy(sgp_tiles* t)
{
// ... 501 lines not shown
```

Before: 547.3 steps/s.

## Pack hard-constraint solver data into contiguous per-workgroup layout built once per step

```diff
diff --git a/substrata_amd/csrc/sgp_dev_solve.h b/substrata_amd/csrc/sgp_dev_solve.h
--- a/substrata_amd/csrc/sgp_dev_solve.h
+++ b/substrata_amd/csrc/sgp_dev_solve.h
@@ -243,6 +243,85 @@
 	ph.np = np_col & 0xFF;
 #pragma unroll
 	for (int i = 0; i < 4; ++i) if (i == 0 || i < ph.np) ph.loc[i] = V3(side ? CUR(d).loc2[i][slot] : CUR(d).loc1[i][slot]);
+}
+template <typename T> SGP_DEV T hc_plane(const T* plane, uint32_t byte_off) { return *(const T*)((const char*)plane + byte_off); }
+template <int ROWS> SGP_DEV void half_load_packed(const DV& d, uint32_t e, uint32_t cap, int side, int np_col, uint32_t body, ConHalf& h)
+{
+	h.body = body;
+	h.nf = d.hc_pnf[e];
+	h.np_col = np_col;
+	const int np = np_col & 0xFF;
+	const size_t C = d.hc_pack_cap, S2 = 2 * (size_t)cap;
+	const uint32_t at = (2u * e + (uint32_t)side) * 16u, e16 = e * 16u, e8 = e * 8u;
+	if (ROWS == 2) {
+		const sym33 I = body_world_inv_inertia_rec(d, body);
+		const v3 n = V3(h.nf);
+		h.t1 = v3_normalized_perpendicular(n);
+		const v3 t2 = v3_cross(n, h.t1);
+#pragma unroll
+		for (int i = 0; i < 4; ++i) {
+			if (i == 0 || i < np) {
+				const float4 r4 = hc_plane(d.hc_prow + (size_t)i * S2, at);
+				const float2 et = hc_plane(d.hc_pefft + (size_t)i * C, e8);
+				const v3 r = V3(r4);
+				h.c[i][0] = v3_cross(r, n); h.c[i][1] = v3_cross(r, h.t1); h.c[i][2] = v3_cross(r, t2);
+#pragma unroll
+				for (int a = 0; a < 3; ++a) h.iv[i][a] = sym33_mul(I, h.c[i][a]);
+				const float ow = lane_swap1(r4.w);
+				h.eff[i][0] = side ? r4.w : ow; h.bias[i] = side ? ow : r4.w;
+				h.eff[i][1] = et.x; h.eff[i][2] = et.y;
+				h.lam[i] = V3(hc_plane(d.hc_plam + (size_t)i * C, e16));
+			}
+		}
+		return;
+	}
+	if (ROWS == 1) {
+		const sym33 I = body_world_inv_inertia_rec(d, body);
+#pragma unroll
+		for (int i = 0; i < 4; ++i) {
+			if (i == 0 || i < np) {
+#pragma unroll
+				for (int a = 0; a < 3; ++a) {
+					const float4 c4 = hc_plane(d.hc_prow + (size_t)(i * 3 + a) * S2, at);
+					h.c[i][a] = V3(c4); h.iv[i][a] = sym33_mul(I, V3(c4));
+					const float ow = lane_swap1(c4.w);
+					h.eff[i][a] = side ? c4.w : ow;
+					if (a == 0) h.bias[i] = side ? ow : c4.w;
+				}
+				h.lam[i] = V3(hc_plane(d.hc_plam + (size_t)i * C, e16));
+			}
+		}
+		h.t1 = v3_normalized_perpendicular(V3(h.nf));
+		return;
+	}
+#pragma unroll
+	for (int i = 0; i < 4; ++i) {
+		if (i == 0 || i < np) {
+#pragma unroll
+			for (int a = 0; a < 3; ++a) {
+				const float4 c4 = hc_plane(d.hc_prow + (size_t)((i * 3 + a) * 2) * S2, at);
+				const float4 i4 = hc_plane(d.hc_prow + (size_t)((i * 3 + a) * 2 + 1) * S2, at);
+				h.c[i][a] = V3(c4); h.iv[i][a] = V3(i4);
+				const float ow = lane_swap1(c4.w);
+				h.eff[i][a] = side ? c4.w : ow;
+				if (a == 0) h.bias[i] = side ? ow : c4.w;
+				if (i == 0 && a < 2) {
+					const float oi = lane_swap1(i4.w);
+					if (a == 0) { h.t1.x = side ? oi : i4.w; h.t1.y = side ? i4.w : oi; } else h.t1.z = side ? oi : i4.w;
+				}
+			}
+			h.lam[i] = V3(hc_plane(d.hc_plam + (size_t)i * C, e16));
+		}
+	}
+}
+SGP_DEV void pos_half_load_packed(const DV& d, uint32_t e, int side, int np_col, PosHalf& ph)
+{
+	ph.nf = d.hc_pnf[e];
+	ph.np = np_col & 0xFF;
+	const size_t C2 = 2 * (size_t)d.hc_pack_cap;
+	const uint32_t at = (2u * e + (uint32_t)side) * 16u;
+#pragma unroll
+	for (int i = 0; i < 4; ++i) if (i == 0 || i < ph.np) ph.loc[i] = V3(hc_plane(d.hc_ploc + (size_t)i * C2, at));
 }
 SGP_DEV void pos_half_solve(const DV& d, const PosHalf& ph, int side, float4* rec, v3 ii)
 {
diff --git a/substrata_amd/csrc/sgp_k_solve.hip b/substrata_amd/csrc/sgp_k_solve.hip
--- a/substrata_amd/csrc/sgp_k_solve.hip
+++ b/substrata_amd/csrc/sgp_k_solve.hip
@@ -385,13 +385,16 @@
 	}
 }
 
-__global__ void __launch_bounds__(HC_WG_PAIRS) k_hc_sort(DV d)
+#define HC_TABLE 1024
+template <int LAYOUT> __global__ void __launch_bounds__(HC_WG_PAIRS) k_hc_sort(DV d, int rows, uint32_t cap)
 {
 	__shared__ uint32_t s_cnt[SGP_MAX_COLOURS], s_first[SGP_MAX_COLOURS];
 	__shared__ uint4 s_slot[HC_WG_PAIRS];
+	__shared__ uint32_t s_key[LAYOUT ? HC_TABLE : 1], s_pos[LAYOUT ? HC_TABLE : 1], s_n;
 	const uint32_t entries = d.ctr->hc_entries;
 	for (uint32_t e0 = blockIdx.x * HC_WG_PAIRS; e0 < entries; e0 += gridDim.x * HC_WG_PAIRS) {
 		if (threadIdx.x < SGP_MAX_COLOURS) s_cnt[threadIdx.x] = 0u;
+		if constexpr (LAYOUT != 0) { for (uint32_t i = threadIdx.x; i < HC_TABLE; i += HC_WG_PAIRS) s_key[i] = HC_NONE; if (threadIdx.x == 0) s_n = 0u; }
 		__syncthreads();
 		const uint32_t slot = d.hc_list[e0 + threadIdx.x];
 		const uint4 hd = slot != HC_NONE ? con_hdr(CUR(d), slot) : make_uint4(0u, 0u, 0u, 0u);
@@ -409,12 +412,109 @@
 		__syncthreads();
 		s_slot[s_first[col] + rank] = make_uint4(slot, (uint32_t)npc, ab.x, ab.y);
 		__syncthreads();
-		d.hc_entry[e0 + threadIdx.x] = s_slot[threadIdx.x];
-		__syncthreads();
-	}
-}
-
-#define HC_TABLE 1024
+		const uint4 en = s_slot[threadIdx.x];
+		d.hc_entry[e0 + threadIdx.x] = en;
+		if constexpr (LAYOUT != 0) {
+			const bool packed = e0 + HC_WG_PAIRS <= cap;
+			const bool used = en.x != HC_NONE;
+			unsigned long long present = 0ull;
+			if (threadIdx.x < 64) present = __ballot(threadIdx.x < SGP_OVERFLOW_COLOUR && s_cnt[threadIdx.x] != 0u);
+			uint32_t at[2] = { 0u, 0u };
+			if (used) {
+#pragma unroll
+				for (int sd = 0; sd < 2; ++sd) {
+					const uint32_t body = sd ? en.w : en.z;
+					uint32_t a = uf_prio(body) & (HC_TABLE - 1);
+					for (;;) {
+						const uint32_t old = atomicCAS(&s_key[a], HC_NONE, body);
+						if (old == HC_NONE) {
+							const uint32_t pos = atomicAdd(&s_n, 1u);
+							s_pos[a] = pos;
+							if (packed) d.hc_bodies[2 * (size_t)e0 + pos] = body;
+							break;
+						}
+						if (old == body) break;
+						a = (a + 1) & (HC_TABLE - 1);
+					}
+					at[sd] = a;
+				}
+			}
+			__syncthreads();
+			if (threadIdx.x == 0) d.hc_share[e0 / HC_WG_PAIRS] = make_uint4(s_n, (uint32_t)present, (uint32_t)(present >> 32), 0u);
+			if (packed && used) {
+				const uint32_t e = e0 + threadIdx.x, k = en.x;
+				d.hc_local[e] = s_pos[at[0]] | (s_pos[at[1]] << 16);
+				const int np = (int)en.y & 0xFF;
+				const size_t C = d.hc_pack_cap, S2 = 2 * (size_t)cap, st = d.cap_manifolds;
+				d.hc_pnf[e] = CUR(d).n_fric[k];
+#pragma unroll
+				for (int i = 0; i < 4; ++i) {
+					if (i == 0 || i < np) {
+						d.hc_plam[(size_t)i * C + e] = CUR(d).lam[i][k];
+						d.hc_ploc[(size_t)i * 2 * C + 2 * (size_t)e] = CUR(d).loc1[i][k];
+						d.hc_ploc[(size_t)i * 2 * C + 2 * (size_t)e + 1] = CUR(d).loc2[i][k];
+						if (rows == 2) {
+							d.hc_prow[(size_t)i * S2 + 2 * (size_t)e] = CUR(d).r1b[i][k];
+							d.hc_prow[(size_t)i * S2 + 2 * (size_t)e + 1] = CUR(d).r2e[i][k];
+							d.hc_pefft[(size_t)i * C + e] = CUR(d).efft[i][k];
+						} else {
+#pragma unroll
+							for (int a = 0; a < 3; ++a) {
+								const float4* p = axis_rows(d, k, i, a);
+#pragma unroll
+								for (int sd = 0; sd < 2; ++sd) {
+									if (rows == 1) d.hc_prow[(size_t)(i * 3 + a) * S2 + 2 * (size_t)e + sd] = p[(size_t)sd * st];
+									else {
+										d.hc_prow[(size_t)((i * 3 + a) * 2) * S2 + 2 * (size_t)e + sd] = p[(size_t)sd * st];
+										d.hc_prow[(size_t)((i * 3 + a) * 2 + 1) * S2 + 2 * (size_t)e + sd] = p[(size_t)(2 + sd) * st];
+									}
+								}
+							}
+						}
+					}
+				}
+			}
+		}
+		__syncthreads();
+	}
+}
+
+template <int MODE, int ROWS> SGP_DEV void hc_catch_all(const DV& d, int first_colour, int n_colours, int side, uint32_t pair, uint32_t& s_ticket)
+{
+	const uint32_t n_big = d.ctr->hc_n_big;
+	const uint32_t ofirst = d.cstarts[SGP_OVERFLOW_COLOUR], ocount = d.cstarts[SGP_OVERFLOW_COLOUR + 1] - ofirst;
+	if (n_big == 0u && ocount == 0u) return;
+	__syncthreads();
+	if (threadIdx.x == 0) { __threadfence(); s_ticket = atomicAdd(&d.ctr->hc_done, 1u); }
+	__syncthreads();
+	if (s_ticket != gridDim.x - 1u) return;
+	if (threadIdx.x == 0) d.ctr->hc_done = 0u;
+	__threadfence();
+	if (n_big != 0u && n_big <= (uint32_t)HC_BIG_LIST) {
+		uint32_t mine[4]; int mcol[4]; int cnt = 0;
+		for (uint32_t e = pair; e < n_big; e += HC_WG_PAIRS) { const uint32_t k = d.hc_big_list[e]; mine[cnt] = k; mcol[cnt] = (int)((con_npc(CUR(d), k) >> 8) & 0xFF); ++cnt; }
+		for (int c = first_colour; c < n_colours; ++c) {
+#pragma unroll
+			for (int j = 0; j < 4; ++j) if (j < cnt && mcol[j] == c) { if (MODE == 1) solve_velocity_pair_t<VEL_F4, ROWS>(d, mine[j], side, d.vel); else solve_position_pair(d, mine[j], side); }
+			__syncthreads();
+		}
+	} else
+	for (int c = first_colour; c < n_colours && n_big != 0u; ++c) {
+		const uint32_t cb = d.cstarts[c], ce = d.cstarts[c + 1];
+		for (uint32_t k = cb + pair; k < ce; k += HC_WG_PAIRS) {
+			if (!(con_npc(CUR(d), k) & NPCOL_CATCH_ALL)) continue;
+			if (MODE == 1) solve_velocity_pair_t<VEL_F4, ROWS>(d, k, side, d.vel); else solve_position_pair(d, k, side);
+		}
+		__syncthreads();
+	}
+	if (ocount == 0u || threadIdx.x >= 2u) return;
+	uint64_t last = 0; bool have_last = false;
+	for (uint32_t it = 0; it < ocount; ++it) {
+		const uint32_t bslot = overflow_next(d, ofirst, ocount, last, have_last);
+		if (MODE == 1) solve_velocity_pair_t<VEL_F4, ROWS>(d, bslot, side, d.vel); else solve_position_pair(d, bslot, side);
+	}
+}
+
 template <int MODE, int ROWS = -1> __global__ void __launch_bounds__(HC_TPB) k_solve_hc(const StepCounters* ctr_pre, const uint4* hc_entry_pre, DV d, int first_colour)
 {
 	constexpr int RS = MODE == 1 ? 2 : 3;
@@ -468,38 +568,77 @@
 			g[0] = s_rec[RS * at]; g[1] = s_rec[RS * at + 1];
 		}
 	}
-	const uint32_t n_big = d.ctr->hc_n_big;
-	const uint32_t ofirst = d.cstarts[SGP_OVERFLOW_COLOUR], ocount = d.cstarts[SGP_OVERFLOW_COLOUR + 1] - ofirst;
-	if (n_big == 0u && ocount == 0u) return;
-	__syncthreads();
-	if (threadIdx.x == 0) { __threadfence(); s_ticket = atomicAdd(&d.ctr->hc_done, 1u); }
-	__syncthreads();
-	if (s_ticket != gridDim.x - 1u) return;
-	if (threadIdx.x == 0) d.ctr->hc_done = 0u;
-	__threadfence();
-	if (n_big != 0u && n_big <= (uint32_t)HC_BIG_LIST) {
-		uint32_t mine[4]; int mcol[4]; int cnt = 0;
-		for (uint32_t e = pair; e < n_big; e += HC_WG_PAIRS) { const uint32_t k = d.hc_big_list[e]; mine[cnt] = k; mcol[cnt] = (int)((con_npc(CUR(d), k) >> 8) & 0xFF); ++cnt; }
+	hc_catch_all<MODE, ROWS>(d, first_colour, n_colours, side, pair, s_ticket);
+}
+
+template <int MODE, int ROWS> __global__ void __launch_bounds__(HC_TPB) k_solve_hcl(const StepCounters* ctr_pre, const uint4* hc_entry_pre, DV d, int colour_arg, uint32_t cap)
+{
+	constexpr int RS = MODE == 1 ? 2 : 3;
+	__shared__ float4 s_rec[HC_TPB * RS];
+	__shared__ uint32_t s_ticket;
+	const int first_colour = colour_arg & 0xFF;
+	const bool last_pass = (colour_arg & 0x100) != 0;
+	const int side = (int)(threadIdx.x & 1u);
+	const uint32_t pair = threadIdx.x >> 1;
+	const uint32_t entries = ctr_pre->hc_entries;
+	const int n_colours = (int)ctr_pre->n_colours;
+	for (uint32_t e0 = blockIdx.x * HC_WG_PAIRS; e0 < entries && e0 + HC_WG_PAIRS <= cap; e0 += gridDim.x * HC_WG_PAIRS) {
+		__syncthreads();
+		const uint32_t e = e0 + pair;
+		const uint4 entry = hc_entry_pre[e];
+		const uint4 share = d.hc_share[e0 / HC_WG_PAIRS];
+		const unsigned long long present = (unsigned long long)share.y | ((unsigned long long)share.z << 32);
+		const uint32_t slot = entry.x;
+		const bool mine = slot != HC_NONE;
+		const int my_col = mine ? ((int)entry.y >> 8) & 0xFF : -1;
+		const uint32_t n_list = min(share.x, (uint32_t)HC_TPB);
+		const uint32_t list_body = d.hc_bodies[2 * (size_t)e0 + threadIdx.x];
+		const uint32_t local2 = d.hc_local[e];
+		ConHalf h; PosHalf ph;
+		if (mine) { if (MODE == 1) half_load_packed<ROWS>(d, e, cap, side, (int)entry.y, side ? entry.w : entry.z, h); else pos_half_load_packed(d, e, side, (int)entry.y, ph); }
+		const uint32_t at = (side ? local2 >> 16 : local2) & (uint32_t)(HC_TPB - 1);
+		if (threadIdx.x < n_list) {
+			const float4* g = (MODE == 1 ? d.vel + VEL_F4 * (size_t)list_body : d.pose + POSE_F4 * (size_t)list_body);
+			s_rec[RS * threadIdx.x] = g[0]; s_rec[RS * threadIdx.x + 1] = g[1];
+			if (MODE != 1) s_rec[RS * threadIdx.x + 2] = g[2];
+		}
+		if (MODE == 1) h.body = at;
+		__syncthreads();
 		for (int c = first_colour; c < n_colours; ++c) {
-#pragma unroll
-			for (int j = 0; j < 4; ++j) if (j < cnt && mcol[j] == c) { if (MODE == 1) solve_velocity_pair_t<VEL_F4, ROWS>(d, mine[j], side, d.vel); else solve_position_pair(d, mine[j], side); }
+			if (!((present >> c) & 1ull)) continue;
+			if (my_col == c) { if (MODE == 1) half_solve<2>(h, side, s_rec, d.dbg_flags); else pos_half_solve(d, ph, side, s_rec + RS * at, V3(s_rec[RS * at + 2])); }
 			__syncthreads();
 		}
-	} else
-	for (int c = first_colour; c < n_colours && n_big != 0u; ++c) {
-		const uint32_t cb = d.cstarts[c], ce = d.cstarts[c + 1];
-		for (uint32_t k = cb + pair; k < ce; k += HC_WG_PAIRS) {
-			if (!(con_npc(CUR(d), k) & NPCOL_CATCH_ALL)) continue;
-			if (MODE == 1) solve_velocity_pair_t<VEL_F4, ROWS>(d, k, side, d.vel); else solve_position_pair(d, k, side);
-		}
-		__syncthreads();
-	}
-	if (ocount == 0u || threadIdx.x >= 2u) return;
-	uint64_t last = 0; bool have_last = false;
-	for (uint32_t it = 0; it < ocount; ++it) {
-		const uint32_t bslot = overflow_next(d, ofirst, ocount, last, have_last);
-		if (MODE == 1) solve_velocity_pair_t<VEL_F4, ROWS>(d, bslot, side, d.vel); else solve_position_pair(d, bslot, side);
-	}
+		if (MODE == 1 && my_col >= 0 && side == 0) {
+			const int np = h.np_col & 0xFF;
+			const size_t C = d.hc_pack_cap;
+#pragma unroll
+			for (int i = 0; i < 4; ++i) {
+				if (i < np) {
+					const float4 l = F4(h.lam[i], 0.0f);
+					d.hc_plam[(size_t)i * C + (e0 + pair)] = l;
+					if (last_pass) CUR(d).lam[i][slot] = l;
+				}
+			}
+		}
+		if (threadIdx.x < n_list && s_rec[RS * threadIdx.x].w > 0.0f) {
+			float4* g = (MODE == 1 ? d.vel + VEL_F4 * (size_t)list_body : d.pose + POSE_F4 * (size_t)list_body);
+			g[0] = s_rec[RS * threadIdx.x]; g[1] = s_rec[RS * threadIdx.x + 1];
+		}
+	}
+	for (uint32_t e0 = blockIdx.x * HC_WG_PAIRS; e0 < entries; e0 += gridDim.x * HC_WG_PAIRS) {
+		if (e0 + HC_WG_PAIRS <= cap) continue;
+		const uint4 entry = hc_entry_pre[e0 + pair];
+		const uint4 share = d.hc_share[e0 / HC_WG_PAIRS];
+		const unsigned long long present = (unsigned long long)share.y | ((unsigned long long)share.z << 32);
+		const int my_col = entry.x != HC_NONE ? ((int)entry.y >> 8) & 0xFF : -1;
+		for (int c = first_colour; c < n_colours; ++c) {
+			if (!((present >> c) & 1ull)) continue;
+			if (my_col == c) { if (MODE == 1) solve_velocity_pair_t<VEL_F4, ROWS>(d, entry.x, side, d.vel); else solve_position_pair(d, entry.x, side); }
+			__syncthreads();
+		}
+	}
+	hc_catch_all<MODE, ROWS>(d, first_colour, n_colours, side, pair, s_ticket);
 }
 
 #define SMALL_LDS_BODIES 2048
@@ -734,14 +873,17 @@
 	}
 	else hipLaunchKernelGGL(k_solve_tail, dim3(1), dim3(512), 0, s, d, first_colour, mode);
 }
-void launch_hc_build(const DV& d, int first_colour, uint32_t est, hipStream_t s)
+static uint32_t hc_pack_cap_for(const DV& d, int layout, int compact_rows) { return !layout ? 0u : (compact_rows == 0 ? d.hc_pack_cap0 : d.hc_pack_cap); }
+void launch_hc_build(const DV& d, int first_colour, uint32_t est, hipStream_t s, int layout, int compact_rows)
 {
 	const uint32_t blocks = std::max(1u, std::min(1024u, (est + est / 8 + TPB - 1) / TPB));
 	hipLaunchKernelGGL(k_hc_hook, dim3(blocks), dim3(TPB), 0, s, d, first_colour);
 	hipLaunchKernelGGL(k_hc_count, dim3(blocks), dim3(TPB), 0, s, d, first_colour);
 	hipLaunchKernelGGL(k_hc_alloc, dim3(blocks), dim3(TPB), 0, s, d, first_colour);
 	hipLaunchKernelGGL(k_hc_scatter, dim3(blocks), dim3(TPB), 0, s, d, first_colour);
-	hipLaunchKernelGGL(k_hc_sort, dim3(std::max(1u, std::min(2048u, (2u * est + HC_CLASSES * HC_WG_PAIRS) / HC_WG_PAIRS))), dim3(HC_WG_PAIRS), 0, s, d);
+	const dim3 sort_blocks(std::max(1u, std::min(2048u, (2u * est + HC_CLASSES * HC_WG_PAIRS) / HC_WG_PAIRS)));
+	if (layout) hipLaunchKernelGGL(k_hc_sort<1>, sort_blocks, dim3(HC_WG_PAIRS), 0, s, d, compact_rows, hc_pack_cap_for(d, layout, compact_rows));
+	else hipLaunchKernelGGL(k_hc_sort<0>, sort_blocks, dim3(HC_WG_PAIRS), 0, s, d, 0, 0u);
 }
 void launch_hc_probe(const DV& d, int probe_colour, uint32_t probe_est, hipStream_t s)
 {
@@ -751,9 +893,20 @@
 	hipLaunchKernelGGL(k_hc_probe, dim3(pb), dim3(TPB), 0, s, d, probe_colour);
 	hipLaunchKernelGGL(k_hc_init, dim3(pb), dim3(TPB), 0, s, d, probe_colour);
 }
-void launch_solve_hc(const DV& d, int first_colour, uint32_t est, int mode, hipStream_t s, int compact_rows)
+void launch_solve_hc(const DV& d, int first_colour, uint32_t est, int mode, hipStream_t s, int compact_rows, int layout, bool last_velocity_pass)
 {
 	const uint32_t blocks = std::max(1u, std::min(2048u, (2u * est + HC_CLASSES * HC_WG_PAIRS) / HC_WG_PAIRS));
+	if (layout) {
+		const uint32_t cap = hc_pack_cap_for(d, layout, compact_rows);
+		const int colour_arg = first_colour | (mode == 1 && last_velocity_pass ? 0x100 : 0);
+		if (mode == 1) {
+			if (compact_rows == 2) hipLaunchKernelGGL((k_solve_hcl<1, 2>), dim3(blocks), dim3(HC_TPB), 0, s, (const StepCounters*)d.ctr, (const uint4*)d.hc_entry, d, colour_arg, cap);
+			else if (compact_rows) hipLaunchKernelGGL((k_solve_hcl<1, 1>), dim3(blocks), dim3(HC_TPB), 0, s, (const StepCounters*)d.ctr, (const uint4*)d.hc_entry, d, colour_arg, cap);
+			else hipLaunchKernelGGL((k_solve_hcl<1, 0>), dim3(blocks), dim3(HC_TPB), 0, s, (const StepCounters*)d.ctr, (const uint4*)d.hc_entry, d, colour_arg, cap);
+		}
+		else hipLaunchKernelGGL((k_solve_hcl<2, -1>), dim3(blocks), dim3(HC_TPB), 0, s, (const StepCounters*)d.ctr, (const uint4*)d.hc_entry, d, colour_arg, cap);
+		return;
+	}
 	if (mode == 1) {
 		if (compact_rows == 2) hipLaunchKernelGGL((k_solve_hc<1, 2>), dim3(blocks), dim3(HC_TPB), 0, s, (const StepCounters*)d.ctr, (const uint4*)d.hc_entry, d, first_colour);
 		else if (compact_rows) hipLaunchKernelGGL((k_solve_hc<1, 1>), dim3(blocks), dim3(HC_TPB), 0, s, (const StepCounters*)d.ctr, (const uint4*)d.hc_entry, d, first_colour);
diff --git a/substrata_amd/csrc/sgp_kernels.h b/substrata_amd/csrc/sgp_kernels.h
--- a/substrata_amd/csrc/sgp_kernels.h
+++ b/substrata_amd/csrc/sgp_kernels.h
@@ -259,6 +259,15 @@
 	uint4*    hc_entry;
 	uint32_t  cap_hc_list;
 	uint32_t* hc_big_list;
+	uint4*    hc_share;
+	uint32_t* hc_bodies;
+	uint32_t* hc_local;
+	float4*   hc_pnf;
+	float4*   hc_prow;
+	float2*   hc_pefft;
+	float4*   hc_plam;
+	float4*   hc_ploc;
+	uint32_t  hc_pack_cap, hc_pack_cap0;
 	uint32_t dbg_flags;
 	float4* rows;
 	ConstraintArrays ca[2];
@@ -317,9 +326,9 @@
 void launch_warm_bodies(const DV& d, uint32_t nb, hipStream_t s);
 void launch_solve_tail(const DV& d, int first_colour, int mode, hipStream_t s, int compact_rows = 0);
 #define SGP_SMALL_WORLD_BODIES 2048
-void launch_hc_build(const DV& d, int first_colour, uint32_t est, hipStream_t s);
+void launch_hc_build(const DV& d, int first_colour, uint32_t est, hipStream_t s, int layout, int compact_rows);
 void launch_hc_probe(const DV& d, int probe_colour, uint32_t probe_est, hipStream_t s);
-void launch_solve_hc(const DV& d, int first_colour, uint32_t est, int mode, hipStream_t s, int compact_rows);
+void launch_solve_hc(const DV& d, int first_colour, uint32_t est, int mode, hipStream_t s, int compact_rows, int layout, bool last_velocity_pass);
 void launch_solve_small(const DV& d, int warm_start, int iterations, int lane_pairs, hipStream_t s);
 void launch_integrate_pose(const DV& d, uint32_t nb, hipStream_t s);
 void launch_finalize(const DV& d, uint32_t nb, hipStream_t s);
diff --git a/substrata_amd/csrc/sgp_world.hip b/substrata_amd/csrc/sgp_world.hip
--- a/substrata_amd/csrc/sgp_world.hip
+++ b/substrata_amd/csrc/sgp_world.hip
@@ -184,6 +184,22 @@
 		}
 	}
 	d.cap_hc_list = 2u * M + 4096u; DEV_ALLOC(d.hc_list, d.cap_hc_list); DEV_ALLOC(d.hc_entry, d.cap_hc_list); DEV_ALLOC(d.hc_big_list, 1024);
+	{
+		int dev = 0, cus = 0; if (hipGetDevice(&dev) != hipSuccess || hipDeviceGetAttribute(&cus, hipDeviceAttributeMultiprocessorCount, dev) != hipSuccess || cus <= 0) cus = 256;
+		const char* e = getenv("SGP_HC_LAYOUT"); w->hc_layout = !(e && e[0] == '0');
+		const uint32_t list_shares = d.cap_hc_list / 256u + 1u;
+		DEV_ALLOC(d.hc_share, list_shares);
+		d.hc_pack_cap = d.hc_pack_cap0 = 0;
+		if (w->hc_layout) {
+			uint32_t cap = std::min(2u * (uint32_t)cus, list_shares) * 256u, cap0 = std::max(cap / 512u, 1u) * 256u;
+			const char* pc = getenv("SGP_HC_PACK_CAP");
+			if (pc && atoll(pc) >= 0) { cap = (uint32_t)std::min<long long>(atoll(pc), (long long)cap) / 256u * 256u; cap0 = cap; }
+			d.hc_pack_cap = cap; d.hc_pack_cap0 = cap0;
+			const size_t c1 = std::max<size_t>(cap, 256);
+			DEV_ALLOC(d.hc_bodies, 2 * c1); DEV_ALLOC(d.hc_local, c1); DEV_ALLOC(d.hc_pnf, c1);
+			DEV_ALLOC(d.hc_prow, std::max<size_t>(24 * c1, 48 * (size_t)cap0)); DEV_ALLOC(d.hc_pefft, 4 * c1); DEV_ALLOC(d.hc_plam, 4 * c1); DEV_ALLOC(d.hc_ploc, 8 * c1);
+		}
+	}
 	DEV_ALLOC(d.ulist[0], M); DEV_ALLOC(d.ulist[1], M);
 	for (int k = 0; k < 4; ++k) { DEV_ALLOC(d.man_p1[k], M); DEV_ALLOC(d.man_p2[k], M); }
 	DEV_ALLOC(d.rows, (size_t)48 * M);
@@ -555,6 +571,7 @@
 	uint32_t hc_est;
 	int      hc_probe;
 	uint32_t hc_probe_est;
+	int      hc_layout;
 	int      tile_solver;
 	int      small_pairs;
 	int      ev_reset;
@@ -616,6 +633,7 @@
 	}
 	p.tile_solver = (w->use_tile_solver && w->dv.ts_nt && !p.small_world && w->n_vehicles == 0 && p.vel_iters > 0 && w->n_con >= w->ts_min_constraints &&
 	                 w->high >= SGP_MAX_COLOURS * w->dv.ts_nt && w->last_active <= w->dv.ts_nt * 1536u && !w->h_sp->compact_rows) ? w->use_tile_solver : 0;
+	p.hc_layout = (w->hc_layout && p.hc_first >= 0 && !p.tile_solver) ? 1 : 0;
 	p.ev_reset = w->ev_reset_pending ? 1 : 0;
 	p.sp = *w->h_sp;
 	p.sp.parity = 0u;
@@ -660,13 +678,13 @@
 		{ KScope k(w, KC_SETUP); launch_setup(d, p.est_man, s); }
 	}
 	if (p.hc_first >= 0 && p.hc_probe >= 0) { KScope k(w, KC_SETUP); launch_hc_probe(d, p.hc_probe, p.hc_probe_est, s); }
-	if (p.hc_first >= 0) { KScope k(w, KC_SETUP); launch_hc_build(d, p.hc_first, p.hc_est, s); }
+	if (p.hc_first >= 0) { KScope k(w, KC_SETUP); launch_hc_build(d, p.hc_first, p.hc_est, s, p.hc_layout, (int)p.sp.compact_rows); }
 	STAGE_MARK(4);
-	auto solve_pass = [&](int mode, int kc) {
+	auto solve_pass = [&](int mode, int kc, bool last_pass) {
 		const bool veh_fused = p.n_vehicles && p.tail_first > 0 && mode != 0 && w->fuse_vehicle_solve;
 		if (p.n_vehicles && !veh_fused) { KScope k(w, KC_VEHICLE); launch_vehicle_solve(d, mode, s); }
 		for (int c = 0; c < p.tail_first; ++c) { KScope k(w, kc); if (c == 0 && veh_fused) launch_solve_colour_veh(d, c, p.colour_est[c], mode, s, (int)p.sp.compact_rows); else launch_solve_colour(d, c, p.colour_est[c], mode, s, (int)p.sp.compact_rows); }
-		if (p.hc_first >= 0) { KScope k(w, kc); launch_solve_hc(d, p.hc_first, p.hc_est, mode, s, (int)p.sp.compact_rows); }
+		if (p.hc_first >= 0) { KScope k(w, kc); launch_solve_hc(d, p.hc_first, p.hc_est, mode, s, (int)p.sp.compact_rows, p.hc_layout, last_pass); }
 		else { KScope k(w, kc); launch_solve_tail(d, p.tail_first, mode, s, (int)p.sp.compact_rows); }
 	};
 	if (p.small_world) { KScope k(w, KC_SOLVE_VELOCITY); launch_solve_small(d, p.warm_start, p.vel_iters, p.small_pairs, s); }
@@ -679,15 +697,15 @@
 		else if (p.tile_solver == 3 && p.hc_first >= 0) {
 			for (int it = 0; it < p.vel_iters; ++it) {
 				{ KScope k(w, KC_SOLVE_VELOCITY); launch_ts_solve(d, 1, p.tail_first, s); }
-				{ KScope k(w, KC_SOLVE_VELOCITY); launch_solve_hc(d, p.hc_first, p.hc_est, 1, s, (int)p.sp.compact_rows); }
+				{ KScope k(w, KC_SOLVE_VELOCITY); launch_solve_hc(d, p.hc_first, p.hc_est, 1, s, (int)p.sp.compact_rows, p.hc_layout, it + 1 == p.vel_iters); }
 			}
 		}
-		else for (int it = 0; it < p.vel_iters; ++it) solve_pass(1, KC_SOLVE_VELOCITY);
+		else for (int it = 0; it < p.vel_iters; ++it) solve_pass(1, KC_SOLVE_VELOCITY, it + 1 == p.vel_iters);
 	}
 	STAGE_MARK(5);
 	{ KScope k(w, KC_INTEGRATE_POSE); launch_integrate_pose(d, nb, s); }
 	STAGE_MARK(6);
-	for (int it = 0; it < p.pos_iters; ++it) solve_pass(2, KC_SOLVE_POSITION);
+	for (int it = 0; it < p.pos_iters; ++it) solve_pass(2, KC_SOLVE_POSITION, false);
 	STAGE_MARK(7);
 	{ KScope k(w, KC_FINALIZE); launch_finalize(d, nb, s); }
 	for (int r = 0; r < SGP_ISLAND_MARK_ROUNDS; ++r) { KScope k(w, KC_ISLAND_HOOK); launch_island_mark(d, p.est_man, r == 0 ? 1 : 0, s); }
diff --git a/substrata_amd/csrc/sgp_world_checkpoint.hip b/substrata_amd/csrc/sgp_world_checkpoint.hip
--- a/substrata_amd/csrc/sgp_world_checkpoint.hip
+++ b/substrata_amd/csrc/sgp_world_checkpoint.hip
@@ -133,6 +133,7 @@
 	add(w->d_mesh_verts, 'S', 0, sizeof(float4) * w->cap_mesh_verts); add(w->d_mesh_tris, 'S', 0, sizeof(uint4) * w->cap_mesh_tris);
 	add(w->d_mesh_tri_mat, 'S', 0, sizeof(uint32_t) * w->cap_mesh_tri_mat); add(w->d_mesh_nodes, 'S', 0, sizeof(MeshNode) * w->cap_mesh_nodes);
 	add(w->d_mesh_field, 'S', 0, sizeof(uint32_t) * w->cap_mesh_field);
+	add(d.hc_share, 'S', 0); add(d.hc_bodies, 'S', 0); add(d.hc_local, 'S', 0); add(d.hc_pnf, 'S', 0); add(d.hc_prow, 'S', 0); add(d.hc_pefft, 'S', 0); add(d.hc_plam, 'S', 0); add(d.hc_ploc, 'S', 0);
 	uint32_t k = 0;
 	for (void* p : w->allocs) { if (!seen.count(p)) { auto it = w->alloc_bytes.find(p); if (it != w->alloc_bytes.end()) out.push_back(CkptArray{ CKPT_UNNAMED_BASE + k, p, it->second, it->second }); } ++k; }
 }
diff --git a/substrata_amd/csrc/sgp_world_internal.h b/substrata_amd/csrc/sgp_world_internal.h
--- a/substrata_amd/csrc/sgp_world_internal.h
+++ b/substrata_amd/csrc/sgp_world_internal.h
@@ -110,6 +110,7 @@
 	uint32_t compact_rows_min = 1000000;
 	int use_tile_solver = 0;
 	uint32_t ts_min_constraints = 16384;
+	bool hc_layout = true;
 	bool use_components = true; uint32_t hc_budget = 160; uint32_t n_cus = 256; uint32_t hc_min_colours = 4; int hc_k = -1; uint32_t hc_bump = 1, hc_since_bump = 0xFFFFu; uint32_t hc_probe_in = 8, hc_probe_gap = 16;
 	bool bp_dense_last = false;
 	bool plan_seen = false;
diff --git a/substrata_amd/csrc/sgp_world_tiles.hip b/substrata_amd/csrc/sgp_world_tiles.hip
--- a/substrata_amd/csrc/sgp_world_tiles.hip
+++ b/substrata_amd/csrc/sgp_world_tiles.hip
@@ -269,10 +269,17 @@
 {
 	if (!w || !dev_ptr_out) return fail(SGP_ERR_INVALID, "sgp_world_device_array: NULL");
 	void* p = nullptr;
+	uint32_t n = w->high;
+	const uint32_t hc_entries = w->h_ctr ? w->h_ctr->hc_entries : 0u;
+	const uint32_t hc_cap = (w->h_sp && w->h_sp->compact_rows == 0u) ? w->dv.hc_pack_cap0 : w->dv.hc_pack_cap;
 	switch (which) { case 0: p = w->dv.pose; break; case 1: p = w->dv.vel; break;
+	case 2: p = w->dv.hc_entry; n = hc_entries; break;
+	case 3: p = w->dv.hc_share; n = hc_entries / 256u; break;
+	case 4: p = w->dv.hc_bodies; n = 2u * std::min(hc_entries, hc_cap); break;
+	case 5: p = w->dv.hc_local; n = std::min(hc_entries, hc_cap); break;
 	default: return fail(SGP_ERR_INVALID, "sgp_world_device_array: bad index"); }
 	*dev_ptr_out = p;
-	if (count_out) *count_out = w->high;
+	if (count_out) *count_out = n;
 	return SGP_OK;
 }
 
```

Result: faster. 553.5 steps/s (median of 6 runs) (+1.1%).
